# theislab/dca

Measured on NVIDIA H100. Metric: cells/sec (ZINB AE epoch, device-timed), higher is better.
Workload: dtype bf16-gemm/f32-acc/f32-loss

## Files before the change

### dca_b200/_lib.py

```python
from __future__ import annotations

import ctypes as C
import os

_HERE = os.path.dirname(os.path.abspath(__file__))
LIB_PATH = os.path.join(_HERE, "libdca_b200.so")

DCA_MAX_HIDDEN = 8
DCA_NAME_LEN = 48

ACTIVATION_IDS = {"relu": 0, "linear": 1, "elu": 2, "selu": 3, "tanh": 4, "sigmoid": 5, "hard_sigmoid": 6,
                  "softplus": 7, "softsign": 8, "exponential": 9, "LeakyReLU": 10, "PReLU": 11}
OPTIMIZERS = {"RMSprop": (0, 1e-3), "SGD": (1, 1e-2), "Adagrad": (2, 1e-2), "Adadelta": (3, 1.0), "Adam": (4, 1e-3),
              "Adamax": (5, 2e-3), "Nadam": (6, 2e-3)}
OPTIMIZERS.update({k.lower(): v for k, v in list(OPTIMIZERS.items())})
AE_TYPE_IDS = {"zinb-conddisp": 0, "zinb": 1, "nb-conddisp": 2, "nb": 3,
               "poisson": 4, "normal": 5, "nb-shared": 6, "zinb-shared": 7, "zinb-elempi": 8, "nb-fork": 9, "zinb-fork": 10}
F32, BF16 = 0, 1
GEMM_AUTO, GEMM_GENERIC, GEMM_TCGEN05 = 0, 1, 2
REGION_PARAMS, REGION_GRADS, REGION_RMS, REGION_BN_STATE, REGION_EPOCH_ACC = 0, 1, 2, 3, 4


class DcaError(RuntimeError):
    pass


class Config(C.Structure):
    _fields_ = [
        ("struct_bytes", C.c_int32), ("n_in", C.c_int32), ("n_out", C.c_int32),
        ("n_hidden", C.c_int32), ("hidden", C.c_int32 * DCA_MAX_HIDDEN),
        ("ae_type", C.c_int32), ("batchnorm", C.c_int32), ("max_batch", C.c_int32),
        ("x_dtype", C.c_int32), ("gemm_path", C.c_int32),
        ("ridge", C.c_float), ("l1", C.c_float), ("l2", C.c_float),
        ("l1_enc", C.c_float), ("l2_enc", C.c_float),
        ("bn_momentum", C.c_float), ("bn_eps", C.c_float),
        ("rms_rho", C.c_float), ("rms_eps", C.c_float),
        ("elempi_shared", C.c_int32), ("sync_bn", C.c_int32),
        ("activation", C.c_int32), ("input_dropout", C.c_float),
        ("hidden_dropout", C.c_float * DCA_MAX_HIDDEN), ("dropout_seed", C.c_uint64),
    ]


class TensorInfo(C.Structure):
    _fields_ = [("name", C.c_char * DCA_NAME_LEN), ("offset", C.c_int64),
                ("rows", C.c_int32), ("cols", C.c_int32)]


class PackedCountsDesc(C.Structure):
    _fields_ = [
        ("struct_bytes", C.c_int32), ("bits", C.c_int32), ("n_rows", C.c_int64), ("genes", C.c_int32),
        ("max_row_nibble_bytes", C.c_int32), ("packed", C.c_void_p), ("ovf_indptr", C.c_void_p),
        ("ovf_entries", C.c_void_p), ("nib_indptr", C.c_void_p), ("nibbles", C.c_void_p), ("n_counts", C.c_void_p),
    ]


_vp, _i32, _i64, _f, _sz = C.c_void_p, C.c_int32, C.c_int64, C.c_float, C.c_size_t
PROTOTYPES = {
    "dca_version": (C.c_int, []),
    "dca_last_error": (C.c_char_p, []),
    "dca_config_default": (None, [C.POINTER(Config)]),
    "dca_arena_bytes": (C.c_int, [C.POINTER(Config), C.POINTER(_sz)]),
    "dca_create": (C.c_int, [C.POINTER(Config), _vp, _sz, C.POINTER(_vp)]),
    "dca_destroy": (C.c_int, [_vp]),
    "dca_param_count": (C.c_int, [_vp, C.POINTER(_i64), C.POINTER(_i32)]),
    "dca_param_info": (C.c_int, [_vp, _i32, C.POINTER(TensorInfo)]),
    "dca_state_count": (C.c_int, [_vp, C.POINTER(_i64), C.POINTER(_i32)]),
    "dca_state_info": (C.c_int, [_vp, _i32, C.POINTER(TensorInfo)]),
    "dca_region": (C.c_int, [_vp, _i32, C.POINTER(_vp), C.POINTER(_i64)]),
    "dca_init_params": (C.c_int, [_vp, C.c_uint64, _vp]),
    "dca_params_changed": (C.c_int, [_vp, _vp]),
    "dca_train_step": (C.c_int, [_vp, _vp, _i64, _vp, _i64, _vp, _vp, _i32, _vp]),
    "dca_train_step_phase": (C.c_int, [_vp, _vp, _i64, _vp, _i64, _vp, _vp, _i32, _i32, _vp]),
    "dca_grad_buckets": (C.c_int, [_vp, C.POINTER(_i64)]),
    "dca_comm_unique_id": (C.c_int, [_vp]),
    "dca_comm_init": (C.c_int, [_vp, _vp, _i32, _i32]),
    "dca_comm_destroy": (C.c_int, [_vp]),
    "dca_allreduce": (C.c_int, [_vp, _vp]),
    "dca_train_step_dp": (C.c_int, [_vp, _vp, _i64, _vp, _i64, _vp, _vp, _i32, _vp]),
    "dca_set_optimizer": (C.c_int, [_vp, _i32, _vp]),
    "dca_reset_optimizer": (C.c_int, [_vp, _vp]),
    "dca_apply_update": (C.c_int, [_vp, _f, _f, _f, _vp]),
    "dca_eval_step": (C.c_int, [_vp, _vp, _i64, _vp, _i64, _vp, _vp, _i32, _vp]),
    "dca_predict": (C.c_int, [_vp, _vp, _i64, _vp, _vp, _i32, _vp, _vp, _vp, _i64, _vp, _vp]),
    "dca_read_loss": (C.c_int, [_vp, C.POINTER(_f), C.POINTER(_i32), _vp]),
    "dca_read_epoch_acc": (C.c_int, [_vp, C.POINTER(C.c_double * 4), _i32, _vp]),
    "dca_train_step_host": (C.c_int, [_vp, _vp, _vp, _vp, _i32, _f, _f, C.POINTER(_f), _vp]),
    "dca_set_input_transform": (C.c_int, [_vp, _vp, _vp, _i32, _i32, _vp]),
    "dca_set_loss_ring": (C.c_int, [_vp, _vp, _i32]),
    "dca_stream_begin": (C.c_int, [_vp, _vp, _i64, _vp, _i64, _i32, _vp]),
    "dca_stream_begin_packed": (C.c_int, [_vp, _vp, _i32, _i64, _vp, _vp, _vp, _i64, _i32, _vp]),
    "dca_stream_begin_sparse": (C.c_int, [_vp, _vp, _vp, _vp, _vp, _vp, _vp, _i64, _i32, _vp]),
    "dca_stream_step": (C.c_int, [_vp, _i64, _i64, _vp]),
    "dca_stream_end": (C.c_int, [_vp, _vp]),
    "dca_expand_packed_counts": (C.c_int, [_vp, _i32, _vp, _vp, _vp, _i32, _i32, _vp, _vp, _i32, _i32, _vp, _vp, _i32, _vp,
                                           _vp]),
    "dca_expand_sparse_counts": (C.c_int, [_vp, _vp, _vp, _i32, _vp, _vp, _vp, _i32, _i32, _vp, _vp, _i32, _i32, _vp, _vp,
                                           _i32, _vp, _vp]),
    "dca_zinb_loss_fwd_bwd": (C.c_int, [_vp, _i64, _vp, _vp, _vp, _vp, _vp, _i64, _i32, _i32, _i32, _f, _f,
                                        _vp, _vp, _vp, _i32, _vp, _vp, _vp, _sz, _vp]),
    "dca_zinb_loss_workspace_bytes": (C.c_int, [_i32, _i32, C.POINTER(_sz)]),
    "dca_zinb_loss_fwd": (C.c_int, [_vp, _i64, _vp, _vp, _vp, _vp, _vp, _i64, _i32, _i32, _i32, _f,
                                    _vp, _vp, _sz, _vp]),
    "dca_zinb_elem_host": (C.c_int, [_i32, _f, _f, _f, _f, _f, _f, C.POINTER(_f * 4)]),
    "dca_dropout_mask_host": (C.c_int, [C.c_uint64, C.c_uint64, _i32, _i64, _f, _vp]),
    "dca_activation_host": (C.c_int, [_i32, _f, _f, C.POINTER(_f * 2)]),
    "dca_dense_heads_fwd": (C.c_int, [_vp, _i64, _i32, _i32, _i32, _vp, _vp, _vp, _vp, _vp, _vp, _vp,
                                      _vp, _vp, _vp, _i64, _vp]),
    "dca_tc_heads_fwd": (C.c_int, [_vp, _i32, _vp, _vp, _i32, _i32, C.POINTER(_i32 * 3), _vp, _vp, _vp, _vp, _i64, _vp]),
    "dca_tc_heads_loss": (C.c_int, [_vp, _i32, _vp, _vp, _i32, _vp, _i64, _vp, _vp, _f, _f, _vp, _vp, _vp, _i64, _vp,
                                    _vp, _sz, _vp]),
    "dca_tc_gene_gemm": (C.c_int, [_i32, _vp, _vp, _vp, _i64, _i32, _i32, _i32, _vp, _vp, _vp, _vp, _vp, _vp, _i64, _i32,
                                   _vp, _vp, _vp, _vp]),
    "dca_tc_gene_gemm_sms": (C.c_int, [_i32, _vp, _vp, _vp, _i64, _i32, _i32, _i32, _vp, _vp, _vp, _vp, _vp, _vp, _i64,
                                       _i32, _vp, _vp, _vp, _vp, _i32]),
    "dca_tc_gene_gemm_rows": (C.c_int, [_i32, _vp, _vp, _vp, _i64, _vp, _i32, _i32, _i32, _vp, _vp, _vp, _vp, _vp, _vp,
                                        _i64, _i32, _vp, _vp, _vp, _vp, _i32]),
    "dca_tc_probe": (C.c_int, [_vp, _i32, _i32, _vp, _i32, _i32, _i32, _i32, _i32, _i32, _i32, _i32, _i32, _i32, _i32,
                               _vp, _vp]),
    "dca_profile_enable": (C.c_int, [_vp, _i32]),
    "dca_profile_read": (C.c_int, [_vp, C.POINTER(C.c_double * 6), C.POINTER(C.c_int64 * 6), _i32]),
    "dca_engine_info": (C.c_int, [_vp, C.POINTER(_i32 * 8)]),
    "dca_write_text_matrix": (C.c_int, [C.c_char_p, _vp, _i32, _i64, _i64, _i64, _vp, _vp, _i32, _i32]),
    "dca_read_text_counts": (C.c_int, [C.c_char_p, _i32, _i32, _i64, _i32, _vp, _vp, _i64, _vp, _vp, _i64, _vp]),
    "dca_count_escapes": (C.c_int, [_vp, _i32, _i64, _i64, _i64, _vp, _i32]),
    "dca_pack_counts": (C.c_int, [_vp, _i32, _i64, _i64, _i64, _i32, _vp, _vp, _vp, _i32]),
    "dca_sparse_counts": (C.c_int, [_vp, _i32, _i64, _i64, _i64, _vp, _vp, _i32]),
    "dca_pack_sparse": (C.c_int, [_vp, _i32, _i64, _i64, _i64, _vp, _vp, _vp, _vp, _vp, _i32]),
    "dca_preprocess_workspace_bytes": (C.c_int, [_i64, _i32, C.POINTER(_sz)]),
    "dca_counts_csr_to_dense": (C.c_int, [_vp, _vp, _vp, _i64, _i32, _vp, _i64, _vp]),
    "dca_count_totals": (C.c_int, [_vp, _i64, _i64, _i32, _vp, _vp, _vp, _vp, _sz, _vp]),
    "dca_gather_counts": (C.c_int, [_vp, _i64, _vp, _i64, _vp, _i32, _vp, _i64, _vp]),
    "dca_log_moments": (C.c_int, [_vp, _i64, _i64, _i32, _vp, C.c_double, _i32, _vp, _vp, _vp, _sz, _vp]),
    "dca_normalize_write": (C.c_int, [_vp, _i64, _i64, _i32, _vp, C.c_double, _i32, _vp, _vp, _vp, _i32, _i64, _vp]),
    "dca_stats_workspace_bytes": (C.c_int, [_i64, _i32, _i64, C.POINTER(_sz)]),
    "dca_stats_begin": (C.c_int, [_i64, _i32, _vp, _sz, _vp]),
    "dca_count_totals_rows": (C.c_int, [_vp, _i64, _i64, _i64, _i64, _i32, _vp, _vp, _sz, _vp]),
    "dca_count_totals_finish": (C.c_int, [_i64, _i32, _vp, _vp, _vp, _sz, _vp]),
    "dca_log_moments_rows": (C.c_int, [_i32, _vp, _i64, _i64, _i64, _i64, _i32, _vp, C.c_double, _i32, _vp, _vp, _sz,
                                       _vp]),
    "dca_log_moments_finish": (C.c_int, [_i32, _i64, _i32, _i32, _vp, _vp, _sz, _vp]),
    "dca_set_input_transform_exact": (C.c_int, [_vp, _vp, _vp, C.c_double, _i32, _vp]),
    "dca_stream_row_totals": (C.c_int, [_vp, _vp]),
    "dca_stream_predict": (C.c_int, [_vp, _i64, _i64, _vp, _vp, _vp, _i64, _vp, _vp]),
    "dca_stream_eval": (C.c_int, [_vp, _i64, _i64, _vp]),
    "dca_stream_capacity": (C.c_int, [_vp, C.POINTER(_i64), C.POINTER(_i64)]),
    "dca_expand_packed_counts_exact": (C.c_int, [_vp, _i32, _vp, _vp, _vp, _i32, _i32, C.c_double, _i32, _vp, _vp, _vp,
                                                 _vp, _i32, _vp, _vp]),
    "dca_expand_sparse_counts_exact": (C.c_int, [_vp, _vp, _vp, _i32, _vp, _vp, _vp, _i32, _i32, C.c_double, _i32, _vp,
                                                 _vp, _vp, _vp, _i32, _vp, _vp]),
    "dca_pack_count_rows": (C.c_int, [_vp, _i64, _i64, _i32, _vp, _i64, _vp]),
    "dca_pack_rows_device": (C.c_int, [_vp, _i64, _i64, _i64, C.POINTER(PackedCountsDesc), _vp]),
    "dca_expand_rows_exact": (C.c_int, [C.POINTER(PackedCountsDesc), _vp, _i32, C.c_double, _i32, _vp, _vp, _vp, _vp, _i32,
                                        _vp, _vp]),
    "dca_packed_train_step": (C.c_int, [_vp, C.POINTER(PackedCountsDesc), _vp, _i32, _vp]),
    "dca_packed_eval_step": (C.c_int, [_vp, C.POINTER(PackedCountsDesc), _vp, _i32, _vp]),
    "dca_packed_predict": (C.c_int, [_vp, C.POINTER(PackedCountsDesc), _vp, _i32, _vp, _vp, _vp, _i64, _vp, _vp]),
    "dca_launch_count": (C.c_int64, []),
    "dca_set_tunable": (C.c_int, [C.c_char_p, C.c_int64]),
}

_lib = None


def load():
    global _lib
    if _lib is not None:
        return _lib
    if not os.path.exists(LIB_PATH):
        raise ImportError(
            "dca_b200: %s not found. Build it with `python -c 'import __graft_entry__ as g; g.build()'` "
            "(or `make -C dca_b200/csrc`). There is no CPU fallback." % LIB_PATH)
    lib = C.CDLL(LIB_PATH)
    for name, (res, args) in PROTOTYPES.items():
        fn = getattr(lib, name)
        fn.restype = res
        fn.argtypes = args
    _lib = lib
    return lib


def check(status: int, what: str = ""):
    if status != 0:
        msg = load().dca_last_error().decode("utf-8", "replace")
        if status == -1:
            raise ValueError("%s: %s" % (what or "dca_b200", msg))
        raise DcaError("%s failed (status %d): %s" % (what or "dca_b200", status, msg))


def set_tunable(name: str, value: int):
    check(load().dca_set_tunable(name.encode(), int(value)), "dca_set_tunable")


def default_config() -> Config:
    cfg = Config()
    load().dca_config_default(C.byref(cfg))
    return cfg
```

### dca_b200/csrc/dca_internal.cuh

```cuda
#pragma once
#include <cuda_runtime.h>
#include <cuda_bf16.h>
#include <stdint.h>
#include <stddef.h>
#include <atomic>
#include "../../include/dca_b200.h"

namespace dca {

void set_error(const char* fmt, ...);
extern std::atomic<long long> g_launches;
inline void count_launch(int n = 1) { g_launches.fetch_add(n, std::memory_order_relaxed); }

#define DCA_CUDA_OK(expr)                                                              \
  do {                                                                                 \
    cudaError_t _e = (expr);                                                           \
    if (_e != cudaSuccess) {                                                           \
      ::dca::set_error("%s failed: %s (%s:%d)", #expr, cudaGetErrorString(_e), __FILE__, __LINE__); \
      return DCA_ERR_CUDA;                                                             \
    }                                                                                  \
  } while (0)

#define DCA_LAUNCH_CHECK()                                                             \
  do {                                                                                 \
    ::dca::count_launch();                                                             \
    cudaError_t _e = cudaGetLastError();                                               \
    if (_e != cudaSuccess) {                                                           \
      ::dca::set_error("kernel launch failed: %s (%s:%d)", cudaGetErrorString(_e), __FILE__, __LINE__); \
      return DCA_ERR_CUDA;                                                             \
    }                                                                                  \
  } while (0)

#define DCA_TRY(expr)                \
  do {                               \
    int _s = (expr);                 \
    if (_s != DCA_OK) return _s;     \
  } while (0)

static inline int cdiv(long long a, long long b) { return (int)((a + b - 1) / b); }

enum Epilogue : int {
  EPI_STORE = 0,
  EPI_ACCUM = 1,
  EPI_MEAN_ACT = 2,
  EPI_DISP_ACT = 3,
  EPI_SIGMOID = 4,
  EPI_LINEAR_SCALE = 5
};

struct GemmArgs {
  const void* A; int64_t lda; int a_bf16; int transA;
  const int32_t* a_rows;
  const float* B; int64_t ldb; int transB;
  float* C; int64_t ldc;
  int M, N, K;
  const float* bias;
  const float* row_scale;
  int epilogue;
  int splits;
};
int gemm_generic(const GemmArgs& g, cudaStream_t s);

int fill_rows_with_bias(float* C, int64_t ldc, int M, int N, const float* bias, cudaStream_t s);
int col_sums(const float* a, const float* b, int64_t ld, int M, int N, double* out_sum, double* out_prod,
             double* scratch, cudaStream_t s);
int col_sums_scratch_elems(int M, int N);
int bn_train_finalize(const double* sum, const double* sq, int M, int N, float eps, float momentum,
                      float* mean, float* inv_std, float* moving_mean, float* moving_var, cudaStream_t s);
int bn_relu_fwd(const float* a, int64_t ld, int M, int N, const float* mean, const float* inv_std,
                const float* beta, float* xhat, float* h, __nv_bfloat16* h_bf16, cudaStream_t s);
int bn_infer_prepare(const float* moving_mean, const float* moving_var, int N, float eps,
                     float* mean, float* inv_std, cudaStream_t s);
int bias_relu_fwd(const float* a, int64_t ld, int M, int N, float* h, __nv_bfloat16* h_bf16, cudaStream_t s);
int relu_bwd(float* dh, const float* h, int64_t ld, int M, int N, cudaStream_t s);
int bn_bwd_apply(float* g_inout, const float* xhat, int64_t ld, int M, int N, const float* inv_std,
                 const double* sum_g, const double* sum_gx, float* dbeta, cudaStream_t s, int stat_rows = 0);
int col_sum_to_float(const double* sum, int N, float* out, cudaStream_t s);
int theta_prepare(const float* theta_raw, int G, float* theta, float* chain, cudaStream_t s);
int theta_grad_finish(const float* dtheta, const float* chain, int G, float scale, float* grad_out, cudaStream_t s);
int add_reg_grad(const float* w, float* g, int64_t n, float l1, float l2, cudaStream_t s);
int reg_penalty(const float* w, int64_t n, float l1, float l2, double* acc, cudaStream_t s);
int rmsprop_update(float* params, const float* grads, float* rms, int64_t n, float lr, float clip,
                   float rho, float eps, float grad_scale, __nv_bfloat16* shadow, float* loss_out, cudaStream_t s);
struct OptScalars { int kind; float lr, clip, gs, c0, c1, c2, c3, c4; };
int optimizer_update(float* params, const float* grads, float* s1, float* s2, int64_t n, OptScalars o, __nv_bfloat16* shadow,
                     float* loss_out, cudaStream_t s);
int glorot_fill(float* w, int64_t n, int fan_in, int fan_out, uint64_t seed, uint64_t stream_id, cudaStream_t s);
int fill_value(float* p, int64_t n, float v, cudaStream_t s);
int cast_to_bf16(const float* in, __nv_bfloat16* out, int64_t n, cudaStream_t s);

__device__ __forceinline__ float pre_log_value(float y, double sf64, int flags) {
  float q = (flags & DCA_PRE_SIZE_FACTORS) ? (float)((double)y / sf64) : y;
  if ((flags & DCA_PRE_LOG1P) && q != 0.f) q = (float)log1p((double)q);
  return q;
}
struct ExactXform {
  const double* n_counts; double median; int flags;
  const double* mean; const double* std; const float* x_zero;
};
int exact_zero_inputs(const double* mean, const double* std, int n, float* x_zero, cudaStream_t s);
int expand_counts(const void* cnt, int bits, const float* sf_in, int M, int n, const float* mean, const float* inv_std, int use_sf,
                  int use_log1p, float* Yout, void* Xout, int x_bf16, float* sf_out, const int64_t* ovf_indptr,
                  const void* ovf_entries, cudaStream_t s, const ExactXform* ex = nullptr, const int32_t* rows = nullptr);
int expand_sparse(const void* bitmap, const int64_t* nib_indptr, const void* nibbles, const float* sf_in, int M, int n,
                  const float* mean, const float* inv_std, int use_sf, int use_log1p, float* Yout, void* Xout, int x_bf16,
                  float* sf_out, const int64_t* ovf_indptr, const void* ovf_entries, int max_row_nibble_bytes, cudaStream_t s,
                  const ExactXform* ex = nullptr, const int32_t* rows = nullptr);
int check_packed_counts(const char* who, const dca_packed_counts* p);
int gather_rows_bf16(const void* X, int x_bf16, int64_t ldx, const int32_t* rows, int M, int n, __nv_bfloat16* out,
                     cudaStream_t s);

namespace tc {
int heads_fwd_tc(const __nv_bfloat16* Hb, int B, const __nv_bfloat16* const W[3], const float* const bias[3], int G,
                 int n_heads, const int kind[3], const float* row_scale, float* const out[3], int64_t ld_out, int sm_count,
                 cudaStream_t s);
int gene_gemm_tc(int mode, const __nv_bfloat16* const Z[3], int64_t ldz, const int32_t* rows, int B, int G, int n_heads,
                 const __nv_bfloat16* H, const __nv_bfloat16* const W[3], float* out_b, float* const dW[3], int64_t dW_ld,
                 int dW_transposed, float* const db[3], void* ws, size_t ws_bytes, int sm_count, cudaStream_t s);
size_t gene_gemm_workspace_bytes(int B);
int flash_zinb_tc(const __nv_bfloat16* H3, int B, int G, const __nv_bfloat16* const W[3], const float* const bias[3],
                  const float* Y, int64_t ldy, const int32_t* rows, const float* sf, float ridge, float inv_n,
                  float* dH3, float* const dW[3], float* const db[3], void* ws, size_t ws_bytes, double* loss_sum,
                  const double* penalty, float* loss_slot, double* epoch_acc, int batch, const float* lf_dev, int sm_count,
                  cudaStream_t s);
}

struct LossArgs {
  const float* Y; int64_t ldy; const int32_t* rows; const float* sf;
  const float* m; const float* d; const float* pi; int64_t ld;
  int B, G; int ae_type; float ridge; float inv_n;
  void* dzm; void* dzd; void* dzp; int grad_bf16;
  float* dtheta;
  double* loss_sum;
  void* ws; size_t ws_bytes;
  int counter_ready = 0;
  float* fin_loss_slot = nullptr; double* fin_epoch_acc = nullptr; const double* fin_penalty = nullptr; int fin_batch = 0;
};
size_t loss_workspace_bytes(int B, int G);
extern int g_fused_heads_default;
const float* loss_log_fact_table();
int zinb_loss_fwd_bwd(const LossArgs& a, cudaStream_t s);
int zinb_loss_fwd(const LossArgs& a, cudaStream_t s);

struct HeadsLossArgs {
  const __nv_bfloat16* H3; int B, G;
  const __nv_bfloat16* W[3]; const float* bias[3];
  const float* Y; int64_t ldy; const int32_t* rows; const float* sf;
  float ridge, inv_n;
  __nv_bfloat16* dz[3]; int64_t ldz;
  double* loss_sum; void* ws; size_t ws_bytes;
  int counter_ready = 0;
  float* fin_loss_slot = nullptr; double* fin_epoch_acc = nullptr; const double* fin_penalty = nullptr; int fin_batch = 0;
};
int heads_loss_tc(const HeadsLossArgs& a, cudaStream_t s);

}
```

### dca_b200/csrc/dense_tc.cu

```cuda
#include <mutex>
#include "engine.h"
#include "tc_common.cuh"
#include "head_act.cuh"

namespace dca {
namespace tc {

typedef CUresult (*EncodeTiledFn)(CUtensorMap*, CUtensorMapDataType, cuuint32_t, void*, const cuuint64_t*,
                                  const cuuint64_t*, const cuuint32_t*, const cuuint32_t*, CUtensorMapInterleave,
                                  CUtensorMapSwizzle, CUtensorMapL2promotion, CUtensorMapFloatOOBfill);

static EncodeTiledFn encode_fn() {
  static EncodeTiledFn fn = nullptr;
  static std::once_flag once;
  std::call_once(once, [] {
    void* p = nullptr;
    cudaDriverEntryPointQueryResult q;
    if (cudaGetDriverEntryPoint("cuTensorMapEncodeTiled", &p, cudaEnableDefault, &q) == cudaSuccess &&
        q == cudaDriverEntryPointSuccess)
      fn = reinterpret_cast<EncodeTiledFn>(p);
  });
  return fn;
}

int make_tensor_map_2d(CUtensorMap* out, const void* base, int elem_bytes, int is_bf16, uint64_t rows, uint64_t cols,
                       uint64_t ld_elems, uint32_t box_rows, uint32_t box_cols, int swizzle) {
  EncodeTiledFn fn = encode_fn();
  if (!fn) { set_error("cuTensorMapEncodeTiled is not available from the driver"); return DCA_ERR_CUDA; }
  cuuint64_t dims[2] = {cols, rows};
  cuuint64_t strides[1] = {ld_elems * (uint64_t)elem_bytes};
  cuuint32_t box[2] = {box_cols, box_rows};
  cuuint32_t estr[2] = {1, 1};
  const CUtensorMapDataType dt = is_bf16 ? CU_TENSOR_MAP_DATA_TYPE_BFLOAT16 : CU_TENSOR_MAP_DATA_TYPE_FLOAT32;
  CUresult r = fn(out, dt, 2, const_cast<void*>(base), dims, strides, box, estr, CU_TENSOR_MAP_INTERLEAVE_NONE,
                  swizzle ? CU_TENSOR_MAP_SWIZZLE_128B : CU_TENSOR_MAP_SWIZZLE_NONE, CU_TENSOR_MAP_L2_PROMOTION_L2_256B,
                  CU_TENSOR_MAP_FLOAT_OOB_FILL_NONE);
  if (r != CUDA_SUCCESS) {
    set_error("cuTensorMapEncodeTiled failed (%d): rows=%llu cols=%llu ld=%llu box=%ux%u elem=%d", (int)r,
              (unsigned long long)rows, (unsigned long long)cols, (unsigned long long)ld_elems, box_rows, box_cols, elem_bytes);
    return DCA_ERR_CUDA;
  }
  return DCA_OK;
}

struct ProbeParams {
  int a_mn, b_mn, M, N, K;
  int a_boxes, a_box_bytes, a_box_c0, a_box_c1;
  int b_boxes, b_box_bytes, b_box_c0, b_box_c1;
  uint32_t a_lbo, a_sbo, a_kstep, a_kblock_steps, a_kblock_bytes, a_mn64_bytes;
  uint32_t b_lbo, b_sbo, b_kstep, b_kblock_steps, b_kblock_bytes, b_mn64_bytes;
};

template <int NC, int TA, int TB>
__device__ __forceinline__ void probe_mma(float (&acc)[NC / 2], uint64_t da, uint64_t db) {
  if constexpr (NC == 128) wgmma_m64n128k16<TA, TB>(acc, da, db, 1u);
  else wgmma_m64n64k16<TA, TB>(acc, da, db, 1u);
}

template <int NC>
__device__ __forceinline__ void probe_chunk(const ProbeParams& p, uint32_t sa, uint32_t sb, int m0, int n0, float* D) {
  float acc[NC / 2];
#pragma unroll
  for (int i = 0; i < NC / 2; ++i) acc[i] = 0.f;
  const uint32_t a0 = sa + (uint32_t)(m0 / 64) * p.a_mn64_bytes, b0 = sb + (uint32_t)(n0 / 64) * p.b_mn64_bytes;
  wgmma_fence();
  for (int j = 0; j < p.K / 16; ++j) {
    const uint32_t aoff = (j / p.a_kblock_steps) * p.a_kblock_bytes + (j % p.a_kblock_steps) * p.a_kstep;
    const uint32_t boff = (j / p.b_kblock_steps) * p.b_kblock_bytes + (j % p.b_kblock_steps) * p.b_kstep;
    const uint64_t da = make_smem_desc(a0 + aoff, p.a_lbo, p.a_sbo), db = make_smem_desc(b0 + boff, p.b_lbo, p.b_sbo);
    if (p.a_mn) { if (p.b_mn) probe_mma<NC, 1, 1>(acc, da, db); else probe_mma<NC, 1, 0>(acc, da, db); }
    else        { if (p.b_mn) probe_mma<NC, 0, 1>(acc, da, db); else probe_mma<NC, 0, 0>(acc, da, db); }
  }
  wgmma_commit();
  wgmma_wait<0>();
  acc_fence(acc);
  const int w = threadIdx.x >> 5, l = threadIdx.x & 31;
#pragma unroll
  for (int i = 0; i < NC / 2; ++i) {
    const int row = m0 + 16 * w + (l >> 2) + 8 * ((i >> 1) & 1), col = n0 + 8 * (i >> 2) + 2 * (l & 3) + (i & 1);
    D[(size_t)row * p.N + col] = acc[i];
  }
}

__global__ void __launch_bounds__(128, 1)
tc_probe_kernel(const __grid_constant__ CUtensorMap map_a, const __grid_constant__ CUtensorMap map_b,
                const ProbeParams p, float* __restrict__ D) {
  extern __shared__ __align__(1024) uint8_t smem_raw[];
  uint8_t* smem = smem_raw + ((1024u - (smem_u32(smem_raw) & 1023u)) & 1023u);
  __shared__ uint64_t bar_load;
  uint8_t* sa = smem;
  uint8_t* sb = smem + (size_t)p.a_boxes * p.a_box_bytes;
  if (threadIdx.x == 0) { mbar_init(&bar_load, 1); fence_barrier_init(); }
  __syncthreads();
  if (threadIdx.x == 0) {
    mbar_expect_tx(&bar_load, (uint32_t)(p.a_boxes * p.a_box_bytes + p.b_boxes * p.b_box_bytes));
    for (int i = 0; i < p.a_boxes; ++i) tma_load_2d(sa + (size_t)i * p.a_box_bytes, &map_a, i * p.a_box_c0, i * p.a_box_c1, &bar_load);
    for (int i = 0; i < p.b_boxes; ++i) tma_load_2d(sb + (size_t)i * p.b_box_bytes, &map_b, i * p.b_box_c0, i * p.b_box_c1, &bar_load);
  }
  mbar_wait(&bar_load, 0);
  for (int m0 = 0; m0 < p.M; m0 += 64)
    for (int n0 = 0; n0 < p.N;) {
      if (p.N - n0 >= 128) { probe_chunk<128>(p, smem_u32(sa), smem_u32(sb), m0, n0, D); n0 += 128; }
      else { probe_chunk<64>(p, smem_u32(sa), smem_u32(sb), m0, n0, D); n0 += 64; }
    }
}

namespace k2 {
constexpr int BM = 128, BN = 128, BK = 64;
constexpr int kThreads = 256;
constexpr uint32_t kABytes = BM * BK * 2, kBBytes = BN * BK * 2;
constexpr uint32_t kSmemBytes = kABytes + kBBytes + 1024;

struct Params {
  int B, G, n_heads;
  int kind[3];
  int m_tiles, n_tiles_per_head;
  const float* bias[3];
  const float* row_scale;
  float* out[3]; int64_t ld_out;
};

__global__ void __launch_bounds__(kThreads, 2)
heads_fwd_kernel(const __grid_constant__ CUtensorMap map_h, const __grid_constant__ CUtensorMap map_w0,
                 const __grid_constant__ CUtensorMap map_w1, const __grid_constant__ CUtensorMap map_w2, const Params p) {
  extern __shared__ __align__(1024) uint8_t smem_raw[];
  uint8_t* smem = smem_raw + ((1024u - (smem_u32(smem_raw) & 1023u)) & 1023u);
  __shared__ uint64_t full_bar;
  const int mt = blockIdx.x % p.m_tiles, r = blockIdx.x / p.m_tiles;
  const int nt = r % p.n_tiles_per_head, hs = r / p.n_tiles_per_head;
  if (threadIdx.x == 0) {
    mbar_init(&full_bar, 1);
    fence_barrier_init();
    const CUtensorMap* mw = hs == 0 ? &map_w0 : (hs == 1 ? &map_w1 : &map_w2);
    mbar_expect_tx(&full_bar, kABytes + kBBytes);
    tma_load_2d(smem, &map_h, 0, mt * BM, &full_bar);
    tma_load_2d(smem + kABytes, mw, nt * BN, 0, &full_bar);
    tma_load_2d(smem + kABytes + kBBytes / 2, mw, nt * BN + 64, 0, &full_bar);
  }
  __syncthreads();
  const int wg = threadIdx.x >> 7, w = (threadIdx.x >> 5) & 3, l = threadIdx.x & 31;
  const int col0 = nt * BN + 2 * (l & 3);
  const int row0 = mt * BM + wg * 64 + 16 * w + (l >> 2);
  const float* bias = p.bias[hs];
  const int kind = p.kind[hs];
  float2 bz[16];
#pragma unroll
  for (int c = 0; c < 16; ++c) bz[c] = (col0 + 8 * c < p.G) ? *reinterpret_cast<const float2*>(bias + col0 + 8 * c) : make_float2(0.f, 0.f);
  float rs[2] = {1.f, 1.f};
  if (kind == EPI_MEAN_ACT && p.row_scale) {
    if (row0 < p.B) rs[0] = p.row_scale[row0];
    if (row0 + 8 < p.B) rs[1] = p.row_scale[row0 + 8];
  }
  float acc[64];
#pragma unroll
  for (int i = 0; i < 64; ++i) acc[i] = 0.f;
  mbar_wait(&full_bar, 0);
  head_tile_mma(acc, smem_u32(smem) + wg * 64 * 128, smem_u32(smem) + kABytes);
  float* out = p.out[hs];
  auto emit = [&](auto act) {
#pragma unroll
    for (int h = 0; h < 2; ++h) {
      const int row = row0 + 8 * h;
      if (row >= p.B) continue;
      float* orow = out + (int64_t)row * p.ld_out;
#pragma unroll
      for (int c = 0; c < 16; ++c) {
        const int col = col0 + 8 * c;
        if (col < p.G)
          *reinterpret_cast<float2*>(orow + col) =
              make_float2(act(acc[4 * c + 2 * h], bz[c].x, rs[h]), act(acc[4 * c + 2 * h + 1], bz[c].y, rs[h]));
      }
    }
  };
  if (kind == EPI_MEAN_ACT) emit([](float a, float b, float s) { return head_out<EPI_MEAN_ACT>(a, b, s); });
  else if (kind == EPI_DISP_ACT) emit([](float a, float b, float s) { return head_out<EPI_DISP_ACT>(a, b, s); });
  else emit([](float a, float b, float s) { return head_out<EPI_SIGMOID>(a, b, s); });
}
}

int heads_fwd_tc(const __nv_bfloat16* Hb, int B, const __nv_bfloat16* const W[3], const float* const bias[3], int G,
                 int n_heads, const int kind[3], const float* row_scale, float* const out[3], int64_t ld_out, int sm_count,
                 cudaStream_t s) {
  using namespace k2;
  if (ld_out % 4 != 0 || G % 8 != 0) { set_error("heads_fwd_tc: G must be a multiple of 8 and ld_out of 4 (TMA strides)"); return DCA_ERR_BAD_ARG; }
  CUtensorMap mh, mw[3];
  DCA_TRY(make_tensor_map_2d(&mh, Hb, 2, 1, (uint64_t)B, 64, 64, BM, BK, 1));
  for (int i = 0; i < 3; ++i)
    DCA_TRY(make_tensor_map_2d(&mw[i], W[i < n_heads ? i : 0], 2, 1, 64, (uint64_t)G, (uint64_t)G, 64, 64, 1));
  Params p;
  p.B = B; p.G = G; p.n_heads = n_heads;
  for (int i = 0; i < 3; ++i) { const int k = i < n_heads ? i : 0; p.kind[i] = kind[i]; p.bias[i] = bias[k]; p.out[i] = out[k]; }
  p.m_tiles = cdiv(B, BM); p.n_tiles_per_head = cdiv(G, BN);
  p.row_scale = row_scale; p.ld_out = ld_out;
  (void)sm_count;
  static bool attr_set = false;
  if (!attr_set) {
    DCA_CUDA_OK(cudaFuncSetAttribute(heads_fwd_kernel, cudaFuncAttributeMaxDynamicSharedMemorySize, (int)kSmemBytes));
    attr_set = true;
  }
  const int grid = p.m_tiles * p.n_tiles_per_head * n_heads;
  heads_fwd_kernel<<<grid, kThreads, kSmemBytes, s>>>(mh, mw[0], mw[1], mw[2], p);
  DCA_LAUNCH_CHECK();
  return DCA_OK;
}

}

Engine::~Engine() {
  comm_destroy();
  for (auto e : prof.ev) cudaEventDestroy(e);
  for (auto& g : graphs) if (g.exec) cudaGraphExecDestroy(g.exec);
  if (hs.copy) cudaStreamDestroy(hs.copy);
  if (hs.expand) cudaStreamDestroy(hs.expand);
  for (int k = 0; k < 3; ++k) {
    if (hs.ready[k]) cudaEventDestroy(hs.ready[k]);
    if (hs.step_done[k]) cudaEventDestroy(hs.step_done[k]);
  }
  for (int k = 0; k < 2; ++k) {
    if (hs.h2d_done[k]) cudaEventDestroy(hs.h2d_done[k]);
    if (hs.cnt_free[k]) cudaEventDestroy(hs.cnt_free[k]);
  }
}

}

using namespace dca;

extern "C" int dca_tc_probe(const void* A, int32_t a_rows, int32_t a_cols, const void* Bm, int32_t b_rows, int32_t b_cols,
                            int32_t a_mn_major, int32_t b_mn_major, int32_t M, int32_t N, int32_t K,
                            int32_t a_lbo, int32_t a_sbo, int32_t b_lbo, int32_t b_sbo, float* D, void* stream) {
  using namespace tc;
  if (M != 128 || N % 64 != 0 || N < 64 || N > 256 || K % 64 != 0 || K <= 0 || K > 256) {
    set_error("dca_tc_probe: need M=128, N%%64==0 (64..256), K%%64==0 (<=256)"); return DCA_ERR_BAD_ARG;
  }
  ProbeParams p{};
  p.a_mn = a_mn_major; p.b_mn = b_mn_major; p.M = M; p.N = N; p.K = K;
  CUtensorMap ma, mb;
  auto setup = [&](int mn, int mn_extent, int rows, int cols, const void* base, CUtensorMap* map, int& boxes, int& box_bytes,
                   int& c0, int& c1, uint32_t& lbo, uint32_t& sbo, uint32_t& kstep, uint32_t& kb_steps, uint32_t& kb_bytes,
                   uint32_t& mn64_bytes, int lbo_o, int sbo_o) -> int {
    if (!mn) {
      if (rows != mn_extent || cols != K) { set_error("dca_tc_probe: K-major operand must be [MN x K]"); return DCA_ERR_BAD_ARG; }
      DCA_TRY(make_tensor_map_2d(map, base, 2, 1, rows, cols, cols, mn_extent, 64, 1));
      boxes = K / 64; box_bytes = mn_extent * 128; c0 = 64; c1 = 0;
      lbo = 0; sbo = 1024; kstep = 32; kb_steps = 4; kb_bytes = box_bytes; mn64_bytes = 64 * 128;
    } else {
      if (rows != K || cols != mn_extent || mn_extent % 64) { set_error("dca_tc_probe: MN-major operand must be [K x MN], MN%%64==0"); return DCA_ERR_BAD_ARG; }
      DCA_TRY(make_tensor_map_2d(map, base, 2, 1, rows, cols, cols, K, 64, 1));
      boxes = mn_extent / 64; box_bytes = K * 128; c0 = 64; c1 = 0;
      lbo = box_bytes; sbo = 1024; kstep = 2048; kb_steps = 1u << 30; kb_bytes = 0; mn64_bytes = box_bytes;
    }
    if (lbo_o >= 0) lbo = lbo_o;
    if (sbo_o >= 0) sbo = sbo_o;
    return DCA_OK;
  };
  DCA_TRY(setup(a_mn_major, M, a_rows, a_cols, A, &ma, p.a_boxes, p.a_box_bytes, p.a_box_c0, p.a_box_c1, p.a_lbo, p.a_sbo,
                p.a_kstep, p.a_kblock_steps, p.a_kblock_bytes, p.a_mn64_bytes, a_lbo, a_sbo));
  DCA_TRY(setup(b_mn_major, N, b_rows, b_cols, Bm, &mb, p.b_boxes, p.b_box_bytes, p.b_box_c0, p.b_box_c1, p.b_lbo, p.b_sbo,
                p.b_kstep, p.b_kblock_steps, p.b_kblock_bytes, p.b_mn64_bytes, b_lbo, b_sbo));
  const size_t smem = (size_t)p.a_boxes * p.a_box_bytes + (size_t)p.b_boxes * p.b_box_bytes + 1024;
  DCA_CUDA_OK(cudaFuncSetAttribute(tc_probe_kernel, cudaFuncAttributeMaxDynamicSharedMemorySize, (int)smem));
  tc_probe_kernel<<<1, 128, smem, (cudaStream_t)stream>>>(ma, mb, p, D);
  DCA_LAUNCH_CHECK();
  return DCA_OK;
}

extern "C" int dca_tc_heads_fwd(const void* Hb, int32_t batch, const void* Wk, const float* bias, int32_t genes,
                                int32_t n_heads, const int32_t kind[3], const float* row_scale, float* out0, float* out1,
                                float* out2, int64_t ld_out, void* stream) {
  if (!Hb || !Wk || !bias || batch <= 0 || genes <= 0 || n_heads < 1 || n_heads > 3 || !out0) {
    set_error("dca_tc_heads_fwd: bad argument"); return DCA_ERR_BAD_ARG;
  }
  int dev = 0, sms = 132;
  cudaGetDevice(&dev);
  cudaDeviceGetAttribute(&sms, cudaDevAttrMultiProcessorCount, dev);
  int k[3] = {kind[0], n_heads > 1 ? kind[1] : 0, n_heads > 2 ? kind[2] : 0};
  float* outs[3] = {out0, out1, out2};
  const __nv_bfloat16* W[3]; const float* b[3];
  for (int i = 0; i < 3; ++i) {
    const int j = i < n_heads ? i : 0;
    W[i] = (const __nv_bfloat16*)Wk + (size_t)j * 64 * genes; b[i] = bias + (size_t)j * genes;
  }
  return tc::heads_fwd_tc((const __nv_bfloat16*)Hb, batch, W, b, genes, n_heads, k, row_scale, outs, ld_out, sms,
                          (cudaStream_t)stream);
}
```

### dca_b200/csrc/engine.cu

```cuda
#include <cmath>
#include <cstdarg>
#include <cstdio>
#include <cstring>
#include <cstdlib>
#include <string>
#include <vector>
#include "dca_internal.cuh"
#include "engine.h"

namespace dca {

std::atomic<long long> g_launches{0};
static thread_local char g_err[512] = "";

void set_error(const char* fmt, ...) {
  va_list ap;
  va_start(ap, fmt);
  vsnprintf(g_err, sizeof(g_err), fmt, ap);
  va_end(ap);
}

namespace {

inline size_t align_up(size_t v, size_t a = 256) { return (v + a - 1) / a * a; }

__global__ void add_double_kernel(double* p, double v) { *p += v; }
__global__ void gather_sf_kernel(const float* __restrict__ sf, const int32_t* __restrict__ rows, int n,
                                 float* __restrict__ out) {
  const int i = blockIdx.x * blockDim.x + threadIdx.x;
  if (i < n) out[i] = sf ? sf[rows ? rows[i] : i] : 1.0f;
}
__global__ void copy_strided_kernel(const float* __restrict__ in, int64_t ldi, float* __restrict__ out, int64_t ldo,
                                    int M, int N) {
  const int64_t i = (int64_t)blockIdx.x * blockDim.x + threadIdx.x;
  if (i >= (int64_t)M * N) return;
  const int r = (int)(i / N), c = (int)(i % N);
  out[(int64_t)r * ldo + c] = in[(int64_t)r * ldi + c];
}

int validate(const dca_config* c) {
  if (!c) { set_error("config is NULL"); return DCA_ERR_BAD_ARG; }
  if (c->struct_bytes != (int32_t)sizeof(dca_config)) {
    set_error("dca_config.struct_bytes=%d does not match library (%zu): header/library mismatch", c->struct_bytes,
              sizeof(dca_config));
    return DCA_ERR_BAD_ARG;
  }
  if (c->n_in <= 0 || c->n_out <= 0) { set_error("n_in/n_out must be positive (got %d, %d)", c->n_in, c->n_out); return DCA_ERR_BAD_ARG; }
  if (c->n_hidden < 0 || c->n_hidden > DCA_MAX_HIDDEN) { set_error("n_hidden must be in [0,%d]", DCA_MAX_HIDDEN); return DCA_ERR_BAD_ARG; }
  for (int i = 0; i < c->n_hidden; ++i)
    if (c->hidden[i] <= 0) { set_error("hidden[%d] must be positive", i); return DCA_ERR_BAD_ARG; }
  if (c->ae_type < 0 || c->ae_type > DCA_AE_ZINB_FORK) { set_error("autoencoder type not supported (ae_type=%d)", c->ae_type); return DCA_ERR_UNSUPPORTED; }
  if (c->max_batch <= 0) { set_error("max_batch must be positive"); return DCA_ERR_BAD_ARG; }
  if (c->x_dtype != DCA_F32 && c->x_dtype != DCA_BF16) { set_error("x_dtype must be DCA_F32 or DCA_BF16"); return DCA_ERR_BAD_ARG; }
  if (c->gemm_path < 0 || c->gemm_path > 2) { set_error("unknown gemm_path %d", c->gemm_path); return DCA_ERR_BAD_ARG; }
  if (c->activation < DCA_ACT_RELU || c->activation > DCA_ACT_PRELU) { set_error("unknown activation %d", c->activation); return DCA_ERR_BAD_ARG; }
  if (c->activation == DCA_ACT_PRELU && c->ae_type >= DCA_AE_NB_FORK) {
    set_error("activation PReLU is not available for the fork types"); return DCA_ERR_UNSUPPORTED;
  }
  if (!(c->input_dropout >= 0.f && c->input_dropout < 1.f)) { set_error("input_dropout must be in [0, 1)"); return DCA_ERR_BAD_ARG; }
  for (int i = 0; i < c->n_hidden; ++i)
    if (!(c->hidden_dropout[i] >= 0.f && c->hidden_dropout[i] < 1.f)) { set_error("hidden_dropout[%d] must be in [0, 1)", i); return DCA_ERR_BAD_ARG; }
  return DCA_OK;
}

void add_tensor(std::vector<dca_tensor_info>& v, int64_t& off, const std::string& name, int rows, int cols) {
  dca_tensor_info t;
  memset(&t, 0, sizeof(t));
  snprintf(t.name, sizeof(t.name), "%s", name.c_str());
  t.offset = off; t.rows = rows; t.cols = cols;
  off += (int64_t)rows * cols;
  v.push_back(t);
}

std::string layer_name(int i, int n) {
  const int center = n / 2;
  if (i == center) return "center";
  if (i < center) return "enc" + std::to_string(i);
  return "dec" + std::to_string(i - center);
}

}

int Engine::plan(const dca_config& c) {
  cfg = c;
  L = c.n_hidden;
  has_pi = (c.ae_type == DCA_AE_ZINB_CONDDISP || c.ae_type == DCA_AE_ZINB);
  cond = (c.ae_type == DCA_AE_ZINB_CONDDISP || c.ae_type == DCA_AE_NB_CONDDISP);
  params.clear(); states.clear(); reg_items.clear();
  int64_t off = 0, soff = 0;
  x_kind = 0; n_branch = 0; trunk_L = L;
  if (c.ae_type >= DCA_AE_POISSON) {
    DCA_TRY(x_plan_params(c, off, soff));
  } else {
  int prev = c.n_in;
  maxh = 1;
  for (int i = 0; i < L; ++i) {
    const std::string nm = layer_name(i, L);
    const int h = c.hidden[i];
    lay[i].in = prev; lay[i].out = h;
    lay[i].W = off; add_tensor(params, off, nm + "/kernel", prev, h);
    lay[i].b = off; add_tensor(params, off, nm + "/bias", 1, h);
    if (c.batchnorm) {
      lay[i].beta = off; add_tensor(params, off, nm + "/bn_beta", 1, h);
      lay[i].mm = soff; add_tensor(states, soff, nm + "/bn_moving_mean", 1, h);
      lay[i].mv = soff; add_tensor(states, soff, nm + "/bn_moving_var", 1, h);
    }
    if (c.activation == DCA_ACT_PRELU) { lay[i].alpha = off; add_tensor(params, off, nm + "_act/alpha", 1, h); }
    lay[i].drop = c.hidden_dropout[i]; lay[i].id = i;
    prev = h;
    if (h > maxh) maxh = h;
  }
  K_head = prev;
  head_W[0] = off; add_tensor(params, off, "mean/kernel", prev, c.n_out);
  head_b[0] = off; add_tensor(params, off, "mean/bias", 1, c.n_out);
  head_W[1] = head_b[1] = head_W[2] = head_b[2] = theta_off = -1;
  if (cond) {
    head_W[1] = off; add_tensor(params, off, "dispersion/kernel", prev, c.n_out);
    head_b[1] = off; add_tensor(params, off, "dispersion/bias", 1, c.n_out);
  }
  if (has_pi) {
    head_W[2] = off; add_tensor(params, off, "pi/kernel", prev, c.n_out);
    head_b[2] = off; add_tensor(params, off, "pi/bias", 1, c.n_out);
  }
  if (!cond) { theta_off = off; add_tensor(params, off, "dispersion/theta", 1, c.n_out); }
  }
  P = off; S = soff;

  const int G = c.n_out;
  const size_t B = (size_t)c.max_batch;
  size_t o = 0;
  auto take = [&](size_t bytes) { size_t at = o; o = align_up(o + bytes); return at; };
  o_params = take(sizeof(float) * (size_t)P);
  o_grads = take(sizeof(float) * (size_t)(P + 2));
  o_rms = take(sizeof(float) * (size_t)P);
  o_opt2 = take(sizeof(float) * (size_t)P);
  o_state = take(sizeof(float) * (size_t)(S > 0 ? S : 1));
  o_acc = take(sizeof(double) * 8);
  for (int i = 0; i < L; ++i) {
    const size_t h = (size_t)c.hidden[i];
    lay[i].o_a = take(sizeof(float) * B * h);
    lay[i].o_xhat = take(sizeof(float) * B * h);
    lay[i].o_h = take(sizeof(float) * B * h);
    lay[i].o_mean = take(sizeof(float) * h);
    lay[i].o_inv = take(sizeof(float) * h);
  }
  for (int k = 0; k < 3; ++k) o_head[k] = take(sizeof(float) * B * (size_t)G);
  o_dh[0] = take(sizeof(float) * B * (size_t)maxh);
  o_dh[1] = take(sizeof(float) * B * (size_t)maxh);
  const size_t statw = (size_t)(maxh > G ? maxh : G);
  o_dsum = take(sizeof(double) * statw);
  o_dprod = take(sizeof(double) * statw);
  o_scratch = take(sizeof(double) * (size_t)col_sums_scratch_elems((int)B, (int)statw));
  o_theta = take(sizeof(float) * (size_t)G);
  o_chain = take(sizeof(float) * (size_t)G);
  o_dtheta = take(sizeof(float) * (size_t)G);
  o_sfb = take(sizeof(float) * B);
  loss_ws_bytes = loss_workspace_bytes((int)B, G);
  o_lossws = take(loss_ws_bytes);
  o_rowsbuf = take(sizeof(int32_t) * B);
  o_step = take(256);
  if (c.activation == DCA_ACT_PRELU) o_actscr = take(sizeof(float) * B * (size_t)maxh);
  if (c.input_dropout > 0.f) o_xdrop = take((c.x_dtype == DCA_BF16 ? sizeof(__nv_bfloat16) : sizeof(float)) * B * (size_t)c.n_in);
  mid_ok = !x_kind && plain_hidden() && mid_supported(c.hidden, L);
  o_bar = take(256);
  o_midpart = take(sizeof(double) * mid_partial_doubles());
  o_midgpart = take(sizeof(float) * mid_grad_partial_floats(L));
  n_slots = 0;
  slot_head[0] = 0; slot_kind[0] = EPI_MEAN_ACT; n_slots = 1;
  if (cond) { slot_head[n_slots] = 1; slot_kind[n_slots] = EPI_DISP_ACT; ++n_slots; }
  if (has_pi) { slot_head[n_slots] = 2; slot_kind[n_slots] = EPI_SIGMOID; ++n_slots; }
  const bool want_tc = c.gemm_path != DCA_GEMM_GENERIC && !x_kind;
  tc_heads = want_tc && L >= 1 && K_head == 64 && (G % 8 == 0);
  tc_enc = want_tc && L >= 1 && c.hidden[0] == 64 && (c.n_in % 8 == 0);
  if (tc_heads) for (int k = 0; k < 3; ++k) if (head_W[k] >= 0 && (head_W[k] % 8) != 0) tc_heads = false;
  {
    const char* ev = getenv("DCA_FUSED_HEADS");
    const bool want = ev ? atoi(ev) != 0 : g_fused_heads_default != 0;
    fused_heads = want && tc_heads && cond && has_pi && L >= 1 && (G % 8 == 0);
  }
  if (tc_enc && (lay[0].W % 8) != 0) tc_enc = false;
  if (tc_heads || tc_enc) o_pbf = take(2 * (size_t)P);
  if (tc_heads || tc_enc) { ggws_bytes = tc::gene_gemm_workspace_bytes((int)B); o_ggws = take(ggws_bytes); }
  if (tc_heads) {
    o_h3b = take(2 * B * 64);
    for (int k = 0; k < n_slots; ++k) o_dzb[k] = take(2 * B * (size_t)G);
  }
  if (tc_enc) {
    o_da1b = take(2 * B * 64);
    if (c.x_dtype != DCA_BF16) o_xb = take(2 * B * (size_t)c.n_in);
  }
  for (int k = 0; k < 2; ++k) { o_cnt[k] = take(sizeof(uint16_t) * B * (size_t)c.n_in); o_sfst[k] = take(sizeof(float) * B); }
  ovf_cap = (int64_t)(B * (size_t)c.n_in / 32); if (ovf_cap < 4096) ovf_cap = 4096;
  for (int k = 0; k < 2; ++k) { o_ovp[k] = take(sizeof(int64_t) * (B + 1)); o_ove[k] = take(8 * (size_t)ovf_cap); }
  nib_cap = (int64_t)(B * (size_t)c.n_in / 4) + 64;
  for (int k = 0; k < 2; ++k) { o_nibp[k] = take(sizeof(int64_t) * (B + 1)); o_nib[k] = take((size_t)nib_cap); }
  o_gmean = take(sizeof(float) * (size_t)c.n_in); o_ginv = take(sizeof(float) * (size_t)c.n_in);
  o_gmean64 = take(sizeof(double) * (size_t)c.n_in); o_gstd64 = take(sizeof(double) * (size_t)c.n_in);
  o_gx0 = take(sizeof(float) * (size_t)c.n_in);
  for (int k = 0; k < 2; ++k) o_ncst[k] = take(sizeof(double) * B);
  const size_t xb = (c.x_dtype == DCA_BF16) ? 2 : 4;
  for (int k = 0; k < kExpBufs; ++k) {
    o_sx[k] = take(xb * B * (size_t)c.n_in);
    o_sy[k] = take(sizeof(float) * B * (size_t)G);
    o_ssf[k] = take(sizeof(float) * B);
  }
  o_stage_x = o_sx[0]; o_stage_y = o_sy[0]; o_stage_sf = o_ssf[0];
  if (x_kind) x_plan_arena(B, take);
  arena_bytes = o;
  return DCA_OK;
}

void Engine::mark(int phase, cudaStream_t s) {
  if (!prof.on) return;
  if (prof.n == prof.ev.size()) {
    cudaEvent_t e;
    if (cudaEventCreate(&e) != cudaSuccess) return;
    prof.ev.push_back(e); prof.phase.push_back(-1);
  }
  prof.phase[prof.n] = phase;
  cudaEventRecord(prof.ev[prof.n], s);
  ++prof.n;
}

int Engine::prof_collect() {
  if (prof.n == 0) return DCA_OK;
  DCA_CUDA_OK(cudaEventSynchronize(prof.ev[prof.n - 1]));
  for (size_t i = 0; i + 1 < prof.n; ++i) {
    const int ph = prof.phase[i];
    if (ph < 0 || ph >= DCA_N_PHASES) continue;
    float ms = 0.f;
    if (cudaEventElapsedTime(&ms, prof.ev[i], prof.ev[i + 1]) == cudaSuccess) { prof.ms[ph] += ms; prof.cnt[ph] += 1; }
  }
  prof.n = 0;
  return DCA_OK;
}

void Engine::bind(void* base_) {
  base = reinterpret_cast<char*>(base_);
}

int Engine::gemm_auto(GemmArgs g, cudaStream_t s) {
  const long long tiles = (long long)cdiv(g.M, 64) * cdiv(g.N, 64), target = 2ll * sm_count;
  int splits = 1;
  if (g.epilogue == EPI_ACCUM && tiles < target && g.K >= 256) {
    splits = (int)((target + tiles - 1) / tiles);
    const int maxs = g.K / 128;
    if (splits > maxs) splits = maxs;
    if (splits < 1) splits = 1;
  }
  g.splits = splits;
  return gemm_generic(g, s);
}

int Engine::forward(const void* X, int64_t ldx, const int32_t* rows, int Bn, bool training, cudaStream_t s) {
  const void* hin = X; int64_t ldin = ldx; int in_bf16 = x_override_bf16 ? 1 : (cfg.x_dtype == DCA_BF16); const int32_t* gather = rows;
  cur_x = XOperand{};
  if (tc_enc && (reinterpret_cast<uintptr_t>(X) & 15) == 0) {
    if (in_bf16 && ldx % 8 == 0) cur_x = XOperand{reinterpret_cast<const __nv_bfloat16*>(X), ldx, rows};
    else if (!in_bf16 && ldx % 4 == 0) {
      DCA_TRY(gather_rows_bf16(X, in_bf16, ldx, rows, Bn, cfg.n_in, bf(o_xb), s));
      cur_x = XOperand{bf(o_xb), cfg.n_in, nullptr};
    }
  }
  const bool fused = use_mid(Bn);
  for (int i = 0; i < (fused ? 1 : L); ++i) {
    Layer& l = lay[i];
    float* a = f(l.o_a);
    DCA_TRY(fill_rows_with_bias(a, l.out, Bn, l.out, pp(l.b), s));
    if (i == 0 && cur_x.base) {
      const __nv_bfloat16* Z[3] = {cur_x.base, cur_x.base, cur_x.base};
      const __nv_bfloat16* W1[3] = {bf(o_pbf) + lay[0].W, bf(o_pbf) + lay[0].W, bf(o_pbf) + lay[0].W};
      DCA_TRY(tc::gene_gemm_tc(1, Z, cur_x.ld, cur_x.rows, Bn, cfg.n_in, 1, nullptr, W1, a, nullptr, 0, 0, nullptr, base + o_ggws, ggws_bytes, sm_count, s));
    } else {
    GemmArgs g{};
    g.A = hin; g.lda = ldin; g.a_bf16 = in_bf16; g.transA = 0; g.a_rows = gather;
    g.B = pp(l.W); g.ldb = l.out; g.transB = 0;
    g.C = a; g.ldc = l.out; g.M = Bn; g.N = l.out; g.K = l.in; g.epilogue = EPI_ACCUM;
    DCA_TRY(gemm_auto(g, s));
    }
    if (fused) break;
    if (cfg.batchnorm) {
      if (training) {
        DCA_TRY(col_sums(a, nullptr, l.out, Bn, l.out, d(o_dsum), d(o_dprod), d(o_scratch), s));
        DCA_TRY(bn_allreduce(d(o_dsum), d(o_dprod), l.out, s));
        DCA_TRY(bn_train_finalize(d(o_dsum), d(o_dprod), bn_rows(Bn), l.out, cfg.bn_eps, cfg.bn_momentum, f(l.o_mean),
                                  f(l.o_inv), st(l.mm), st(l.mv), s));
      } else {
        DCA_TRY(bn_infer_prepare(st(l.mm), st(l.mv), l.out, cfg.bn_eps, f(l.o_mean), f(l.o_inv), s));
      }
    }
    DCA_TRY(act_fwd(l, Bn, training, (tc_heads && i == L - 1) ? bf(o_h3b) : nullptr, s));
    hin = f(l.o_h); ldin = l.out; in_bf16 = 0; gather = nullptr;
  }
  if (fused) {
    mid::Params mp;
    mid_params(mp, Bn, training);
    DCA_TRY(mid_forward(mp, s));
    hin = f(lay[L - 1].o_h); ldin = lay[L - 1].out; in_bf16 = 0; gather = nullptr;
  }
  head_in = hin; head_ld = ldin; head_bf16 = in_bf16; head_rows = gather;
  return DCA_OK;
}

int Engine::x_gather_sf(const float* sf, const int32_t* rows, int Bn, cudaStream_t s) {
  gather_sf_kernel<<<cdiv(Bn, 256), 256, 0, s>>>(sf, rows, Bn, f(o_sfb));
  DCA_LAUNCH_CHECK();
  return DCA_OK;
}

void Engine::mid_params(mid::Params& p, int Bn, bool training) {
  memset(&p, 0, sizeof(p));
  p.L = L; p.B = Bn; p.training = training ? 1 : 0; p.batchnorm = cfg.batchnorm; p.center = L / 2;
  for (int i = 0; i < L; ++i) {
    Layer& l = lay[i];
    p.w[i] = l.out; p.W[i] = pp(l.W); p.b[i] = pp(l.b);
    p.beta[i] = cfg.batchnorm ? pp(l.beta) : nullptr;
    p.mm[i] = cfg.batchnorm ? st(l.mm) : nullptr; p.mv[i] = cfg.batchnorm ? st(l.mv) : nullptr;
    p.mean[i] = f(l.o_mean); p.inv[i] = f(l.o_inv); p.xhat[i] = f(l.o_xhat); p.h[i] = f(l.o_h);
    p.gW[i] = gp(l.W); p.gb[i] = gp(l.b); p.gbeta[i] = cfg.batchnorm ? gp(l.beta) : nullptr;
  }
  p.a0 = f(lay[0].o_a); p.a_center = f(lay[L / 2].o_a);
  p.h_last_bf16 = tc_heads ? bf(o_h3b) : nullptr;
  p.partial = d(o_midpart); p.gpart = f(o_midgpart); p.bar = reinterpret_cast<unsigned*>(base + o_bar);
  p.eps = cfg.bn_eps; p.momentum = cfg.bn_momentum;
}

int Engine::heads_forward(int Bn, float* m_out, float* d_out, float* p_out, int64_t ld_out, const float* row_scale,
                          cudaStream_t s) {
  const int G = cfg.n_out;
  if (tc_heads && (ld_out % 4 == 0)) {
    float* outs_by_head[3] = {m_out, d_out, p_out};
    bool all = true;
    for (int k = 0; k < n_slots; ++k) all = all && outs_by_head[slot_head[k]] && ((reinterpret_cast<uintptr_t>(outs_by_head[slot_head[k]]) & 15) == 0);
    if (all) {
      float* outs[3] = {nullptr, nullptr, nullptr};
      for (int k = 0; k < n_slots; ++k) outs[k] = outs_by_head[slot_head[k]];
      for (int k = n_slots; k < 3; ++k) outs[k] = outs[0];
      const __nv_bfloat16* Wk[3]; const float* bk[3];
      for (int k = 0; k < 3; ++k) { const int kk = k < n_slots ? k : 0; Wk[k] = bf(o_pbf) + head_W[slot_head[kk]]; bk[k] = pp(head_b[slot_head[kk]]); }
      return tc::heads_fwd_tc(bf(o_h3b), Bn, Wk, bk, G, n_slots, slot_kind, row_scale, outs, ld_out, sm_count, s);
    }
  }
  struct H { int k; float* out; int epi; const float* rs; } hs[3] = {
      {0, m_out, EPI_MEAN_ACT, row_scale}, {1, d_out, EPI_DISP_ACT, nullptr}, {2, p_out, EPI_SIGMOID, nullptr}};
  for (auto& h : hs) {
    if (head_W[h.k] < 0 || !h.out) continue;
    GemmArgs g{};
    g.A = head_in; g.lda = head_ld; g.a_bf16 = head_bf16; g.transA = 0; g.a_rows = head_rows;
    g.B = pp(head_W[h.k]); g.ldb = G; g.transB = 0;
    g.C = h.out; g.ldc = ld_out; g.M = Bn; g.N = G; g.K = K_head;
    g.bias = pp(head_b[h.k]); g.row_scale = h.rs; g.epilogue = h.epi; g.splits = 1;
    DCA_TRY(gemm_generic(g, s));
  }
  return DCA_OK;
}

int Engine::penalty(cudaStream_t s, bool& any) {
  any = false;
  auto coeff = [&](int i, float& l1, float& l2) {
    const int center = L / 2;
    const bool enc = (i >= 0 && i <= center);
    l1 = (enc && cfg.l1_enc != 0.f) ? cfg.l1_enc : cfg.l1;
    l2 = (enc && cfg.l2_enc != 0.f) ? cfg.l2_enc : cfg.l2;
  };
  for (int i = 0; i < L; ++i) {
    float l1, l2; coeff(i, l1, l2);
    if (l1 != 0.f || l2 != 0.f) any = true;
  }
  if (cfg.l1 != 0.f || cfg.l2 != 0.f) any = true;
  if (!any) return DCA_OK;
  DCA_CUDA_OK(cudaMemsetAsync(d(o_acc) + 5, 0, sizeof(double), s));
  for (int i = 0; i < L; ++i) {
    float l1, l2; coeff(i, l1, l2);
    if (l1 == 0.f && l2 == 0.f) continue;
    const int64_t n = (int64_t)lay[i].in * lay[i].out;
    DCA_TRY(reg_penalty(pp(lay[i].W), n, l1, l2, d(o_acc) + 5, s));
    DCA_TRY(add_reg_grad(pp(lay[i].W), gp(lay[i].W), n, l1, l2, s));
  }
  if (cfg.l1 != 0.f || cfg.l2 != 0.f) {
    for (int k = 0; k < 3; ++k) {
      if (head_W[k] < 0) continue;
      const int64_t n = (int64_t)K_head * cfg.n_out;
      DCA_TRY(reg_penalty(pp(head_W[k]), n, cfg.l1, cfg.l2, d(o_acc) + 5, s));
      DCA_TRY(add_reg_grad(pp(head_W[k]), gp(head_W[k]), n, cfg.l1, cfg.l2, s));
    }
  }
  return DCA_OK;
}

int Engine::train_step(const void* X, int64_t ldx, const float* Y, int64_t ldy, const float* sf, const int32_t* rows,
                       int Bn, cudaStream_t s, int phase) {
  if (phase < 0 || phase > 3) { set_error("dca_train_step: phase must be 0, 1, 2 or 3"); return DCA_ERR_BAD_ARG; }
  if (!X || !Y) { set_error("dca_train_step: X and Y must not be NULL"); return DCA_ERR_BAD_ARG; }
  if (Bn <= 0 || Bn > cfg.max_batch) { set_error("dca_train_step: batch %d outside (0, max_batch=%d]", Bn, cfg.max_batch); return DCA_ERR_BAD_ARG; }
  if (!graphs_enabled || prof.on || s == nullptr || s == cudaStreamLegacy || s == cudaStreamPerThread)
    return phase == 3 ? train_step_dp_body(X, ldx, Y, ldy, sf, rows, Bn, s) : train_step_body(X, ldx, Y, ldy, sf, rows, Bn, s, phase);
  StepGraph* g = nullptr;
  for (auto& c : graphs)
    if (c.X == X && c.ldx == ldx && c.Y == Y && c.ldy == ldy && c.sf == sf && c.Bn == Bn && c.has_rows == (rows != nullptr) && c.phase == phase) { g = &c; break; }
  if (!g) {
    if (graphs.size() >= 16) { for (auto& c : graphs) if (c.exec) cudaGraphExecDestroy(c.exec); graphs.clear(); }
    graphs.push_back(StepGraph{X, ldx, Y, ldy, sf, Bn, rows != nullptr, phase, nullptr, 0, 0});
    g = &graphs.back();
  }
  int32_t* rbuf = reinterpret_cast<int32_t*>(base + o_rowsbuf);
  if (!g->exec && g->seen >= 1 && g->seen < 1000) {
    const long long l0 = g_launches.load();
    if (cudaStreamBeginCapture(s, cudaStreamCaptureModeThreadLocal) == cudaSuccess) {
      const int st = phase == 3 ? train_step_dp_body(X, ldx, Y, ldy, sf, rows ? rbuf : nullptr, Bn, s)
                                : train_step_body(X, ldx, Y, ldy, sf, rows ? rbuf : nullptr, Bn, s, phase);
      cudaGraph_t graph = nullptr;
      const cudaError_t ce = cudaStreamEndCapture(s, &graph);
      if (st == DCA_OK && ce == cudaSuccess && graph && cudaGraphInstantiate(&g->exec, graph, 0) == cudaSuccess) {
        g->launches = g_launches.load() - l0;
        g_launches.store(l0);
      } else {
        if (getenv("DCA_GRAPH_DEBUG"))
          fprintf(stderr, "[dca_b200] graph capture failed: body status %d (%s), end-capture %s\n", st, g_err,
                  cudaGetErrorString(ce));
        g->exec = nullptr; g->seen = 1000;
        (void)cudaGetLastError();
      }
      if (graph) cudaGraphDestroy(graph);
    } else {
      if (getenv("DCA_GRAPH_DEBUG")) fprintf(stderr, "[dca_b200] cudaStreamBeginCapture failed: %s\n", cudaGetErrorString(cudaGetLastError()));
      (void)cudaGetLastError(); g->seen = 1000;
    }
  }
  if (g->exec) {
    if (rows && phase != 2) DCA_CUDA_OK(cudaMemcpyAsync(rbuf, rows, sizeof(int32_t) * (size_t)Bn, cudaMemcpyDeviceToDevice, s));
    DCA_CUDA_OK(cudaGraphLaunch(g->exec, s));
    count_launch((int)g->launches);
    return DCA_OK;
  }
  if (g->seen < 1000) ++g->seen;
  return phase == 3 ? train_step_dp_body(X, ldx, Y, ldy, sf, rows, Bn, s) : train_step_body(X, ldx, Y, ldy, sf, rows, Bn, s, phase);
}

int Engine::train_step_body(const void* X, int64_t ldx, const float* Y, int64_t ldy, const float* sf, const int32_t* rows,
                            int Bn, cudaStream_t s, int phase) {
  if (x_kind) return phase == 2 ? DCA_OK : x_train_step_body(X, ldx, Y, ldy, sf, rows, Bn, s);
  const int G = cfg.n_out;
  float* dh = f(o_dh[0]); float* dh2 = f(o_dh[1]);
  const int32_t* xrows = rows;
  if (cfg.input_dropout > 0.f) {
    if (phase != 2) {
      DCA_TRY(bump_step(s));
      DCA_TRY(drop_input(X, x_override_bf16 ? 1 : (cfg.x_dtype == DCA_BF16), ldx, rows, Bn, s));
    }
    X = base + o_xdrop; ldx = cfg.n_in; xrows = nullptr;
  } else if (phase != 2 && !plain_hidden()) DCA_TRY(bump_step(s));
  if (phase != 2) {
  DCA_CUDA_OK(cudaMemsetAsync(gp(0), 0, sizeof(float) * (size_t)(P + 2), s));
  bool any_pen = false;
  mark(0, s);
  DCA_TRY(penalty(s, any_pen));
  DCA_TRY(forward(X, ldx, xrows, Bn, true, s));
  mark(1, s);
  float* Mb = f(o_head[0]); float* Db = f(o_head[1]); float* Pb = f(o_head[2]);
  const float inv_n = 1.0f / ((float)Bn * (float)G);
  const bool fuse = fused_heads && (ldy % 4 == 0) && ((reinterpret_cast<uintptr_t>(Y) & 15) == 0);
  if (fuse) {
    mark(2, s);
    DCA_CUDA_OK(cudaMemsetAsync(dh, 0, sizeof(float) * (size_t)Bn * K_head, s));
    const float* lf_dev = loss_log_fact_table();
    if (!lf_dev) return DCA_ERR_CUDA;
    const __nv_bfloat16* Wk[3]; const float* bk[3]; float* dWp[3]; float* dbp[3];
    for (int k = 0; k < 3; ++k) { Wk[k] = bf(o_pbf) + head_W[k]; bk[k] = pp(head_b[k]); dWp[k] = gp(head_W[k]); dbp[k] = gp(head_b[k]); }
    DCA_TRY(tc::flash_zinb_tc(bf(o_h3b), Bn, G, Wk, bk, Y, ldy, rows, sf, cfg.ridge, inv_n, dh, dWp, dbp, base + o_lossws,
                              loss_ws_bytes, d(o_acc) + 4, any_pen ? d(o_acc) + 5 : nullptr, gp(P), d(o_acc), Bn, lf_dev,
                              sm_count, s));
  } else {
  const bool heads_loss = tc_heads && cond && has_pi && (ldy % 4 == 0) && ((reinterpret_cast<uintptr_t>(Y) & 15) == 0);
  if (!heads_loss) DCA_TRY(heads_forward(Bn, Mb, cond ? Db : nullptr, has_pi ? Pb : nullptr, G, nullptr, s));
  if (!cond) DCA_TRY(theta_prepare(pp(theta_off), G, f(o_theta), f(o_chain), s));
  mark(2, s);

  if (heads_loss) {
    HeadsLossArgs ha{};
    ha.H3 = bf(o_h3b); ha.B = Bn; ha.G = G;
    for (int k = 0; k < 3; ++k) { ha.W[k] = bf(o_pbf) + head_W[slot_head[k]]; ha.bias[k] = pp(head_b[slot_head[k]]); ha.dz[k] = bf(o_dzb[k]); }
    ha.Y = Y; ha.ldy = ldy; ha.rows = rows; ha.sf = sf; ha.ridge = cfg.ridge; ha.inv_n = inv_n; ha.ldz = G;
    ha.loss_sum = d(o_acc) + 4; ha.ws = base + o_lossws; ha.ws_bytes = loss_ws_bytes;
    ha.counter_ready = 1;
    ha.fin_loss_slot = gp(P); ha.fin_epoch_acc = d(o_acc); ha.fin_penalty = any_pen ? d(o_acc) + 5 : nullptr; ha.fin_batch = Bn;
    DCA_TRY(heads_loss_tc(ha, s));
  } else {
  LossArgs la{};
  la.Y = Y; la.ldy = ldy; la.rows = rows; la.sf = sf;
  la.m = Mb; la.d = cond ? Db : f(o_theta); la.pi = has_pi ? Pb : nullptr; la.ld = G;
  la.B = Bn; la.G = G; la.ae_type = cfg.ae_type; la.ridge = cfg.ridge; la.inv_n = inv_n;
  la.dzm = Mb; la.dzd = cond ? Db : nullptr; la.dzp = has_pi ? Pb : nullptr; la.grad_bf16 = 0;
  if (tc_heads) {
    void* slot_buf[3] = {nullptr, nullptr, nullptr};
    for (int k = 0; k < n_slots; ++k) slot_buf[slot_head[k]] = bf(o_dzb[k]);
    la.dzm = slot_buf[0]; la.dzd = cond ? slot_buf[1] : nullptr; la.dzp = has_pi ? slot_buf[2] : nullptr; la.grad_bf16 = 1;
  }
  la.dtheta = cond ? nullptr : f(o_dtheta);
  la.loss_sum = d(o_acc) + 4; la.ws = base + o_lossws; la.ws_bytes = loss_ws_bytes;
  la.counter_ready = 1;
  la.fin_loss_slot = gp(P); la.fin_epoch_acc = d(o_acc); la.fin_penalty = any_pen ? d(o_acc) + 5 : nullptr; la.fin_batch = Bn;
  DCA_TRY(zinb_loss_fwd_bwd(la, s));
  if (!cond) {
    DCA_TRY(theta_grad_finish(f(o_dtheta), f(o_chain), G, inv_n, gp(theta_off), s));
  }
  }

  mark(3, s);
  if (L > 0) DCA_CUDA_OK(cudaMemsetAsync(dh, 0, sizeof(float) * (size_t)Bn * K_head, s));
  float* dz[3] = {Mb, cond ? Db : nullptr, has_pi ? Pb : nullptr};
  if (tc_heads) {
    const __nv_bfloat16* Z[3]; const __nv_bfloat16* Wk[3]; float* dWp[3]; float* dbp[3];
    for (int k = 0; k < 3; ++k) {
      const int kk = k < n_slots ? k : 0;
      Z[k] = bf(o_dzb[kk]); Wk[k] = bf(o_pbf) + head_W[slot_head[kk]];
      dWp[k] = gp(head_W[slot_head[kk]]); dbp[k] = gp(head_b[slot_head[kk]]);
    }
    if (dp_split_heads && comm && n_slots > 1) {
      for (int k = 0; k < n_slots; ++k) {
        const __nv_bfloat16* Z1[3] = {Z[k], Z[k], Z[k]}; const __nv_bfloat16* W1[3] = {Wk[k], Wk[k], Wk[k]};
        float* dW1[3] = {dWp[k], dWp[k], dWp[k]}; float* db1[3] = {dbp[k], dbp[k], dbp[k]};
        DCA_TRY(tc::gene_gemm_tc(3, Z1, G, nullptr, Bn, G, 1, bf(o_h3b), W1, dh, dW1, G, 1, db1, base + o_ggws, ggws_bytes, sm_count, s));
        const int h = slot_head[k];
        DCA_CUDA_OK(cudaEventRecord(ev_fork, s));
        DCA_CUDA_OK(cudaStreamWaitEvent(comm_stream, ev_fork, 0));
        DCA_TRY(allreduce_range(head_W[h], head_b[h] + G, comm_stream));
      }
    } else
    DCA_TRY(tc::gene_gemm_tc(3, Z, G, nullptr, Bn, G, n_slots, bf(o_h3b), Wk, dh, dWp, G, 1, dbp, base + o_ggws, ggws_bytes, sm_count, s));
  } else
  for (int k = 0; k < 3; ++k) {
    if (head_W[k] < 0 || !dz[k]) continue;
    GemmArgs g{};
    g.A = head_in; g.lda = head_ld; g.a_bf16 = head_bf16; g.transA = 1; g.a_rows = head_rows;
    g.B = dz[k]; g.ldb = G; g.transB = 0;
    g.C = gp(head_W[k]); g.ldc = G; g.M = K_head; g.N = G; g.K = Bn; g.epilogue = EPI_ACCUM;
    DCA_TRY(gemm_auto(g, s));
    DCA_TRY(col_sums(dz[k], nullptr, G, Bn, G, d(o_dsum), nullptr, d(o_scratch), s));
    DCA_TRY(col_sum_to_float(d(o_dsum), G, gp(head_b[k]), s));
    if (L > 0) {
      GemmArgs b{};
      b.A = dz[k]; b.lda = G; b.a_bf16 = 0; b.transA = 0; b.a_rows = nullptr;
      b.B = pp(head_W[k]); b.ldb = G; b.transB = 1;
      b.C = dh; b.ldc = K_head; b.M = Bn; b.N = K_head; b.K = G; b.epilogue = EPI_ACCUM;
      DCA_TRY(gemm_auto(b, s));
    }
  }
  }
  }
  if (phase == 1) { mark(-1, s); return DCA_OK; }
  mark(4, s);
  if (L > 0 && use_mid(Bn)) {
    mid::Params mp;
    mid_params(mp, Bn, true);
    mp.dh_last = dh; mp.da0 = dh2; mp.da0_bf16 = cur_x.base ? bf(o_da1b) : nullptr;
    mp.max_ctas = dp_reserve_sms ? (sm_count - dp_reserve_sms) : 0;
    DCA_TRY(mid_backward(mp, s));
    Layer& l = lay[0];
    if (cur_x.base) {
      const __nv_bfloat16* Z[3] = {cur_x.base, cur_x.base, cur_x.base};
      float* dWp[3] = {gp(l.W), gp(l.W), gp(l.W)};
      DCA_TRY(tc::gene_gemm_tc(2, Z, cur_x.ld, cur_x.rows, Bn, cfg.n_in, 1, bf(o_da1b), nullptr, nullptr, dWp, l.out, 0, nullptr, nullptr, 0, sm_count - dp_reserve_sms, s));
    } else {
      GemmArgs g{};
      g.A = X; g.lda = ldx; g.a_bf16 = x_override_bf16 ? 1 : (cfg.x_dtype == DCA_BF16); g.transA = 1; g.a_rows = xrows;
      g.B = dh2; g.ldb = l.out; g.transB = 0;
      g.C = gp(l.W); g.ldc = l.out; g.M = l.in; g.N = l.out; g.K = Bn; g.epilogue = EPI_ACCUM;
      DCA_TRY(gemm_auto(g, s));
    }
  } else
  for (int i = L - 1; i >= 0; --i) {
    Layer& l = lay[i];
    DCA_TRY(act_bwd(l, dh, Bn, s));
    if (cfg.batchnorm) {
      DCA_TRY(col_sums(dh, f(l.o_xhat), l.out, Bn, l.out, d(o_dsum), d(o_dprod), d(o_scratch), s));
      if (bn_synced()) {
        DCA_TRY(col_sum_to_float(d(o_dsum), l.out, gp(l.beta), s));
        DCA_TRY(bn_allreduce(d(o_dsum), d(o_dprod), l.out, s));
        DCA_TRY(bn_bwd_apply(dh, f(l.o_xhat), l.out, Bn, l.out, f(l.o_inv), d(o_dsum), d(o_dprod), nullptr, s, bn_rows(Bn)));
      } else
      DCA_TRY(bn_bwd_apply(dh, f(l.o_xhat), l.out, Bn, l.out, f(l.o_inv), d(o_dsum), d(o_dprod), gp(l.beta), s));
    }
    if (i == 0 && cur_x.base) {
      DCA_TRY(cast_to_bf16(dh, bf(o_da1b), (int64_t)Bn * l.out, s));
      const __nv_bfloat16* Z[3] = {cur_x.base, cur_x.base, cur_x.base};
      float* dWp[3] = {gp(l.W), gp(l.W), gp(l.W)};
      DCA_TRY(tc::gene_gemm_tc(2, Z, cur_x.ld, cur_x.rows, Bn, cfg.n_in, 1, bf(o_da1b), nullptr, nullptr, dWp, l.out, 0, nullptr, nullptr, 0, sm_count, s));
      DCA_TRY(col_sums(dh, nullptr, l.out, Bn, l.out, d(o_dsum), nullptr, d(o_scratch), s));
      DCA_TRY(col_sum_to_float(d(o_dsum), l.out, gp(l.b), s));
      continue;
    }
    const void* ain = (i == 0) ? X : (const void*)f(lay[i - 1].o_h);
    GemmArgs g{};
    g.A = ain; g.lda = (i == 0) ? ldx : lay[i - 1].out; g.a_bf16 = (i == 0) ? (x_override_bf16 ? 1 : (cfg.x_dtype == DCA_BF16)) : 0;
    g.transA = 1; g.a_rows = (i == 0) ? xrows : nullptr;
    g.B = dh; g.ldb = l.out; g.transB = 0;
    g.C = gp(l.W); g.ldc = l.out; g.M = l.in; g.N = l.out; g.K = Bn; g.epilogue = EPI_ACCUM;
    DCA_TRY(gemm_auto(g, s));
    DCA_TRY(col_sums(dh, nullptr, l.out, Bn, l.out, d(o_dsum), nullptr, d(o_scratch), s));
    DCA_TRY(col_sum_to_float(d(o_dsum), l.out, gp(l.b), s));
    if (i > 0) {
      GemmArgs b{};
      b.A = dh; b.lda = l.out; b.transA = 0;
      b.B = pp(l.W); b.ldb = l.out; b.transB = 1;
      b.C = dh2; b.ldc = l.in; b.M = Bn; b.N = l.in; b.K = l.out; b.epilogue = EPI_STORE; b.splits = 1;
      DCA_TRY(gemm_generic(b, s));
      float* t = dh; dh = dh2; dh2 = t;
    }
  }
  mark(-1, s);
  return DCA_OK;
}

int Engine::apply_update(float lr, float clip, float grad_scale, cudaStream_t s) {
  mark(5, s);
  float* ring_slot = loss_ring ? loss_ring + (ring_pos++ % ring_n) : nullptr;
  if (opt_kind != DCA_OPT_RMSPROP) {
    OptScalars o{}; o.kind = opt_kind; o.lr = lr; o.clip = clip; o.gs = grad_scale;
    const double t = (double)(++opt_iter), b1 = 0.9, b2 = 0.999;
    if (opt_kind == DCA_OPT_ADAM) o.c0 = (float)((double)lr * sqrt(1.0 - pow(b2, t)) / (1.0 - pow(b1, t)));
    else if (opt_kind == DCA_OPT_ADAMAX) o.c0 = (float)((double)lr / (1.0 - pow(b1, t)));
    else if (opt_kind == DCA_OPT_NADAM) {
      const double sd = 0.004;
      const double mu_t = b1 * (1.0 - 0.5 * pow(0.96, t * sd)), mu_t1 = b1 * (1.0 - 0.5 * pow(0.96, (t + 1.0) * sd));
      const double sched_new = nadam_sched * mu_t, sched_next = sched_new * mu_t1;
      nadam_sched = sched_new;
      o.c0 = (float)(1.0 / (1.0 - sched_new)); o.c1 = (float)(1.0 / (1.0 - sched_next)); o.c2 = (float)(1.0 / (1.0 - pow(b2, t)));
      o.c3 = (float)mu_t; o.c4 = (float)mu_t1;
    }
    DCA_TRY(optimizer_update(pp(0), gp(0), f(o_rms), f(o_opt2), P, o, (tc_heads || tc_enc) ? bf(o_pbf) : nullptr, ring_slot, s));
    mark(-1, s);
    return DCA_OK;
  }
  DCA_TRY(rmsprop_update(pp(0), gp(0), f(o_rms), P, lr, clip, cfg.rms_rho, cfg.rms_eps, grad_scale,
                         (tc_heads || tc_enc) ? bf(o_pbf) : nullptr, ring_slot, s));
  mark(-1, s);
  return DCA_OK;
}

int Engine::reset_optimizer(cudaStream_t s) {
  DCA_CUDA_OK(cudaMemsetAsync(f(o_rms), 0, sizeof(float) * (size_t)P, s));
  DCA_CUDA_OK(cudaMemsetAsync(f(o_opt2), 0, sizeof(float) * (size_t)P, s));
  opt_iter = 0; nadam_sched = 1.0;
  return DCA_OK;
}

int Engine::eval_step(const void* X, int64_t ldx, const float* Y, int64_t ldy, const float* sf, const int32_t* rows,
                      int Bn, cudaStream_t s) {
  if (!X || !Y) { set_error("dca_eval_step: X and Y must not be NULL"); return DCA_ERR_BAD_ARG; }
  if (Bn <= 0 || Bn > cfg.max_batch) { set_error("dca_eval_step: batch %d outside (0, max_batch=%d]", Bn, cfg.max_batch); return DCA_ERR_BAD_ARG; }
  if (x_kind) return x_eval_step(X, ldx, Y, ldy, sf, rows, Bn, s);
  const int G = cfg.n_out;
  DCA_TRY(forward(X, ldx, rows, Bn, false, s));
  float* Mb = f(o_head[0]); float* Db = f(o_head[1]); float* Pb = f(o_head[2]);
  DCA_TRY(heads_forward(Bn, Mb, cond ? Db : nullptr, has_pi ? Pb : nullptr, G, nullptr, s));
  if (!cond) DCA_TRY(theta_prepare(pp(theta_off), G, f(o_theta), f(o_chain), s));
  LossArgs la{};
  la.Y = Y; la.ldy = ldy; la.rows = rows; la.sf = sf;
  la.m = Mb; la.d = cond ? Db : f(o_theta); la.pi = has_pi ? Pb : nullptr; la.ld = G;
  la.B = Bn; la.G = G; la.ae_type = cfg.ae_type; la.ridge = cfg.ridge; la.inv_n = 1.f;
  la.loss_sum = d(o_acc) + 2; la.ws = base + o_lossws; la.ws_bytes = loss_ws_bytes;
  DCA_TRY(zinb_loss_fwd(la, s));
  add_double_kernel<<<1, 1, 0, s>>>(d(o_acc) + 3, (double)Bn * (double)G);
  DCA_LAUNCH_CHECK();
  return DCA_OK;
}

int Engine::predict(const void* X, int64_t ldx, const float* sf, const int32_t* rows, int Bn, float* mean_out,
                    float* disp_out, float* pi_out, int64_t ld_out, float* latent_out, cudaStream_t s) {
  if (!X) { set_error("dca_predict: X must not be NULL"); return DCA_ERR_BAD_ARG; }
  if (Bn <= 0 || Bn > cfg.max_batch) { set_error("dca_predict: batch %d outside (0, max_batch=%d]", Bn, cfg.max_batch); return DCA_ERR_BAD_ARG; }
  if (x_kind) return x_predict(X, ldx, sf, rows, Bn, mean_out, disp_out, pi_out, ld_out, latent_out, s);
  const int G = cfg.n_out;
  DCA_TRY(forward(X, ldx, rows, Bn, false, s));
  if (latent_out) {
    if (L == 0) { set_error("dca_predict: no hidden layer -> no latent output"); return DCA_ERR_BAD_ARG; }
    const int c = L / 2;
    copy_strided_kernel<<<cdiv((int64_t)Bn * lay[c].out, 256), 256, 0, s>>>(f(lay[c].o_a), lay[c].out, latent_out,
                                                                            lay[c].out, Bn, lay[c].out);
    DCA_LAUNCH_CHECK();
  }
  const bool want_heads = mean_out || (cond && disp_out) || (has_pi && pi_out);
  if (want_heads) {
    gather_sf_kernel<<<cdiv(Bn, 256), 256, 0, s>>>(sf, rows, Bn, f(o_sfb));
    DCA_LAUNCH_CHECK();
    DCA_TRY(heads_forward(Bn, mean_out, cond ? disp_out : nullptr, has_pi ? pi_out : nullptr, ld_out, f(o_sfb), s));
  }
  if (!cond && disp_out) {
    DCA_TRY(theta_prepare(pp(theta_off), G, disp_out, f(o_chain), s));
  }
  return DCA_OK;
}

bool Engine::tc_supported() const { return tc_heads && tc_enc; }
const char* Engine::tc_reason() const {
  return "tensor-core path needs hidden_size[0] == hidden_size[-1] == 64, n_in % 8 == 0 and n_out % 8 == 0";
}
int Engine::setup_tc() {
  if (const char* e = getenv("DCA_GRAPH")) graphs_enabled = !(e[0] == '0');
  int dev = 0;
  DCA_CUDA_OK(cudaGetDevice(&dev));
  DCA_CUDA_OK(cudaDeviceGetAttribute(&sm_count, cudaDevAttrMultiProcessorCount, dev));
  if (mid_ok && !mid_device_ok()) mid_ok = false;
  if (tc_heads || tc_enc) {
    int major = 0;
    DCA_CUDA_OK(cudaDeviceGetAttribute(&major, cudaDevAttrComputeCapabilityMajor, dev));
    if (major != 9) { set_error("libdca_b200 is built for sm_90a only (device compute capability %d.x)", major); return DCA_ERR_UNSUPPORTED; }
  }
  return DCA_OK;
}
int Engine::refresh_shadows(cudaStream_t s) {
  if (!tc_heads && !tc_enc) return DCA_OK;
  return cast_to_bf16(pp(0), bf(o_pbf), P, s);
}

int Engine::init_params(uint64_t seed, cudaStream_t s) {
  DCA_CUDA_OK(cudaMemsetAsync(pp(0), 0, sizeof(float) * (size_t)P, s));
  DCA_TRY(reset_optimizer(s));
  DCA_CUDA_OK(cudaMemsetAsync(gp(0), 0, sizeof(float) * (size_t)(P + 2), s));
  DCA_CUDA_OK(cudaMemsetAsync(d(o_acc), 0, sizeof(double) * 8, s));
  uint64_t sid = 0;
  if (x_kind) {
    for (auto& t : params) {
      const std::string nm(t.name);
      if (nm.size() < 7 || nm.compare(nm.size() - 7, 7, "/kernel") != 0) continue;
      const int fi = t.rows == 1 ? t.cols : t.rows, fo = t.cols;
      DCA_TRY(glorot_fill(pp(t.offset), (int64_t)t.rows * t.cols, fi, fo, seed, sid++, s));
    }
    if (cfg.batchnorm)
      for (auto& t : states) {
        const std::string nm(t.name);
        DCA_TRY(fill_value(st(t.offset), t.cols, nm.find("moving_var") != std::string::npos ? 1.f : 0.f, s));
      }
    return DCA_OK;
  }
  for (int i = 0; i < L; ++i)
    DCA_TRY(glorot_fill(pp(lay[i].W), (int64_t)lay[i].in * lay[i].out, lay[i].in, lay[i].out, seed, sid++, s));
  for (int k = 0; k < 3; ++k)
    if (head_W[k] >= 0) DCA_TRY(glorot_fill(pp(head_W[k]), (int64_t)K_head * cfg.n_out, K_head, cfg.n_out, seed, 100 + k, s));
  if (cfg.batchnorm)
    for (int i = 0; i < L; ++i) {
      DCA_TRY(fill_value(st(lay[i].mm), lay[i].out, 0.f, s));
      DCA_TRY(fill_value(st(lay[i].mv), lay[i].out, 1.f, s));
    }
  return DCA_OK;
}

}

using namespace dca;


extern "C" int dca_version(void) { return DCA_B200_VERSION; }
extern "C" const char* dca_last_error(void) { return g_err; }
extern "C" int64_t dca_launch_count(void) { return (int64_t)g_launches.load(); }

extern "C" void dca_config_default(dca_config* c) {
  if (!c) return;
  memset(c, 0, sizeof(*c));
  c->struct_bytes = (int32_t)sizeof(dca_config);
  c->n_hidden = 3; c->hidden[0] = 64; c->hidden[1] = 32; c->hidden[2] = 64;
  c->ae_type = DCA_AE_ZINB_CONDDISP;
  c->batchnorm = 1; c->max_batch = 32; c->x_dtype = DCA_F32; c->gemm_path = DCA_GEMM_AUTO;
  c->bn_momentum = 0.99f; c->bn_eps = 1e-3f; c->rms_rho = 0.9f; c->rms_eps = 1e-7f;
}

extern "C" int dca_arena_bytes(const dca_config* cfg, size_t* bytes) {
  DCA_TRY(validate(cfg));
  if (!bytes) { set_error("dca_arena_bytes: bytes is NULL"); return DCA_ERR_BAD_ARG; }
  Engine e;
  DCA_TRY(e.plan(*cfg));
  *bytes = e.arena_bytes;
  return DCA_OK;
}

extern "C" int dca_create(const dca_config* cfg, void* arena, size_t arena_bytes, dca_handle** out) {
  if (!out) { set_error("dca_create: out is NULL"); return DCA_ERR_BAD_ARG; }
  *out = nullptr;
  DCA_TRY(validate(cfg));
  int ndev = 0;
  if (cudaGetDeviceCount(&ndev) != cudaSuccess || ndev == 0) {
    (void)cudaGetLastError();
    set_error("dca_create: no CUDA device available (this library has no CPU fallback)");
    return DCA_ERR_NO_DEVICE;
  }
  dca_handle* h = new dca_handle();
  int st = h->e.plan(*cfg);
  if (st != DCA_OK) { delete h; return st; }
  if (cfg->gemm_path == DCA_GEMM_TCGEN05 && !h->e.tc_supported()) {
    set_error("dca_create: gemm_path=TCGEN05 requested but the layer shapes do not qualify (%s)", h->e.tc_reason());
    delete h; return DCA_ERR_UNSUPPORTED;
  }
  cudaGetDevice(&h->device);
  if (arena) {
    if (arena_bytes < h->e.arena_bytes) {
      set_error("dca_create: arena too small (%zu < %zu)", arena_bytes, h->e.arena_bytes);
      delete h; return DCA_ERR_BAD_ARG;
    }
    if (reinterpret_cast<uintptr_t>(arena) & 255) { set_error("dca_create: arena must be 256-byte aligned"); delete h; return DCA_ERR_BAD_ARG; }
    h->e.bind(arena);
  } else {
    void* p = nullptr;
    cudaError_t ce = cudaMalloc(&p, h->e.arena_bytes);
    if (ce != cudaSuccess) { set_error("dca_create: cudaMalloc(%zu) failed: %s", h->e.arena_bytes, cudaGetErrorString(ce)); delete h; return DCA_ERR_CUDA; }
    h->owned = p;
    h->e.bind(p);
  }
  cudaError_t ce = cudaMemset(h->e.base, 0, h->e.arena_bytes);
  if (ce != cudaSuccess) { set_error("dca_create: cudaMemset failed: %s", cudaGetErrorString(ce)); if (h->owned) cudaFree(h->owned); delete h; return DCA_ERR_CUDA; }
  st = h->e.setup_tc();
  if (st != DCA_OK) { if (h->owned) cudaFree(h->owned); delete h; return st; }
  *out = h;
  return DCA_OK;
}

extern "C" int dca_destroy(dca_handle* h) {
  if (!h) return DCA_OK;
  if (h->owned) cudaFree(h->owned);
  delete h;
  return DCA_OK;
}

#define DCA_NEED_HANDLE(h) \
  if (!(h)) { set_error("%s: handle is NULL", __func__); return DCA_ERR_BAD_ARG; }

extern "C" int dca_param_count(const dca_handle* h, int64_t* n, int32_t* nt) {
  DCA_NEED_HANDLE(h);
  if (n) *n = h->e.P;
  if (nt) *nt = (int32_t)h->e.params.size();
  return DCA_OK;
}
extern "C" int dca_param_info(const dca_handle* h, int32_t i, dca_tensor_info* info) {
// ... 611 lines not shown
```

### dca_b200/csrc/gene_gemm_tc.cu

```cuda
#include "engine.h"
#include "tc_common.cuh"

namespace dca {
namespace tc {
int g_gg_profile = 0;
namespace gg {

constexpr int kThreads = 256;
constexpr uint32_t kZBytes = 128 * 128 * 2;
constexpr uint32_t kWBytes = 64 * 128 * 2;
constexpr uint32_t kHBytes = 128 * 64 * 2;
constexpr uint32_t kOutBytes = 128 * 64 * 4;
constexpr uint32_t kOnesBytes = 16 * 128;
constexpr int kMaxGb = 4;
constexpr int kMaxSlots = 16;

template <bool DO_A, bool DO_B>
constexpr int stages() { return DO_A && DO_B ? 2 : 3; }
template <bool DO_A, bool DO_B>
constexpr uint32_t stage_bytes() { return kZBytes + (DO_B ? kWBytes : 0) + (DO_A ? kHBytes : 0); }
template <bool DO_A, bool DO_B, bool COLSUM>
constexpr uint32_t smem_bytes() {
  return stages<DO_A, DO_B>() * stage_bytes<DO_A, DO_B>() + (DO_A ? kOutBytes : 0) + (COLSUM ? kOnesBytes : 0) + 1024;
}

struct Params {
  int B, G, n_heads;
  int n_cb, n_gb;
  int gb_per_item, cb_per_item;
  int gene_ranges, cell_splits;
  int total_items;
  float* db[3];
  float* part; int64_t part_stride;
  const int32_t* rows; const __nv_bfloat16* zsrc; int64_t ldz;
};

__device__ __forceinline__ void cp_async_16(uint32_t smem_dst, const void* src, uint32_t src_bytes) {
  asm volatile("cp.async.cg.shared.global [%0], [%1], 16, %2;" ::"r"(smem_dst), "l"(src), "r"(src_bytes) : "memory");
}
__device__ __forceinline__ void cp_async_commit() { asm volatile("cp.async.commit_group;" ::: "memory"); }
template <int N>
__device__ __forceinline__ void cp_async_wait() { asm volatile("cp.async.wait_group %0;" ::"n"(N) : "memory"); }

template <bool DO_A, bool DO_B, bool COLSUM, bool WK, int MAXG>
__global__ void __launch_bounds__(kThreads, 1)
gene_gemm_kernel(const __grid_constant__ CUtensorMap map_z0, const __grid_constant__ CUtensorMap map_z1,
                 const __grid_constant__ CUtensorMap map_z2, const __grid_constant__ CUtensorMap map_h,
                 const __grid_constant__ CUtensorMap map_w0, const __grid_constant__ CUtensorMap map_w1,
                 const __grid_constant__ CUtensorMap map_w2, const __grid_constant__ CUtensorMap map_dw0, const __grid_constant__ CUtensorMap map_dw1,
                 const __grid_constant__ CUtensorMap map_dw2, const int dw_transposed, const Params p) {
  constexpr int kStages = stages<DO_A, DO_B>();
  constexpr uint32_t kStage = stage_bytes<DO_A, DO_B>();
  extern __shared__ __align__(1024) uint8_t smem_raw[];
  uint8_t* smem = smem_raw + ((1024u - (smem_u32(smem_raw) & 1023u)) & 1023u);
  uint8_t* s_st = smem;
  float* s_o = reinterpret_cast<float*>(s_st + kStages * kStage);
  uint8_t* s_ones = reinterpret_cast<uint8_t*>(s_o) + (DO_A ? kOutBytes : 0);
  __shared__ uint64_t full[kStages];

  if (threadIdx.x == 0) {
    for (int i = 0; i < kStages; ++i) mbar_init(&full[i], 1);
    fence_barrier_init();
  }
  if (COLSUM) {
    for (int i = threadIdx.x; i < (int)kOnesBytes / 4; i += kThreads) reinterpret_cast<uint32_t*>(s_ones)[i] = 0x3F803F80u;
    fence_proxy_async_smem();
  }
  __syncthreads();

  const int wg = threadIdx.x >> 7, w = (threadIdx.x >> 5) & 3, l = threadIdx.x & 31;
  const int frow = 16 * w + (l >> 2), fcol = 2 * (l & 3);

  auto stage_begin = [&]() {
    if (threadIdx.x == 0) bulk_wait_read<0>();
    __syncthreads();
  };
  auto stage_end = [&](const CUtensorMap* m, int c0, int c1) {
    fence_proxy_async_smem();
    __syncthreads();
    if (threadIdx.x == 0) { tma_reduce_add_2d(m, c0, c1, s_o); bulk_commit(); }
  };

  uint32_t T0 = 0;
  const bool gather = p.rows != nullptr;
  const int g_rh = threadIdx.x >> 3, g_c = threadIdx.x & 7, g_h = g_rh & 1, g_r0 = g_rh >> 1;
  const uint32_t g_dst = g_h * (kZBytes / 2) + g_r0 * 128 + ((g_c ^ (g_r0 & 7)) << 4);
  int src_row[8];
  for (int item = blockIdx.x; item < p.total_items; item += gridDim.x) {
    const int cs = item % p.cell_splits, r = item / p.cell_splits;
    const int gr = r % p.gene_ranges, head = r / p.gene_ranges;
    const int gb0 = gr * p.gb_per_item, ng = min(p.n_gb, gb0 + p.gb_per_item) - gb0;
    const int cb0 = cs * p.cb_per_item, ncb = min(p.n_cb, cb0 + p.cb_per_item) - cb0;
    const int n_tiles = ng * ncb;
    const CUtensorMap* mz = head == 0 ? &map_z0 : (head == 1 ? &map_z1 : &map_z2);
    const CUtensorMap* mw = head == 0 ? &map_w0 : (head == 1 ? &map_w1 : &map_w2);
    const CUtensorMap* mdw = head == 0 ? &map_dw0 : (head == 1 ? &map_dw1 : &map_dw2);

    auto issue = [&](int t) {
      const int st = (T0 + t) % kStages;
      const int cb = cb0 + t / ng, gb = gb0 + t % ng;
      uint8_t* dst = s_st + st * kStage;
      mbar_expect_tx(&full[st], gather ? kStage - kZBytes : kStage);
      if (!gather) {
        tma_load_2d(dst, mz, gb * 128, cb * 128, &full[st]);
        tma_load_2d(dst + kZBytes / 2, mz, gb * 128 + 64, cb * 128, &full[st]);
      }
      if (DO_B) {
        if (WK) {
          tma_load_2d(dst + kZBytes, mw, gb * 128, 0, &full[st]);
          tma_load_2d(dst + kZBytes + kWBytes / 2, mw, gb * 128 + 64, 0, &full[st]);
        } else {
          tma_load_2d(dst + kZBytes, mw, 0, gb * 128, &full[st]);
        }
      }
      if (DO_A) tma_load_2d(dst + kZBytes + (DO_B ? kWBytes : 0), &map_h, 0, cb * 128, &full[st]);
    };
    auto load_rows = [&](int t) {
      const int cb = cb0 + t / ng;
#pragma unroll
      for (int i = 0; i < 8; ++i) {
        const int r = cb * 128 + g_r0 + 16 * i;
        src_row[i] = r < p.B ? __ldg(p.rows + r) : -1;
      }
    };
    auto copy_rows = [&](int t) {
      const int st = (T0 + t) % kStages, g0 = (gb0 + t % ng) * 128 + g_h * 64 + g_c * 8;
      const uint32_t gbytes = g0 < p.G ? (uint32_t)min(16, 2 * (p.G - g0)) : 0u;
      const uint32_t dst = smem_u32(s_st + st * kStage) + g_dst;
#pragma unroll
      for (int i = 0; i < 8; ++i) {
        const bool ok = src_row[i] >= 0 && gbytes != 0;
        cp_async_16(dst + i * 2048, ok ? p.zsrc + (int64_t)src_row[i] * p.ldz + g0 : p.zsrc, ok ? gbytes : 0u);
      }
      if (t + 1 < n_tiles) load_rows(t + 1);
    };
    if (gather) load_rows(0);
    for (int t = 0; t < kStages - 1; ++t) {
      if (t < n_tiles) {
        if (threadIdx.x == 0) issue(t);
        if (gather) copy_rows(t);
      }
      if (gather) cp_async_commit();
    }

    float acc_b[DO_B ? 32 : 1];
    float acc_a[DO_A ? MAXG : 1][32];
    float acc_c[COLSUM ? MAXG : 1][8];
#pragma unroll
    for (int j = 0; j < (DO_A ? MAXG : 1); ++j)
#pragma unroll
      for (int i = 0; i < 32; ++i) acc_a[j][i] = 0.f;
#pragma unroll
    for (int j = 0; j < (COLSUM ? MAXG : 1); ++j)
#pragma unroll
      for (int i = 0; i < 8; ++i) acc_c[j][i] = 0.f;

    int t = 0;
    for (int cbi = 0; cbi < ncb; ++cbi) {
      const int cb = cb0 + cbi;
#pragma unroll
      for (int i = 0; i < (DO_B ? 32 : 1); ++i) acc_b[i] = 0.f;
#pragma unroll
      for (int jj = 0; jj < (DO_A ? MAXG : 1); ++jj)
      for (int j = jj; j < (DO_A ? min(jj + 1, ng) : ng); ++j) {
        if (t + kStages - 1 < n_tiles) {
          if (threadIdx.x == 0) issue(t + kStages - 1);
          if (gather) copy_rows(t + kStages - 1);
        }
        if (gather) {
          cp_async_commit();
          cp_async_wait<kStages - 1>();
          fence_proxy_async_smem();
          __syncthreads();
        }
        const int st = (T0 + t) % kStages;
        mbar_wait(&full[st], ((T0 + t) / kStages) & 1);
        const uint32_t zb = smem_u32(s_st + st * kStage), wb = zb + kZBytes, hb = wb + (DO_B ? kWBytes : 0);
        wgmma_fence();
        if constexpr (DO_B) {
#pragma unroll
          for (int h = 0; h < 2; ++h)
#pragma unroll
            for (int k = 0; k < 4; ++k) {
              const uint64_t da = make_smem_desc(zb + h * (kZBytes / 2) + wg * 64 * 128 + k * 32, 0, 1024);
              if (WK) wgmma_m64n64k16<0, 0>(acc_b, da, make_smem_desc(wb + h * (kWBytes / 2) + k * 32, 0, 1024), 1u);
              else wgmma_m64n64k16<0, 1>(acc_b, da, make_smem_desc(wb + (h * 4 + k) * 2048, 0, 1024), 1u);
            }
        }
        if constexpr (DO_A) {
#pragma unroll
          for (int k = 0; k < 8; ++k) {
            const uint64_t da = make_smem_desc(zb + wg * (kZBytes / 2) + k * 2048, 0, 1024);
            wgmma_m64n64k16<1, 1>(acc_a[jj], da, make_smem_desc(hb + k * 2048, 0, 1024), 1u);
            if constexpr (COLSUM) wgmma_m64n16k16<1, 0>(acc_c[jj], da, make_smem_desc(smem_u32(s_ones) + (k & 3) * 32, 0, 1024), 1u);
          }
        }
        wgmma_commit();
        wgmma_wait<0>();
        if constexpr (DO_B) acc_fence(acc_b);
        if constexpr (DO_A) {
#pragma unroll
          for (int jj2 = 0; jj2 < MAXG; ++jj2) acc_fence(acc_a[jj2]);
        }
        if constexpr (COLSUM) {
#pragma unroll
          for (int jj2 = 0; jj2 < MAXG; ++jj2) acc_fence(acc_c[jj2]);
        }
        __syncthreads();
        ++t;
      }
      if constexpr (DO_B) {
        float* dst = p.part + (int64_t)(head * p.gene_ranges + gr) * p.part_stride + (int64_t)cb * 128 * 64;
#pragma unroll
        for (int i = 0; i < 32; i += 2) {
          const int row = wg * 64 + frow + 8 * ((i >> 1) & 1), col = 8 * (i >> 2) + fcol;
          *reinterpret_cast<float2*>(dst + row * 64 + col) = make_float2(acc_b[i], acc_b[i + 1]);
        }
      }
    }
    T0 += n_tiles;
    if constexpr (DO_A) {
#pragma unroll
      for (int j = 0; j < MAXG; ++j) {
        if (j >= ng) break;
        const int gb = gb0 + j;
        stage_begin();
        if (dw_transposed) {
#pragma unroll
          for (int i = 0; i < 32; ++i) {
            const int g = wg * 64 + frow + 8 * ((i >> 1) & 1), f = 8 * (i >> 2) + fcol + (i & 1);
            s_o[f * 128 + g] = acc_a[j][i];
          }
          stage_end(mdw, gb * 128, 0);
        } else {
#pragma unroll
          for (int i = 0; i < 32; i += 2) {
            const int g = wg * 64 + frow + 8 * ((i >> 1) & 1), f = 8 * (i >> 2) + fcol;
            *reinterpret_cast<float2*>(s_o + g * 64 + f) = make_float2(acc_a[j][i], acc_a[j][i + 1]);
          }
          stage_end(mdw, 0, gb * 128);
        }
        if constexpr (COLSUM) {
          float* dbh = head == 0 ? p.db[0] : (head == 1 ? p.db[1] : p.db[2]);
          if ((l & 3) == 0 && dbh) {
            const int g = gb * 128 + wg * 64 + frow;
            if (g < p.G) atomicAdd(dbh + g, acc_c[j][0]);
            if (g + 8 < p.G) atomicAdd(dbh + g + 8, acc_c[j][2]);
          }
        }
      }
    }
  }
  if (threadIdx.x == 0) bulk_wait<0>();
}

__global__ void gene_gemm_reduce_kernel(const float* __restrict__ part, int slots, int64_t stride, float* __restrict__ out,
                                        int64_t n) {
  const int64_t i = ((int64_t)blockIdx.x * blockDim.x + threadIdx.x) * 4;
  if (i >= n) return;
  float4 acc = *reinterpret_cast<const float4*>(out + i);
  for (int sl = 0; sl < slots; ++sl) {
    const float4 v = __ldcs(reinterpret_cast<const float4*>(part + sl * stride + i));
    acc.x += v.x; acc.y += v.y; acc.z += v.z; acc.w += v.w;
  }
  *reinterpret_cast<float4*>(out + i) = acc;
}

}

size_t gene_gemm_workspace_bytes(int B) { return sizeof(float) * (size_t)gg::kMaxSlots * cdiv(B, 128) * 128 * 64; }

int gene_gemm_tc(int mode, const __nv_bfloat16* const Z[3], int64_t ldz, const int32_t* rows, int B, int G, int n_heads,
                 const __nv_bfloat16* H, const __nv_bfloat16* const W[3], float* out_b, float* const dW[3], int64_t dW_ld,
                 int dW_transposed, float* const db[3], void* ws, size_t ws_bytes, int sm_count, cudaStream_t s) {
  using namespace gg;
  if (ldz % 8 != 0) { set_error("gene_gemm_tc: ldz must be a multiple of 8 (16-byte TMA stride)"); return DCA_ERR_BAD_ARG; }
  if (mode < 1 || mode > 3) { set_error("gene_gemm_tc: bad mode %d", mode); return DCA_ERR_BAD_ARG; }
  if (rows && (mode == 3 || n_heads != 1)) { set_error("gene_gemm_tc: row indices are for modes 1 and 2 (one Z)"); return DCA_ERR_BAD_ARG; }
  const bool do_a = mode & 2, do_b = mode & 1;
  if (do_b && (!ws || ws_bytes < gene_gemm_workspace_bytes(B))) { set_error("gene_gemm_tc: workspace too small"); return DCA_ERR_BAD_ARG; }
  CUtensorMap mz[3], mh, mw[3], mdw[3];
  for (int i = 0; i < 3; ++i) DCA_TRY(make_tensor_map_2d(&mz[i], Z[i < n_heads ? i : 0], 2, 1, (uint64_t)B, (uint64_t)G, (uint64_t)ldz, 128, 64, 1));
  mh = mz[0];
  for (int i = 0; i < 3; ++i) mw[i] = mdw[i] = mz[0];
  if (do_a) {
    DCA_TRY(make_tensor_map_2d(&mh, H, 2, 1, (uint64_t)B, 64, 64, 128, 64, 1));
    for (int i = 0; i < 3; ++i) {
      float* d = dW[i < n_heads ? i : 0];
      if (dW_transposed) DCA_TRY(make_tensor_map_2d(&mdw[i], d, 4, 0, 64, (uint64_t)G, (uint64_t)dW_ld, 64, 128, 0));
      else {
        if (dW_ld != 64) { set_error("gene_gemm_tc: non-transposed dW needs ld == 64"); return DCA_ERR_BAD_ARG; }
        DCA_TRY(make_tensor_map_2d(&mdw[i], d, 4, 0, (uint64_t)G, 64, 64, 128, 64, 0));
      }
    }
  }
  if (do_b) {
    for (int i = 0; i < 3; ++i) {
      const __nv_bfloat16* w = W[i < n_heads ? i : 0];
      if (mode == 3) DCA_TRY(make_tensor_map_2d(&mw[i], w, 2, 1, 64, (uint64_t)G, (uint64_t)G, 64, 64, 1));
      else DCA_TRY(make_tensor_map_2d(&mw[i], w, 2, 1, (uint64_t)G, 64, 64, 128, 64, 1));
    }
  }
  Params base{};
  base.B = B; base.G = G; base.n_heads = n_heads;
  base.n_cb = cdiv(B, 128); base.n_gb = cdiv(G, 128);
  for (int i = 0; i < 3; ++i) base.db[i] = db ? db[i] : nullptr;
  base.part = reinterpret_cast<float*>(ws); base.part_stride = (int64_t)base.n_cb * 128 * 64;
  base.rows = rows; base.zsrc = Z[0]; base.ldz = ldz;

#define DCA_GG_LAUNCH(P, A, Bb, Cc, WKk, MG)                                                                           \
  do {                                                                                                                 \
    static bool attr = false;                                                                                          \
    constexpr uint32_t sm = smem_bytes<A, Bb, Cc>();                                                                       \
    if (!attr) { DCA_CUDA_OK(cudaFuncSetAttribute(gene_gemm_kernel<A, Bb, Cc, WKk, MG>, cudaFuncAttributeMaxDynamicSharedMemorySize, (int)sm)); attr = true; } \
    gene_gemm_kernel<A, Bb, Cc, WKk, MG><<<min(P.total_items, sm_count), kThreads, sm, s>>>(mz[0], mz[1], mz[2], mh, mw[0], mw[1], mw[2],      \
                                                                          mdw[0], mdw[1], mdw[2], dW_transposed, P);  \
    DCA_LAUNCH_CHECK();                                                                                                \
  } while (0)

  if (do_a) {
    Params p = base;
    int best_gpi = 1; long long best_cost = -1;
    for (int gpi = 1; gpi <= kMaxGb; ++gpi) {
      const long long items = (long long)cdiv(p.n_gb, gpi) * n_heads, rounds = (items + sm_count - 1) / sm_count;
      const long long cost = rounds * ((long long)gpi * p.n_cb + 2ll * gpi);
      if (best_cost < 0 || cost < best_cost) { best_cost = cost; best_gpi = gpi; }
    }
    p.gb_per_item = best_gpi; p.gene_ranges = cdiv(p.n_gb, best_gpi);
    p.cb_per_item = p.n_cb; p.cell_splits = 1;
    p.total_items = p.gene_ranges * n_heads;
    if (mode == 3) DCA_GG_LAUNCH(p, true, false, true, false, kMaxGb);
    else DCA_GG_LAUNCH(p, true, false, false, false, kMaxGb);
  }
  if (do_b) {
    Params p = base;
    p.cb_per_item = 1; p.cell_splits = p.n_cb;
    int gsplits = cdiv(4 * sm_count, p.n_cb * n_heads); if (gsplits < 1) gsplits = 1;
    if (gsplits > kMaxSlots / n_heads) gsplits = kMaxSlots / n_heads;
    if (gsplits > p.n_gb) gsplits = p.n_gb;
    while (gsplits > 1 && cdiv(p.n_gb, gsplits) < 4) --gsplits;
    p.gb_per_item = cdiv(p.n_gb, gsplits); p.gene_ranges = cdiv(p.n_gb, p.gb_per_item);
    p.total_items = p.gene_ranges * p.cell_splits * n_heads;
    if (mode == 3) DCA_GG_LAUNCH(p, false, true, false, true, 1);
    else DCA_GG_LAUNCH(p, false, true, false, false, 1);
    const int64_t n = (int64_t)B * 64;
    gene_gemm_reduce_kernel<<<(unsigned)cdiv(n / 4, 256), 256, 0, s>>>(p.part, p.gene_ranges * n_heads, p.part_stride, out_b, n);
    DCA_LAUNCH_CHECK();
  }
#undef DCA_GG_LAUNCH
  return DCA_OK;
}

}
}

using namespace dca;
extern "C" int dca_tc_gene_gemm_rows(int32_t mode, const void* Z0, const void* Z1, const void* Z2, int64_t ldz,
                                     const int32_t* rows, int32_t batch, int32_t genes, int32_t n_heads, const void* H,
                                     const void* W, float* out_b, float* dW0, float* dW1, float* dW2, int64_t dW_ld,
                                     int32_t dW_transposed, float* db0, float* db1, float* db2, void* stream, int32_t sm_count) {
  if (!Z0 || batch <= 0 || genes <= 0 || n_heads < 1 || n_heads > 3) { set_error("dca_tc_gene_gemm: bad argument"); return DCA_ERR_BAD_ARG; }
  int dev = 0, sms = 132;
  cudaGetDevice(&dev);
  cudaDeviceGetAttribute(&sms, cudaDevAttrMultiProcessorCount, dev);
  if (sm_count > 0 && sm_count < sms) sms = sm_count;
  const __nv_bfloat16* Z[3] = {(const __nv_bfloat16*)Z0, (const __nv_bfloat16*)Z1, (const __nv_bfloat16*)Z2};
  float* dW[3] = {dW0, dW1, dW2};
  float* db[3] = {db0, db1, db2};
  const __nv_bfloat16* Wp[3];
  for (int i = 0; i < 3; ++i) Wp[i] = (const __nv_bfloat16*)W + (mode == 3 ? (size_t)(i < n_heads ? i : 0) * 64 * genes : 0);
  cudaStream_t st = (cudaStream_t)stream;
  const size_t ws_bytes = tc::gene_gemm_workspace_bytes(batch);
  void* ws = nullptr;
  DCA_CUDA_OK(cudaMallocAsync(&ws, ws_bytes, st));
  const int rc = tc::gene_gemm_tc(mode, Z, ldz, rows, batch, genes, n_heads, (const __nv_bfloat16*)H, Wp, out_b, dW,
                                  dW_ld, dW_transposed, db, ws, ws_bytes, sms, st);
  DCA_CUDA_OK(cudaFreeAsync(ws, st));
  return rc;
}
extern "C" int dca_tc_gene_gemm_sms(int32_t mode, const void* Z0, const void* Z1, const void* Z2, int64_t ldz,
                                    int32_t batch, int32_t genes, int32_t n_heads, const void* H, const void* W, float* out_b,
                                    float* dW0, float* dW1, float* dW2, int64_t dW_ld, int32_t dW_transposed, float* db0,
                                    float* db1, float* db2, void* stream, int32_t sm_count) {
  return dca_tc_gene_gemm_rows(mode, Z0, Z1, Z2, ldz, nullptr, batch, genes, n_heads, H, W, out_b, dW0, dW1, dW2, dW_ld,
                               dW_transposed, db0, db1, db2, stream, sm_count);
}
extern "C" int dca_tc_gene_gemm(int32_t mode, const void* Z0, const void* Z1, const void* Z2, int64_t ldz, int32_t batch,
                                int32_t genes, int32_t n_heads, const void* H, const void* W, float* out_b, float* dW0,
                                float* dW1, float* dW2, int64_t dW_ld, int32_t dW_transposed, float* db0, float* db1,
                                float* db2, void* stream) {
  return dca_tc_gene_gemm_sms(mode, Z0, Z1, Z2, ldz, batch, genes, n_heads, H, W, out_b, dW0, dW1, dW2, dW_ld,
                              dW_transposed, db0, db1, db2, stream, 0);
}
```

### dca_b200/csrc/tc_common.cuh

```cuda
#pragma once
#include <cuda.h>
#include <cuda_runtime.h>
#include <cuda_bf16.h>
#include <stdint.h>

namespace dca {
namespace tc {

__device__ __forceinline__ uint32_t smem_u32(const void* p) { return (uint32_t)__cvta_generic_to_shared(p); }

__device__ __forceinline__ void mbar_init(uint64_t* bar, uint32_t count) {
  asm volatile("mbarrier.init.shared::cta.b64 [%0], %1;" ::"r"(smem_u32(bar)), "r"(count));
}
__device__ __forceinline__ void fence_barrier_init() { asm volatile("fence.mbarrier_init.release.cluster;" ::: "memory"); }
__device__ __forceinline__ void mbar_expect_tx(uint64_t* bar, uint32_t bytes) {
  asm volatile("mbarrier.arrive.expect_tx.shared::cta.b64 _, [%0], %1;" ::"r"(smem_u32(bar)), "r"(bytes) : "memory");
}
__device__ __forceinline__ bool mbar_try_wait(uint64_t* bar, uint32_t parity) {
  uint32_t ok;
  asm volatile(
      "{\n\t.reg .pred p;\n\t"
      "mbarrier.try_wait.parity.shared::cta.b64 p, [%1], %2;\n\t"
      "selp.u32 %0, 1, 0, p;\n\t}"
      : "=r"(ok) : "r"(smem_u32(bar)), "r"(parity) : "memory");
  return ok != 0;
}
__device__ __forceinline__ void mbar_wait(uint64_t* bar, uint32_t parity) {
  uint32_t polls = 0;
  long long t0 = 0;
  while (!mbar_try_wait(bar, parity)) {
    if ((++polls & 0x3FFF) == 0) {
      const long long now = clock64();
      if (t0 == 0) t0 = now;
      else if (now - t0 > 4000000000ll) __trap();
    }
  }
}
__device__ __forceinline__ void mbar_arrive(uint64_t* bar) {
  asm volatile("mbarrier.arrive.shared::cta.b64 _, [%0];" ::"r"(smem_u32(bar)) : "memory");
}

__device__ __forceinline__ void mbar_wait_backoff(uint64_t* bar, uint32_t parity, uint32_t sleep_ns) {
  if (mbar_try_wait(bar, parity)) return;
  uint32_t polls = 0;
  long long t0 = 0;
  do {
    if (sleep_ns) __nanosleep(sleep_ns);
    if ((++polls & 0x3FFF) == 0) {
      const long long now = clock64();
      if (t0 == 0) t0 = now;
      else if (now - t0 > 4000000000ll) __trap();
    }
  } while (!mbar_try_wait(bar, parity));
}

__device__ __forceinline__ void fence_proxy_async_smem() { asm volatile("fence.proxy.async.shared::cta;" ::: "memory"); }
__device__ __forceinline__ void named_barrier_sync(uint32_t id, uint32_t nthreads) {
  asm volatile("bar.sync %0, %1;" ::"r"(id), "r"(nthreads) : "memory");
}

__device__ __forceinline__ void tma_prefetch_desc(const CUtensorMap* m) {
  asm volatile("prefetch.tensormap [%0];" ::"l"(reinterpret_cast<uint64_t>(m)) : "memory");
}
__device__ __forceinline__ void tma_load_2d(void* smem_dst, const CUtensorMap* m, int32_t c0, int32_t c1, uint64_t* bar) {
  asm volatile(
      "cp.async.bulk.tensor.2d.shared::cluster.global.mbarrier::complete_tx::bytes [%0], [%1, {%2, %3}], [%4];"
      ::"r"(smem_u32(smem_dst)), "l"(reinterpret_cast<uint64_t>(m)), "r"(c0), "r"(c1), "r"(smem_u32(bar)) : "memory");
}
__device__ __forceinline__ void tma_reduce_add_2d(const CUtensorMap* m, int32_t c0, int32_t c1, const void* smem_src) {
  asm volatile("cp.reduce.async.bulk.tensor.2d.global.shared::cta.add.tile.bulk_group [%0, {%1, %2}], [%3];"
               ::"l"(reinterpret_cast<uint64_t>(m)), "r"(c0), "r"(c1), "r"(smem_u32(smem_src)) : "memory");
}
__device__ __forceinline__ void bulk_commit() { asm volatile("cp.async.bulk.commit_group;" ::: "memory"); }
template <int N>
__device__ __forceinline__ void bulk_wait_read() { asm volatile("cp.async.bulk.wait_group.read %0;" ::"n"(N) : "memory"); }
template <int N>
__device__ __forceinline__ void bulk_wait() { asm volatile("cp.async.bulk.wait_group %0;" ::"n"(N) : "memory"); }

__device__ __forceinline__ uint64_t make_smem_desc(uint32_t smem_addr, uint32_t lbo_bytes, uint32_t sbo_bytes) {
  uint64_t d = 0;
  d |= (uint64_t)((smem_addr & 0x3FFFF) >> 4);
  d |= (uint64_t)((lbo_bytes >> 4) & 0x3FFF) << 16;
  d |= (uint64_t)((sbo_bytes >> 4) & 0x3FFF) << 32;
  d |= (uint64_t)1 << 62;
  return d;
}

__device__ __forceinline__ void wgmma_fence() { asm volatile("wgmma.fence.sync.aligned;" ::: "memory"); }
__device__ __forceinline__ void wgmma_commit() { asm volatile("wgmma.commit_group.sync.aligned;" ::: "memory"); }
template <int N>
__device__ __forceinline__ void wgmma_wait() { asm volatile("wgmma.wait_group.sync.aligned %0;" ::"n"(N) : "memory"); }

template <int TA, int TB>
__device__ __forceinline__ void wgmma_m64n16k16(float (&d)[8], uint64_t da, uint64_t db, uint32_t acc) {
  asm volatile(
      "{\n\t.reg .pred p;\n\tsetp.ne.b32 p, %10, 0;\n\t"
      "wgmma.mma_async.sync.aligned.m64n16k16.f32.bf16.bf16 {%0, %1, %2, %3, %4, %5, %6, %7},"
      " %8, %9, p, 1, 1, %11, %12;\n\t}"
      : "+f"(d[0]), "+f"(d[1]), "+f"(d[2]), "+f"(d[3]), "+f"(d[4]), "+f"(d[5]), "+f"(d[6]), "+f"(d[7])
      : "l"(da), "l"(db), "r"(acc), "n"(TA), "n"(TB));
}
template <int TA, int TB>
__device__ __forceinline__ void wgmma_m64n64k16(float (&d)[32], uint64_t da, uint64_t db, uint32_t acc) {
  asm volatile(
      "{\n\t.reg .pred p;\n\tsetp.ne.b32 p, %34, 0;\n\t"
      "wgmma.mma_async.sync.aligned.m64n64k16.f32.bf16.bf16 {"
      "%0, %1, %2, %3, %4, %5, %6, %7, %8, %9, %10, %11, %12, %13, %14, %15, "
      "%16, %17, %18, %19, %20, %21, %22, %23, %24, %25, %26, %27, %28, %29, %30, %31},"
      " %32, %33, p, 1, 1, %35, %36;\n\t}"
      : "+f"(d[0]), "+f"(d[1]), "+f"(d[2]), "+f"(d[3]), "+f"(d[4]), "+f"(d[5]), "+f"(d[6]), "+f"(d[7]), "+f"(d[8]), "+f"(d[9]), "+f"(d[10]), "+f"(d[11]), "+f"(d[12]), "+f"(d[13]), "+f"(d[14]), "+f"(d[15]), "+f"(d[16]), "+f"(d[17]), "+f"(d[18]), "+f"(d[19]), "+f"(d[20]), "+f"(d[21]), "+f"(d[22]), "+f"(d[23]), "+f"(d[24]), "+f"(d[25]), "+f"(d[26]), "+f"(d[27]), "+f"(d[28]), "+f"(d[29]), "+f"(d[30]), "+f"(d[31])
      : "l"(da), "l"(db), "r"(acc), "n"(TA), "n"(TB));
}
template <int TA, int TB>
__device__ __forceinline__ void wgmma_m64n128k16(float (&d)[64], uint64_t da, uint64_t db, uint32_t acc) {
  asm volatile(
      "{\n\t.reg .pred p;\n\tsetp.ne.b32 p, %66, 0;\n\t"
      "wgmma.mma_async.sync.aligned.m64n128k16.f32.bf16.bf16 {"
      "%0, %1, %2, %3, %4, %5, %6, %7, %8, %9, %10, %11, %12, %13, %14, %15, "
      "%16, %17, %18, %19, %20, %21, %22, %23, %24, %25, %26, %27, %28, %29, %30, %31, "
      "%32, %33, %34, %35, %36, %37, %38, %39, %40, %41, %42, %43, %44, %45, %46, %47, "
      "%48, %49, %50, %51, %52, %53, %54, %55, %56, %57, %58, %59, %60, %61, %62, %63},"
      " %64, %65, p, 1, 1, %67, %68;\n\t}"
      : "+f"(d[0]), "+f"(d[1]), "+f"(d[2]), "+f"(d[3]), "+f"(d[4]), "+f"(d[5]), "+f"(d[6]), "+f"(d[7]), "+f"(d[8]), "+f"(d[9]), "+f"(d[10]), "+f"(d[11]), "+f"(d[12]), "+f"(d[13]), "+f"(d[14]), "+f"(d[15]), "+f"(d[16]), "+f"(d[17]), "+f"(d[18]), "+f"(d[19]), "+f"(d[20]), "+f"(d[21]), "+f"(d[22]), "+f"(d[23]), "+f"(d[24]), "+f"(d[25]), "+f"(d[26]), "+f"(d[27]), "+f"(d[28]), "+f"(d[29]), "+f"(d[30]), "+f"(d[31]), "+f"(d[32]), "+f"(d[33]), "+f"(d[34]), "+f"(d[35]), "+f"(d[36]), "+f"(d[37]), "+f"(d[38]), "+f"(d[39]), "+f"(d[40]), "+f"(d[41]), "+f"(d[42]), "+f"(d[43]), "+f"(d[44]), "+f"(d[45]), "+f"(d[46]), "+f"(d[47]), "+f"(d[48]), "+f"(d[49]), "+f"(d[50]), "+f"(d[51]), "+f"(d[52]), "+f"(d[53]), "+f"(d[54]), "+f"(d[55]), "+f"(d[56]), "+f"(d[57]), "+f"(d[58]), "+f"(d[59]), "+f"(d[60]), "+f"(d[61]), "+f"(d[62]), "+f"(d[63])
      : "l"(da), "l"(db), "r"(acc), "n"(TA), "n"(TB));
}

template <int R>
__device__ __forceinline__ void acc_fence(float (&d)[R]) {
#pragma unroll
  for (int i = 0; i < R; ++i) asm volatile("" : "+f"(d[i])::"memory");
}

__device__ __forceinline__ bool elect_one() {
  uint32_t pred = 0;
  asm volatile("{\n\t.reg .pred px;\n\telect.sync _|px, 0xFFFFFFFF;\n\tselp.u32 %0, 1, 0, px;\n\t}" : "=r"(pred));
  return pred != 0;
}

__device__ __forceinline__ float ex2f(float x) { float y; asm("ex2.approx.ftz.f32 %0, %1;" : "=f"(y) : "f"(x)); return y; }
__device__ __forceinline__ float lg2f(float x) { float y; asm("lg2.approx.ftz.f32 %0, %1;" : "=f"(y) : "f"(x)); return y; }
__device__ __forceinline__ float rcpf(float x) { float y; asm("rcp.approx.ftz.f32 %0, %1;" : "=f"(y) : "f"(x)); return y; }

int make_tensor_map_2d(CUtensorMap* out, const void* base, int elem_bytes, int is_bf16, uint64_t rows, uint64_t cols,
                       uint64_t ld_elems, uint32_t box_rows, uint32_t box_cols, int swizzle);

}
}
```

### dca_b200/csrc/zinb_loss.cu

```cuda
#include "dca_internal.cuh"
#include <string>
#include "zinb_math.cuh"
#include "tc_common.cuh"
#include "head_act.cuh"
#include <cstdlib>

namespace dca {
namespace tc { extern int g_gg_profile; }

namespace {

constexpr int kThreads = 256;
constexpr int kVec = 4;
constexpr int kColsPerBlock = kThreads * kVec;
constexpr int kMaxBlocks = 65536;

struct LossTune { int target_blocks; unsigned producer_sleep_ns, consumer_sleep_ns; int branch_free; int ring; };
LossTune g_tune = {0 , 0u, 0u, 1 ,
                   1 };

int sm_count_cached() {
  static int n = 0;
  if (!n) { int dev = 0; if (cudaGetDevice(&dev) != cudaSuccess || cudaDeviceGetAttribute(&n, cudaDevAttrMultiProcessorCount, dev) != cudaSuccess || n <= 0) n = 132; }
  return n;
// ... 464 lines not shown
    isnz[j] = active && !(y[j] < 1e-8f);
    const unsigned bal = __ballot_sync(kFull, isnz[j]);
    pos[j] = base + __popc(bal & lt); base += __popc(bal);
  }
  const int total = base;
#pragma unroll
  for (int j = 0; j < kVec; ++j)
    if (isnz[j]) q[pos[j]] = make_float4(y[j], mu[j], dd[j], pp[j]);
  __syncwarp();
  refill();
  const float m_lo = fminf(fminf(vm.x, vm.y), fminf(vm.z, vm.w)), m_hi = fmaxf(fmaxf(vm.x, vm.y), fmaxf(vm.z, vm.w));
  const float d_lo = fminf(fminf(dd[0], dd[1]), fminf(dd[2], dd[3])), d_hi = fmaxf(fmaxf(dd[0], dd[1]), fmaxf(dd[2], dd[3]));
  const bool plain = (m_lo > 1e-5f) && (m_hi < 1e6f) &&
                     (COND_DISP ? (d_lo > 0.03125f) && (d_hi < 1e4f) : (d_hi <= 1e6f));
  Raw2 zA, zB; Fin2 fA, fB;
  if (__all_sync(kFull, plain)) {
    zA = zinb_zero_pair<Ops, true>(muA, dA, pA); zB = zinb_zero_pair<Ops, true>(muB, dB, pB);
    fA = finish_factors_pair_plain<Ops, COND_DISP>(dA, pA, inv_n); fB = finish_factors_pair_plain<Ops, COND_DISP>(dB, pB, inv_n);
  } else {
    zA = zinb_zero_pair<Ops>(muA, dA, pA); zB = zinb_zero_pair<Ops>(muB, dB, pB);
    fA = finish_factors_pair<Ops, COND_DISP>(mA, dA, pA, inv_n); fB = finish_factors_pair<Ops, COND_DISP>(mB, dB, pB, inv_n);
  }
  lsum_lg += ((active && !isnz[0]) ? zA.lgD.x : 0.f) + ((active && !isnz[1]) ? zA.lgD.y : 0.f)
           + ((active && !isnz[2]) ? zB.lgD.x : 0.f) + ((active && !isnz[3]) ? zB.lgD.y : 0.f);
  for (int k = lane; k < total; k += 32) {
    const float4 it = q[k];
    const Raw1 e = zinb_nb_raw<Ops>(it.x, it.y, it.z, it.w, lf);
    lsum_nb += e.loss;
    q[k] = make_float4(e.gmu, e.dth, e.dpi, 0.f);
  }
  __syncwarp();
  if (isnz[0]) { const float4 e = q[pos[0]]; zA.gmu.x = e.x; zA.dth.x = e.y; zA.dpi.x = e.z; }
  if (isnz[1]) { const float4 e = q[pos[1]]; zA.gmu.y = e.x; zA.dth.y = e.y; zA.dpi.y = e.z; }
  if (isnz[2]) { const float4 e = q[pos[2]]; zB.gmu.x = e.x; zB.dth.x = e.y; zB.dpi.x = e.z; }
  if (isnz[3]) { const float4 e = q[pos[3]]; zB.gmu.y = e.x; zB.dth.y = e.y; zB.dpi.y = e.z; }
  __syncwarp();
  if (ridge != 0.f) {
    if (active) lsum_r += ridge * (pA.x * pA.x + pA.y * pA.y + pB.x * pB.x + pB.y * pB.y);
    zA.dpi = fma2(splat(2.0f * ridge), pA, zA.dpi); zB.dpi = fma2(splat(2.0f * ridge), pB, zB.dpi);
  }
  if (!COND_DISP && active) { tacc[0] += zA.dth.x; tacc[1] += zA.dth.y; tacc[2] += zB.dth.x; tacc[3] += zB.dth.y; }
  RowGrads g;
  g.gmA = mul2(zA.gmu, fA.fm); g.gmB = mul2(zB.gmu, fB.fm);
  g.gdA = mul2(zA.dth, fA.fd); g.gdB = mul2(zB.dth, fB.fd);
  g.gpA = mul2(zA.dpi, fA.fp); g.gpB = mul2(zB.dpi, fB.fp);
  return g;
}

template <int NT>
__device__ __forceinline__ void block_loss_fold(double dsum, double* red, int* s_last, double* __restrict__ loss_partial,
                                                const FoldArgs& fa, float inv_n) {
  constexpr unsigned kFull = 0xffffffffu;
  constexpr int kWarps = NT / 32;
  const int warp = threadIdx.x >> 5, lane = threadIdx.x & 31;
#pragma unroll
  for (int o = 16; o > 0; o >>= 1) dsum += __shfl_xor_sync(kFull, dsum, o);
  if (lane == 0) red[warp] = dsum;
  __syncthreads();
  if (threadIdx.x == 0) {
    double t = 0.0;
#pragma unroll
    for (int w = 0; w < kWarps; ++w) t += red[w];
    loss_partial[blockIdx.y * gridDim.x + blockIdx.x] = t;
    __threadfence();
    const unsigned nblk = gridDim.x * gridDim.y;
    const unsigned done = atomicAdd(fa.counter, 1u);
    *s_last = (done == nblk - 1);
    if (*s_last) *fa.counter = 0;
  }
  __syncthreads();
  if (!*s_last) return;
  __threadfence();
  const int n = gridDim.x * gridDim.y;
  double a = 0.0;
  for (int i = threadIdx.x; i < n; i += NT) a += __ldcg(loss_partial + i);
#pragma unroll
  for (int o = 16; o > 0; o >>= 1) a += __shfl_xor_sync(kFull, a, o);
  __syncthreads();
  if (lane == 0) red[warp] = a;
  __syncthreads();
  if (threadIdx.x == 0) {
    double t = 0.0;
#pragma unroll
    for (int w = 0; w < kWarps; ++w) t += red[w];
    *fa.loss_sum = t;
    if (fa.loss_slot) {
      double l = t * (double)inv_n;
      if (l != l) l = INFINITY;
      if (fa.penalty) l += *fa.penalty;
      const float lf32 = (float)l;
      fa.loss_slot[0] = lf32;
      fa.loss_slot[1] = (isfinite(lf32)) ? 0.f : 1.f;
      if (fa.epoch_acc) { fa.epoch_acc[0] += l * (double)fa.batch; fa.epoch_acc[1] += (double)fa.batch; }
    }
  }
}

template <bool COND_DISP, typename GT, bool IDXQ>
__global__ void __launch_bounds__(kThreads, 3)
zinb_loss_bwd_ring_kernel(const float* __restrict__ Y, int64_t ldy, const int32_t* __restrict__ rows,
                          const float* __restrict__ sf, const float* m, const float* d, const float* pi,
                          int64_t ld, int B, int G, float ridge, float inv_n, int rows_per_block,
                          GT* dzm, GT* dzd, GT* dzp, float* __restrict__ dth_acc,
                          double* __restrict__ loss_partial, const float* __restrict__ lf_global, const FoldArgs fa) {
  extern __shared__ __align__(128) unsigned char smem_ring[];
  constexpr int kWarps = kThreads / 32;
  constexpr int kArrays = COND_DISP ? 4 : 3;
  constexpr uint32_t kSegBytes = kThreads * 16;
  constexpr uint32_t kSlotBytes = kArrays * kSegBytes;
  constexpr int RING = IDXQ ? kRing + 1 : kRing;
  float4* items = reinterpret_cast<float4*>(smem_ring + RING * kSlotBytes);
  __shared__ double red[kWarps];
  __shared__ float lf[zmath::kLogFactN];
  __shared__ float s_sf[kMaxRowsPerBlock];
  __shared__ int s_row[kMaxRowsPerBlock];
  __shared__ int s_last;

  using Ops = zmath::FastOps;
  using namespace zmath;
  constexpr unsigned kFull = 0xffffffffu;
  const int warp = threadIdx.x >> 5, lane = threadIdx.x & 31;
  const int c0 = blockIdx.x * kColsPerBlock;
  const bool active = c0 + (int)threadIdx.x * kVec < G;
  const int col = active ? (int)threadIdx.x * kVec : (G - c0 - kVec);
  const int r0 = blockIdx.y * rows_per_block;
  const int nrows = min(rows_per_block, B - r0);
  if (threadIdx.x < kLogFactN) lf[threadIdx.x] = lf_global[threadIdx.x];
  for (int t = threadIdx.x; t < nrows; t += kThreads) {
    const int yr = rows ? rows[r0 + t] : (r0 + t);
    s_row[t] = yr;
    s_sf[t] = sf ? sf[yr] : 1.0f;
  }
  __syncthreads();

  const uint32_t my = tc::smem_u32(smem_ring) + threadIdx.x * 16;
  const uint32_t ring_end = my + RING * kSlotBytes;
  const float* ysrc = Y + c0 + col;
  const float* msrc = m + (int64_t)r0 * ld + c0 + col;
  const float* dsrc = COND_DISP ? d + (int64_t)r0 * ld + c0 + col : nullptr;
  const float* psrc = pi + (int64_t)r0 * ld + c0 + col;
  const uint32_t ldy32 = (uint32_t)ldy;
  int nxt = 0;
  uint32_t wslot = my;
  auto cp16 = [](uint32_t dst, const void* src) {
    asm volatile("cp.async.cg.shared.global [%0], [%1], 16;" ::"r"(dst), "l"(src) : "memory");
  };
  auto issue_next = [&]() {
    cp16(wslot, ysrc + (uint64_t)((uint32_t)s_row[nxt]) * ldy32);
    cp16(wslot + kSegBytes, msrc);
    if (COND_DISP) cp16(wslot + 2 * kSegBytes, dsrc);
    cp16(wslot + (kArrays - 1) * kSegBytes, psrc);
    msrc += ld; psrc += ld;
    if (COND_DISP) dsrc += ld;
    ++nxt; wslot += kSlotBytes;
    if (wslot == ring_end) wslot = my;
  };

  float lsum_lg = 0.f, lsum_nb = 0.f, lsum_r = 0.f;
  float tacc[kVec] = {0.f, 0.f, 0.f, 0.f};
  {
#pragma unroll
    for (int i = 0; i < RING; ++i) {
      if (i < nrows) issue_next();
      cp_async_commit();
    }
    float4* q = items + warp * (32 * kVec);
    unsigned char* qb = reinterpret_cast<unsigned char*>(items) + warp * (32 * kVec);
    auto lds32 = [](uint32_t addr) { float v; asm volatile("ld.shared.f32 %0, [%1];" : "=f"(v) : "r"(addr) : "memory"); return v; };
    auto sts32 = [](uint32_t addr, float v) { asm volatile("st.shared.f32 [%0], %1;" ::"r"(addr), "f"(v) : "memory"); };
    float thg[kVec] = {1.f, 1.f, 1.f, 1.f};
    if (!COND_DISP) {
#pragma unroll
      for (int j = 0; j < kVec; ++j) thg[j] = d[c0 + col + j];
    }
    const unsigned lt = (1u << lane) - 1u;
    GT* om = dzm + (int64_t)r0 * ld + c0 + col;
    GT* od = COND_DISP ? dzd + (int64_t)r0 * ld + c0 + col : nullptr;
    GT* op = dzp + (int64_t)r0 * ld + c0 + col;
    uint32_t rslot = my;
    auto lds128 = [](uint32_t addr) {
      float4 v;
      asm volatile("ld.shared.v4.f32 {%0,%1,%2,%3}, [%4];" : "=f"(v.x), "=f"(v.y), "=f"(v.z), "=f"(v.w) : "r"(addr) : "memory");
      return v;
    };
    for (int i = 0; i < nrows; ++i) {
      cp_async_wait<RING - 1>();
      const uint32_t cslot = rslot, wstrip = rslot - (uint32_t)lane * 16u;
      const float4 vy = lds128(rslot), vm = lds128(rslot + kSegBytes);
      const float4 vd = COND_DISP ? lds128(rslot + 2 * kSegBytes) : make_float4(thg[0], thg[1], thg[2], thg[3]);
      const float4 vp = lds128(rslot + (kArrays - 1) * kSegBytes);
      rslot += kSlotBytes;
      if (rslot == ring_end) rslot = my;
      const float row_sf = s_sf[i];
      if constexpr (!IDXQ) {
        const RowGrads g = zinb_row_ring<COND_DISP>(vy, vm, vd, vp, row_sf, active, ridge, inv_n, q, lf, lsum_lg, lsum_nb,
                                                    lsum_r, tacc, [&] { if (nxt < nrows) issue_next(); cp_async_commit(); });
        if (active) {
          st4(om, g.gmA.x, g.gmA.y, g.gmB.x, g.gmB.y);
          if (COND_DISP) st4(od, g.gdA.x, g.gdA.y, g.gdB.x, g.gdB.y);
          st4(op, g.gpA.x, g.gpA.y, g.gpB.x, g.gpB.y);
        }
      } else {
      const float y[kVec] = {vy.x, vy.y, vy.z, vy.w};
      const float2 mA = make_float2(vm.x, vm.y), mB = make_float2(vm.z, vm.w);
      const float2 dA = make_float2(vd.x, vd.y), dB = make_float2(vd.z, vd.w);
      const float2 pA = make_float2(vp.x, vp.y), pB = make_float2(vp.z, vp.w);
      const float2 muA = mul2(mA, splat(row_sf)), muB = mul2(mB, splat(row_sf));
      const float dd[kVec] = {dA.x, dA.y, dB.x, dB.y};
      bool isnz[kVec];
      int pos[kVec], base = 0;
#pragma unroll
      for (int j = 0; j < kVec; ++j) {
        isnz[j] = active && !(y[j] < 1e-8f);
        const unsigned bal = __ballot_sync(kFull, isnz[j]);
        pos[j] = base + __popc(bal & lt); base += __popc(bal);
      }
      const int total = base;
#pragma unroll
      for (int j = 0; j < kVec; ++j)
        if (isnz[j]) qb[pos[j]] = (unsigned char)(lane * kVec + j);
      __syncwarp();
      const float m_lo = fminf(fminf(vm.x, vm.y), fminf(vm.z, vm.w)), m_hi = fmaxf(fmaxf(vm.x, vm.y), fmaxf(vm.z, vm.w));
      const float d_lo = fminf(fminf(dd[0], dd[1]), fminf(dd[2], dd[3])), d_hi = fmaxf(fmaxf(dd[0], dd[1]), fmaxf(dd[2], dd[3]));
      const bool plain = (m_lo > 1e-5f) && (m_hi < 1e6f) &&
                         (COND_DISP ? (d_lo > 0.03125f) && (d_hi < 1e4f) : (d_hi <= 1e6f));
      Raw2 zA, zB; Fin2 fA, fB;
      if (__all_sync(kFull, plain)) {
        zA = zinb_zero_pair<Ops, true>(muA, dA, pA); zB = zinb_zero_pair<Ops, true>(muB, dB, pB);
        fA = finish_factors_pair_plain<Ops, COND_DISP>(dA, pA, inv_n); fB = finish_factors_pair_plain<Ops, COND_DISP>(dB, pB, inv_n);
      } else {
        zA = zinb_zero_pair<Ops>(muA, dA, pA); zB = zinb_zero_pair<Ops>(muB, dB, pB);
        fA = finish_factors_pair<Ops, COND_DISP>(mA, dA, pA, inv_n); fB = finish_factors_pair<Ops, COND_DISP>(mB, dB, pB, inv_n);
      }
      lsum_lg += ((active && !isnz[0]) ? zA.lgD.x : 0.f) + ((active && !isnz[1]) ? zA.lgD.y : 0.f)
               + ((active && !isnz[2]) ? zB.lgD.x : 0.f) + ((active && !isnz[3]) ? zB.lgD.y : 0.f);
      for (int k = lane; k < total; k += 32) {
        const int idx = qb[k];
        const uint32_t e4 = wstrip + (uint32_t)idx * 4u;
        const float th = COND_DISP ? lds32(e4 + 2 * kSegBytes) : __ldg(d + c0 + warp * (32 * kVec) + idx);
        const Raw1 e = zinb_nb_raw<Ops>(lds32(e4), lds32(e4 + kSegBytes) * row_sf, th, lds32(e4 + (kArrays - 1) * kSegBytes), lf);
        lsum_nb += e.loss;
        sts32(e4, e.gmu); sts32(e4 + kSegBytes, e.dth); sts32(e4 + (kArrays - 1) * kSegBytes, e.dpi);
      }
      __syncwarp();
      const float4 r0v = lds128(cslot), r1v = lds128(cslot + kSegBytes), r2v = lds128(cslot + (kArrays - 1) * kSegBytes);
      zA.gmu.x = isnz[0] ? r0v.x : zA.gmu.x; zA.dth.x = isnz[0] ? r1v.x : zA.dth.x; zA.dpi.x = isnz[0] ? r2v.x : zA.dpi.x;
      zA.gmu.y = isnz[1] ? r0v.y : zA.gmu.y; zA.dth.y = isnz[1] ? r1v.y : zA.dth.y; zA.dpi.y = isnz[1] ? r2v.y : zA.dpi.y;
      zB.gmu.x = isnz[2] ? r0v.z : zB.gmu.x; zB.dth.x = isnz[2] ? r1v.z : zB.dth.x; zB.dpi.x = isnz[2] ? r2v.z : zB.dpi.x;
      zB.gmu.y = isnz[3] ? r0v.w : zB.gmu.y; zB.dth.y = isnz[3] ? r1v.w : zB.dth.y; zB.dpi.y = isnz[3] ? r2v.w : zB.dpi.y;
      __syncwarp();
      if (nxt < nrows) issue_next();
      cp_async_commit();
      if (ridge != 0.f) {
        if (active) lsum_r += ridge * (pA.x * pA.x + pA.y * pA.y + pB.x * pB.x + pB.y * pB.y);
        zA.dpi = fma2(splat(2.0f * ridge), pA, zA.dpi); zB.dpi = fma2(splat(2.0f * ridge), pB, zB.dpi);
      }
      if (active) {
        if (!COND_DISP) { tacc[0] += zA.dth.x; tacc[1] += zA.dth.y; tacc[2] += zB.dth.x; tacc[3] += zB.dth.y; }
        const float2 gmA = mul2(zA.gmu, fA.fm), gmB = mul2(zB.gmu, fB.fm);
        const float2 gpA = mul2(zA.dpi, fA.fp), gpB = mul2(zB.dpi, fB.fp);
        st4(om, gmA.x, gmA.y, gmB.x, gmB.y);
        if (COND_DISP) {
          const float2 gdA = mul2(zA.dth, fA.fd), gdB = mul2(zB.dth, fB.fd);
          st4(od, gdA.x, gdA.y, gdB.x, gdB.y);
        }
        st4(op, gpA.x, gpA.y, gpB.x, gpB.y);
      }
      }
      om += ld; op += ld;
      if (COND_DISP) od += ld;
    }
    if (!COND_DISP && active) {
#pragma unroll
      for (int j = 0; j < kVec; ++j) atomicAdd(dth_acc + c0 + col + j, tacc[j]);
    }
  }
  block_loss_fold<kThreads>((double)lsum_nb + (double)lsum_r - (double)kLn2 * (double)lsum_lg,
                            red, &s_last, loss_partial, fa, inv_n);
}

namespace hl {
constexpr int kWG = 4;
constexpr int kCtaThreads = 128 * kWG;
constexpr int kRows = 4;
constexpr int kPieces = 16 / kRows;
constexpr uint32_t kWHeadBytes = 64 * 128 * 2;
constexpr uint32_t kHBytes = 64 * 64 * 2;
constexpr uint32_t kRowBytes = 3 * 128 * 4;
constexpr uint32_t kQPad = 512;
constexpr uint32_t kOffY = kQPad + kRows * kRowBytes;
constexpr uint32_t kWarpBytes = kOffY + kRows * 128 * 4;
constexpr uint32_t kOffH = 3 * kWHeadBytes;
constexpr uint32_t kOffStage = kOffH + kWG * kHBytes;
constexpr uint32_t kOffBias = kOffStage + kWG * 4 * kWarpBytes;
constexpr uint32_t kSmemBytes = kOffBias + 3 * 128 * 4 + 1024;
static_assert(kSmemBytes + 1024 <= 227 * 1024, "heads_loss_kernel: dynamic + 1 KB static shared memory over the sm_90 limit");

struct Params {
  const float* bias[3];
  const float* Y; int64_t ldy; const int32_t* rows; const float* sf;
  int B, G, nblk, units;
  float ridge, inv_n;
  __nv_bfloat16* dz[3]; int64_t ldz;
  double* loss_partial; const float* lf;
};

__device__ __forceinline__ uint32_t slot16(int i, int k) { return (uint32_t)((i ^ ((2 * k) & 6)) * 16); }

__device__ __forceinline__ void stage_acc(const float (&acc)[64], int piece, uint8_t* head_base) {
  const int lane = threadIdx.x & 31, k = (lane >> 2) & 3;
  if ((lane >> 4) != (piece & 1)) return;
  const bool hi = piece >= 2;
  uint8_t* dst = head_base + k * kRowBytes + (lane & 1) * 8;
#pragma unroll
  for (int c = 0; c < 16; ++c) {
    const int g = 8 * c + 2 * (lane & 3);
    *reinterpret_cast<float2*>(dst + slot16(g >> 2, k)) =
        make_float2(hi ? acc[4 * c + 2] : acc[4 * c], hi ? acc[4 * c + 3] : acc[4 * c + 1]);
  }
}

template <int KIND>
__device__ __forceinline__ float4 head_out4(const float4 a, const float4 b) {
  return make_float4(tc::head_out<KIND>(a.x, b.x, 1.0f), tc::head_out<KIND>(a.y, b.y, 1.0f),
                     tc::head_out<KIND>(a.z, b.z, 1.0f), tc::head_out<KIND>(a.w, b.w, 1.0f));
}
}

__global__ void __launch_bounds__(hl::kCtaThreads, 1)
heads_loss_kernel(const __grid_constant__ CUtensorMap map_h, const __grid_constant__ CUtensorMap map_w0,
                  const __grid_constant__ CUtensorMap map_w1, const __grid_constant__ CUtensorMap map_w2, const hl::Params p,
                  const FoldArgs fa) {
  using namespace hl;
  using namespace tc;
  extern __shared__ __align__(1024) uint8_t smem_hl_raw[];
  uint8_t* smem = smem_hl_raw + ((1024u - (smem_u32(smem_hl_raw) & 1023u)) & 1023u);
  __shared__ uint64_t w_bar, h_bar[kWG];
  __shared__ float lf[zmath::kLogFactN];
  __shared__ double red[kCtaThreads / 32];
  __shared__ int s_last;
  const int tid = threadIdx.x, wg = tid >> 7, warp = (tid >> 5) & 3, lane = tid & 31;
  float* s_bias = reinterpret_cast<float*>(smem + kOffBias);
  uint8_t* h_buf = smem + kOffH + wg * kHBytes;
  uint8_t* wbase = smem + kOffStage + (wg * 4 + warp) * kWarpBytes;
  uint8_t* rows_base = wbase + kQPad;
  const uint32_t my_y = smem_u32(wbase + kOffY) + lane * 16;
  if (tid < zmath::kLogFactN) lf[tid] = p.lf[tid];
  if (tid == 0) {
    mbar_init(&w_bar, 1);
    for (int g = 0; g < kWG; ++g) mbar_init(&h_bar[g], 1);
    fence_barrier_init();
  }
  __syncthreads();
  const CUtensorMap* mw[3] = {&map_w0, &map_w1, &map_w2};
  auto load_h = [&](int blk) {
    if ((tid & 127) == 0) { mbar_expect_tx(&h_bar[wg], kHBytes); tma_load_2d(h_buf, &map_h, 0, blk * 64, &h_bar[wg]); }
  };
  const int u0 = (int)((long long)blockIdx.x * p.units / gridDim.x), u1 = (int)((long long)(blockIdx.x + 1) * p.units / gridDim.x);
  uint32_t w_phase = 0, h_phase = 0;
  float lsum_lg = 0.f, lsum_nb = 0.f, lsum_r = 0.f;
  float tacc[kVec] = {0.f, 0.f, 0.f, 0.f};
  for (int u = u0; u < u1;) {
    const int t = u / p.nblk;
    const int seg_end = min(u1, (t + 1) * p.nblk);
    const int b_end = seg_end - t * p.nblk;
    int blk = u - t * p.nblk + wg;
    __syncthreads();
    if (tid == 0) {
      mbar_expect_tx(&w_bar, 3 * kWHeadBytes);
      for (int h = 0; h < 3; ++h) {
        tma_load_2d(smem + h * kWHeadBytes, mw[h], t * 128, 0, &w_bar);
        tma_load_2d(smem + h * kWHeadBytes + kWHeadBytes / 2, mw[h], t * 128 + 64, 0, &w_bar);
      }
    }
    if (tid < 3 * 128) {
      const int gcol = t * 128 + (tid & 127);
      const float* bias = wg == 0 ? p.bias[0] : (wg == 1 ? p.bias[1] : p.bias[2]);
      s_bias[tid] = gcol < p.G ? bias[gcol] : 0.f;
    }
    if (blk < b_end) load_h(blk);
    __syncthreads();
    mbar_wait(&w_bar, w_phase); w_phase ^= 1;
    const int gvalid = min(128, p.G - t * 128);
    const bool active = 4 * lane < gvalid;
    const int col = active ? 4 * lane : gvalid - kVec;
    const int64_t gcol0 = (int64_t)t * 128 + col;
    for (; blk < b_end; blk += kWG) {
      mbar_wait(&h_bar[wg], h_phase); h_phase ^= 1;
      for (int piece = 0; piece < kPieces; ++piece) {
        const int r0 = blk * 64 + warp * 16 + piece * kRows;
        int my_yr = 0; float my_sf = 1.f;
        if (lane < kRows && r0 + lane < p.B) {
          my_yr = p.rows ? p.rows[r0 + lane] : r0 + lane;
          my_sf = p.sf ? p.sf[my_yr] : 1.0f;
        }
        float acc[64];
        head_tile_mma(acc, smem_u32(h_buf), smem_u32(smem));
        stage_acc(acc, piece, rows_base);
#pragma unroll
        for (int k = 0; k < kRows; ++k) {
          const int yr = __shfl_sync(0xffffffffu, my_yr, k);
          if (r0 + k < p.B)
            asm volatile("cp.async.cg.shared.global [%0], [%1], 16;" ::"r"(my_y + k * 512), "l"(p.Y + (int64_t)yr * p.ldy + gcol0)
                         : "memory");
        }
        cp_async_commit();
        head_tile_mma(acc, smem_u32(h_buf), smem_u32(smem) + kWHeadBytes);
        stage_acc(acc, piece, rows_base + 512);
        head_tile_mma(acc, smem_u32(h_buf), smem_u32(smem) + 2 * kWHeadBytes);
        if (piece == kPieces - 1) {
          named_barrier_sync(1 + wg, 128);
          if (blk + kWG < b_end) load_h(blk + kWG);
        }
        stage_acc(acc, piece, rows_base + 1024);
        cp_async_wait<0>();
        __syncwarp();
        for (int k = 0; k < kRows; ++k) {
          const int r = r0 + k;
          if (r >= p.B) break;
          float4 vy;
          asm volatile("ld.shared.v4.f32 {%0,%1,%2,%3}, [%4];" : "=f"(vy.x), "=f"(vy.y), "=f"(vy.z), "=f"(vy.w) : "r"(my_y + k * 512)
                       : "memory");
          const float row_sf = __shfl_sync(0xffffffffu, my_sf, k);
          const uint8_t* src = rows_base + k * kRowBytes + slot16(col >> 2, k);
          const float4 am = *reinterpret_cast<const float4*>(src);
          const float4 ad = *reinterpret_cast<const float4*>(src + 512);
          const float4 ap = *reinterpret_cast<const float4*>(src + 1024);
          __syncwarp();
          const float4 vm = head_out4<EPI_MEAN_ACT>(am, *reinterpret_cast<const float4*>(s_bias + col));
          const float4 vd = head_out4<EPI_DISP_ACT>(ad, *reinterpret_cast<const float4*>(s_bias + 128 + col));
          const float4 vp = head_out4<EPI_SIGMOID>(ap, *reinterpret_cast<const float4*>(s_bias + 256 + col));
          float4* q = reinterpret_cast<float4*>(wbase + k * kRowBytes);
          const RowGrads g = zinb_row_ring<true>(vy, vm, vd, vp, row_sf, active, p.ridge, p.inv_n, q, lf, lsum_lg, lsum_nb,
                                                 lsum_r, tacc, [] {});
          if (active) {
            const int64_t off = (int64_t)r * p.ldz + gcol0;
            st4(p.dz[0] + off, g.gmA.x, g.gmA.y, g.gmB.x, g.gmB.y);
            st4(p.dz[1] + off, g.gdA.x, g.gdA.y, g.gdB.x, g.gdB.y);
            st4(p.dz[2] + off, g.gpA.x, g.gpA.y, g.gpB.x, g.gpB.y);
          }
        }
      }
    }
    u = seg_end;
  }
  block_loss_fold<kCtaThreads>((double)lsum_nb + (double)lsum_r - (double)zmath::kLn2 * (double)lsum_lg, red, &s_last,
                            p.loss_partial, fa, p.inv_n);
}

__global__ void fold_partials_kernel(const double* __restrict__ part, int n, double* out, int accumulate,
                                     const double* penalty, float inv_n, int batch, float* loss_slot, double* epoch_acc) {
  __shared__ double sm[32];
  double a = 0.0;
  for (int i = threadIdx.x; i < n; i += blockDim.x) a += part[i];
#pragma unroll
  for (int o = 16; o > 0; o >>= 1) a += __shfl_xor_sync(0xffffffffu, a, o);
  if ((threadIdx.x & 31) == 0) sm[threadIdx.x >> 5] = a;
  __syncthreads();
  if (threadIdx.x < 32) {
    a = (threadIdx.x < (blockDim.x >> 5)) ? sm[threadIdx.x] : 0.0;
#pragma unroll
    for (int o = 16; o > 0; o >>= 1) a += __shfl_xor_sync(0xffffffffu, a, o);
    if (threadIdx.x == 0) {
      *out = accumulate ? (*out + a) : a;
      if (loss_slot) {
        double l = a * (double)inv_n;
        if (l != l) l = INFINITY;
        if (penalty) l += *penalty;
        const float lf = (float)l;
        loss_slot[0] = lf;
        loss_slot[1] = (isfinite(lf)) ? 0.f : 1.f;
        if (epoch_acc) { epoch_acc[0] += l * (double)batch; epoch_acc[1] += (double)batch; }
      }
    }
  }
}

__device__ float g_log_fact[zmath::kLogFactN];

const float* log_fact_table_device() {
  static thread_local int ready_dev = -1;
  static thread_local float* cached = nullptr;
  int dev = 0;
  if (cudaGetDevice(&dev) != cudaSuccess) { set_error("cudaGetDevice failed"); return nullptr; }
  if (ready_dev == dev && cached) return cached;
  float* p = nullptr;
  if (cudaGetSymbolAddress((void**)&p, g_log_fact) != cudaSuccess) { set_error("cudaGetSymbolAddress failed"); return nullptr; }
  cached = p;
  if (ready_dev != dev) {
    float t[zmath::kLogFactN];
    zmath::fill_log_fact(t);
    if (cudaMemcpy(p, t, sizeof(t), cudaMemcpyHostToDevice) != cudaSuccess) { set_error("log-factorial table upload failed"); return nullptr; }
    ready_dev = dev;
  }
  return p;
}

template <bool BWD>
int launch(const LossArgs& a, cudaStream_t s) {
  if (a.B <= 0 || a.G <= 0) { set_error("zinb_loss: empty batch (B=%d, G=%d)", a.B, a.G); return DCA_ERR_BAD_ARG; }
  const bool has_pi = (a.ae_type == DCA_AE_ZINB_CONDDISP || a.ae_type == DCA_AE_ZINB);
  const bool cond = (a.ae_type == DCA_AE_ZINB_CONDDISP || a.ae_type == DCA_AE_NB_CONDDISP);
  if (!a.Y || !a.m || !a.d || (has_pi && !a.pi) || !a.loss_sum) { set_error("zinb_loss: null input"); return DCA_ERR_BAD_ARG; }
  if (BWD && (!a.dzm || (cond && !a.dzd) || (has_pi && !a.dzp) || (!cond && !a.dtheta))) {
    set_error("zinb_loss: null gradient output"); return DCA_ERR_BAD_ARG;
  }
  const float* lf_dev = log_fact_table_device();
  if (!lf_dev) return DCA_ERR_CUDA;
  const size_t need = loss_workspace_bytes(a.B, a.G);
  if (!a.ws || a.ws_bytes < need) { set_error("zinb_loss: workspace too small (%zu < %zu)", a.ws_bytes, need); return DCA_ERR_BAD_ARG; }
  double* lpart = reinterpret_cast<double*>(a.ws);
  auto al16 = [](const void* q) { return (reinterpret_cast<uintptr_t>(q) & 15) == 0; };
  bool vec = (a.G % 4 == 0) && (a.ld % 4 == 0) && (a.ldy % 4 == 0) && al16(a.Y) && al16(a.m) && (!cond || al16(a.d)) &&
             (!has_pi || al16(a.pi));
  if (BWD) vec = vec && al16(a.dzm) && (!cond || al16(a.dzd)) && (!has_pi || al16(a.dzp));
  const Plan p = make_plan(a.B, a.G, vec ? kColsPerBlock : kThreads);
  dim3 grid(p.col_blocks, p.row_chunks), block(kThreads);
  float* tpart = a.dtheta;
  if (BWD && !cond) DCA_CUDA_OK(cudaMemsetAsync(a.dtheta, 0, sizeof(float) * (size_t)a.G, s));

  static const bool use_compact = [] { const char* e = getenv("DCA_LOSS_KERNEL"); return e && e[0] == 'c'; }();
  const Plan ps = make_plan(a.B, a.G, kColsPerBlock, kMaxRowsPerBlock);
  const bool staged_ok = BWD && vec && has_pi && !use_compact && (long long)ps.row_chunks * ps.col_blocks <= kMaxBlocks &&
                         ps.row_chunks <= 65535;
  if (staged_ok) {
    grid = dim3(ps.col_blocks, ps.row_chunks);
    FoldArgs fa{reinterpret_cast<unsigned*>(reinterpret_cast<char*>(a.ws) + sizeof(double) * (size_t)kMaxBlocks), a.loss_sum,
                a.fin_penalty, a.fin_loss_slot, a.fin_epoch_acc, a.fin_batch};
    if (!a.counter_ready) DCA_CUDA_OK(cudaMemsetAsync(fa.counter, 0, sizeof(unsigned), s));
#define DCA_RING2(CD, GT, IQ)                                                                                     \
  do {                                                                                                             \
    constexpr size_t sm = IQ ? (size_t)(kRing + 1) * (CD ? 4 : 3) * kColsPerBlock * 4 + (size_t)(kThreads / 32) * 32 * kVec     \
                             : (size_t)kRing * (CD ? 4 : 3) * kColsPerBlock * 4 + (size_t)(kThreads / 32) * 32 * kVec * 16; \
    static bool attr = false;                                                                                      \
    if (!attr) { DCA_CUDA_OK(cudaFuncSetAttribute(zinb_loss_bwd_ring_kernel<CD, GT, IQ>, cudaFuncAttributeMaxDynamicSharedMemorySize, (int)sm)); attr = true; } \
    zinb_loss_bwd_ring_kernel<CD, GT, IQ><<<grid, kThreads, sm, s>>>(a.Y, a.ldy, a.rows, a.sf, a.m, a.d, a.pi, a.ld, a.B, a.G, a.ridge, \
        a.inv_n, ps.rows_per_block, (GT*)a.dzm, (GT*)a.dzd, (GT*)a.dzp, tpart, lpart, lf_dev, fa);                  \
  } while (0)
#define DCA_RING(CD, GT) do { if (g_tune.ring == 2) DCA_RING2(CD, GT, true); else DCA_RING2(CD, GT, false); } while (0)
    if (g_tune.ring) {
      if (a.grad_bf16) { if (cond) DCA_RING(true, __nv_bfloat16); else DCA_RING(false, __nv_bfloat16); }
      else             { if (cond) DCA_RING(true, float); else DCA_RING(false, float); }
      DCA_LAUNCH_CHECK();
      return DCA_OK;
    }
#undef DCA_RING
#undef DCA_RING2
#define DCA_STAGED2(CD, GT, BFV)                                                                                   \
  do {                                                                                                             \
    constexpr size_t sm = (size_t)kStageRows * (CD ? 4 : 3) * kColsPerBlock * 4 + (size_t)(kThreads / 32) * 32 * kVec * 16; \
    static bool attr = false;                                                                                      \
    if (!attr) { DCA_CUDA_OK(cudaFuncSetAttribute(zinb_loss_bwd_staged_kernel<CD, GT, BFV>, cudaFuncAttributeMaxDynamicSharedMemorySize, (int)sm)); attr = true; } \
    zinb_loss_bwd_staged_kernel<CD, GT, BFV><<<grid, kStagedThreads, sm, s>>>(a.Y, a.ldy, a.rows, a.sf, a.m, a.d, a.pi, a.ld, a.B, \
        a.G, a.ridge, a.inv_n, ps.rows_per_block, (GT*)a.dzm, (GT*)a.dzd, (GT*)a.dzp, tpart, lpart, lf_dev, fa,     \
        g_tune.producer_sleep_ns, g_tune.consumer_sleep_ns);                                                       \
  } while (0)
#define DCA_STAGED(CD, GT) do { if (g_tune.branch_free) DCA_STAGED2(CD, GT, true); else DCA_STAGED2(CD, GT, false); } while (0)
    if (a.grad_bf16) { if (cond) DCA_STAGED(true, __nv_bfloat16); else DCA_STAGED(false, __nv_bfloat16); }
    else             { if (cond) DCA_STAGED(true, float); else DCA_STAGED(false, float); }
#undef DCA_STAGED2
#undef DCA_STAGED
    DCA_LAUNCH_CHECK();
    return DCA_OK;
  } else if (BWD && vec && has_pi) {
#define DCA_COMPACT(CD, GT)                                                                                   \
  zinb_loss_bwd_compact_kernel<CD, GT><<<grid, block, 0, s>>>(a.Y, a.ldy, a.rows, a.sf, a.m, a.d, a.pi, a.ld, a.B, a.G, \
                                                              a.ridge, a.inv_n, p.rows_per_block, (GT*)a.dzm,  \
                                                              (GT*)a.dzd, (GT*)a.dzp, tpart, lpart, lf_dev)
    if (a.grad_bf16) { if (cond) DCA_COMPACT(true, __nv_bfloat16); else DCA_COMPACT(false, __nv_bfloat16); }
    else             { if (cond) DCA_COMPACT(true, float); else DCA_COMPACT(false, float); }
#undef DCA_COMPACT
  } else {
#define DCA_LOSS_LAUNCH(HP, CD, GT, V)                                                                 \
  zinb_loss_kernel<HP, CD, GT, V, BWD><<<grid, block, 0, s>>>(                                          \
      a.Y, a.ldy, a.rows, a.sf, a.m, a.d, a.pi, a.ld, a.B, a.G, a.ridge, a.inv_n, p.rows_per_block,      \
      (GT*)a.dzm, (GT*)a.dzd, (GT*)a.dzp, tpart, lpart, lf_dev)
#define DCA_LOSS_DISPATCH(GT, V)                                   \
  do {                                                             \
    if (has_pi && cond) DCA_LOSS_LAUNCH(true, true, GT, V);        \
    else if (has_pi && !cond) DCA_LOSS_LAUNCH(true, false, GT, V); \
    else if (!has_pi && cond) DCA_LOSS_LAUNCH(false, true, GT, V); \
    else DCA_LOSS_LAUNCH(false, false, GT, V);                     \
  } while (0)
    if (BWD && a.grad_bf16) {
      if (vec) DCA_LOSS_DISPATCH(__nv_bfloat16, 4); else DCA_LOSS_DISPATCH(__nv_bfloat16, 1);
    } else {
      if (vec) DCA_LOSS_DISPATCH(float, 4); else DCA_LOSS_DISPATCH(float, 1);
    }
#undef DCA_LOSS_DISPATCH
#undef DCA_LOSS_LAUNCH
  }
  DCA_LAUNCH_CHECK();
  fold_partials_kernel<<<1, 256, 0, s>>>(lpart, (int)(grid.x * grid.y), a.loss_sum, BWD ? 0 : 1, a.fin_penalty, a.inv_n,
                                         a.fin_batch, BWD ? a.fin_loss_slot : nullptr, a.fin_epoch_acc);
  DCA_LAUNCH_CHECK();
  return DCA_OK;
}

}

const float* loss_log_fact_table() { return log_fact_table_device(); }
int g_fused_heads_default = 0;

size_t loss_workspace_bytes(int B, int G) {
  (void)B; (void)G;
  return sizeof(double) * (size_t)kMaxBlocks + 256;
}

int zinb_loss_fwd_bwd(const LossArgs& a, cudaStream_t s) { return launch<true>(a, s); }
int zinb_loss_fwd(const LossArgs& a, cudaStream_t s) { return launch<false>(a, s); }

int heads_loss_tc(const HeadsLossArgs& a, cudaStream_t s) {
  using namespace hl;
  const int B = a.B, G = a.G;
  auto al = [](const void* q, uintptr_t n) { return (reinterpret_cast<uintptr_t>(q) & (n - 1)) == 0; };
  if (B <= 0 || G <= 0 || G % 8 != 0 || a.ldy % 4 != 0 || !al(a.Y, 16) || a.ldz % 4 != 0 || a.ldz < G ||
      !al(a.dz[0], 8) || !al(a.dz[1], 8) || !al(a.dz[2], 8)) {
    set_error("heads_loss_tc: need G %% 8 == 0, a 16-byte aligned Y with ldy %% 4 == 0 and 8-byte aligned dZ with ldz %% 4 == 0 (>= G)");
    return DCA_ERR_BAD_ARG;
  }
  const float* lf_dev = log_fact_table_device();
  if (!lf_dev) return DCA_ERR_CUDA;
  if (!a.ws || a.ws_bytes < loss_workspace_bytes(B, G)) { set_error("heads_loss_tc: workspace too small"); return DCA_ERR_BAD_ARG; }
  CUtensorMap mh, mw[3];
  DCA_TRY(tc::make_tensor_map_2d(&mh, a.H3, 2, 1, (uint64_t)B, 64, 64, 64, 64, 1));
  for (int i = 0; i < 3; ++i) DCA_TRY(tc::make_tensor_map_2d(&mw[i], a.W[i], 2, 1, 64, (uint64_t)G, (uint64_t)G, 64, 64, 1));
  Params p;
  for (int i = 0; i < 3; ++i) { p.bias[i] = a.bias[i]; p.dz[i] = a.dz[i]; }
  p.Y = a.Y; p.ldy = a.ldy; p.rows = a.rows; p.sf = a.sf; p.B = B; p.G = G; p.ldz = a.ldz;
  p.nblk = cdiv(B, 64);
  const long long units = (long long)cdiv(G, 128) * p.nblk;
  if (units > INT_MAX) { set_error("heads_loss_tc: %lld (gene tile, cell block) units, over 2^31 - 1", units); return DCA_ERR_BAD_ARG; }
  p.units = (int)units;
  p.ridge = a.ridge; p.inv_n = a.inv_n;
  p.loss_partial = reinterpret_cast<double*>(a.ws); p.lf = lf_dev;
  FoldArgs fa{reinterpret_cast<unsigned*>(reinterpret_cast<char*>(a.ws) + sizeof(double) * (size_t)kMaxBlocks), a.loss_sum,
              a.fin_penalty, a.fin_loss_slot, a.fin_epoch_acc, a.fin_batch};
  if (!a.counter_ready) DCA_CUDA_OK(cudaMemsetAsync(fa.counter, 0, sizeof(unsigned), s));
  static bool attr = false;
  if (!attr) { DCA_CUDA_OK(cudaFuncSetAttribute(heads_loss_kernel, cudaFuncAttributeMaxDynamicSharedMemorySize, (int)kSmemBytes)); attr = true; }
  const int grid = (int)std::min<long long>(p.units, sm_count_cached());
  heads_loss_kernel<<<grid, kCtaThreads, kSmemBytes, s>>>(mh, mw[0], mw[1], mw[2], p, fa);
  DCA_LAUNCH_CHECK();
  return DCA_OK;
}

}

using namespace dca;

extern "C" int dca_set_tunable(const char* name, int64_t value) {
  if (!name) { set_error("dca_set_tunable: null name"); return DCA_ERR_BAD_ARG; }
  const std::string n(name);
  if (n == "loss_target_blocks" && value >= 0 && value <= kMaxBlocks) g_tune.target_blocks = (int)value;
  else if (n == "loss_producer_sleep_ns" && value >= 0 && value <= 100000) g_tune.producer_sleep_ns = (unsigned)value;
  else if (n == "loss_consumer_sleep_ns" && value >= 0 && value <= 100000) g_tune.consumer_sleep_ns = (unsigned)value;
  else if (n == "fused_heads" && (value == 0 || value == 1)) g_fused_heads_default = (int)value;
  else if (n == "loss_branch_free" && (value == 0 || value == 1)) g_tune.branch_free = (int)value;
  else if (n == "loss_ring" && value >= 0 && value <= 2) g_tune.ring = (int)value;
  else if (n == "gg_profile" && (value == 0 || value == 1)) tc::g_gg_profile = (int)value;
  else { set_error("dca_set_tunable: unknown name or value out of range (%s = %lld)", name, (long long)value); return DCA_ERR_BAD_ARG; }
  return DCA_OK;
}

extern "C" int dca_zinb_loss_workspace_bytes(int32_t batch, int32_t genes, size_t* bytes) {
  if (!bytes || batch <= 0 || genes <= 0) { set_error("dca_zinb_loss_workspace_bytes: bad argument"); return DCA_ERR_BAD_ARG; }
  *bytes = loss_workspace_bytes(batch, genes);
  return DCA_OK;
}

extern "C" int dca_zinb_loss_fwd_bwd(const float* Y, int64_t ldy, const int32_t* rows, const float* sf,
                                     const float* m, const float* d, const float* pi, int64_t ld,
                                     int32_t batch, int32_t genes, int32_t ae_type, float ridge, float inv_n,
                                     void* dzm, void* dzd, void* dzp, int32_t grad_dtype, float* dtheta,
                                     double* loss_sum, void* workspace, size_t workspace_bytes, void* stream) {
  if (ae_type < 0 || ae_type > 3) { set_error("dca_zinb_loss_fwd_bwd: unknown ae_type %d", ae_type); return DCA_ERR_BAD_ARG; }
  LossArgs a{Y, ldy, rows, sf, m, d, pi, ld, batch, genes, ae_type, ridge, inv_n, dzm, dzd, dzp,
             grad_dtype == DCA_BF16 ? 1 : 0, dtheta, loss_sum, workspace, workspace_bytes};
  return zinb_loss_fwd_bwd(a, (cudaStream_t)stream);
}

extern "C" int dca_tc_heads_loss(const void* Hb, int32_t batch, const void* Wk, const float* bias, int32_t genes,
                                 const float* Y, int64_t ldy, const int32_t* rows, const float* sf, float ridge, float inv_n,
                                 void* dzm, void* dzd, void* dzp, int64_t ldz, double* loss_sum, void* workspace,
                                 size_t workspace_bytes, void* stream) {
  if (!Hb || !Wk || !bias || !Y || !dzm || !dzd || !dzp || !loss_sum || batch <= 0 || genes <= 0) {
    set_error("dca_tc_heads_loss: bad argument"); return DCA_ERR_BAD_ARG;
  }
  HeadsLossArgs a{};
  a.H3 = (const __nv_bfloat16*)Hb; a.B = batch; a.G = genes;
  for (int i = 0; i < 3; ++i) { a.W[i] = (const __nv_bfloat16*)Wk + (size_t)i * 64 * genes; a.bias[i] = bias + (size_t)i * genes; }
  a.Y = Y; a.ldy = ldy; a.rows = rows; a.sf = sf; a.ridge = ridge; a.inv_n = inv_n;
  a.dz[0] = (__nv_bfloat16*)dzm; a.dz[1] = (__nv_bfloat16*)dzd; a.dz[2] = (__nv_bfloat16*)dzp; a.ldz = ldz;
  a.loss_sum = loss_sum; a.ws = workspace; a.ws_bytes = workspace_bytes;
  return heads_loss_tc(a, (cudaStream_t)stream);
}

extern "C" int dca_zinb_loss_fwd(const float* Y, int64_t ldy, const int32_t* rows, const float* sf,
                                 const float* m, const float* d, const float* pi, int64_t ld, int32_t batch,
                                 int32_t genes, int32_t ae_type, float ridge, double* loss_sum, void* workspace,
                                 size_t workspace_bytes, void* stream) {
  if (ae_type < 0 || ae_type > 3) { set_error("dca_zinb_loss_fwd: unknown ae_type %d", ae_type); return DCA_ERR_BAD_ARG; }
  LossArgs a{Y, ldy, rows, sf, m, d, pi, ld, batch, genes, ae_type, ridge, 1.0f, nullptr, nullptr, nullptr,
             0, nullptr, loss_sum, workspace, workspace_bytes};
  return zinb_loss_fwd(a, (cudaStream_t)stream);
}

extern "C" int dca_zinb_elem_host(int32_t ae_type, float y, float m, float sf, float d, float pi, float ridge,
                                  float out[4]) {
  zmath::Elem e;
  static float lf[zmath::kLogFactN];
  static bool lf_ready = false;
  if (!lf_ready) { zmath::fill_log_fact(lf); lf_ready = true; }
  using P = zmath::PreciseOps;
  if (ae_type & 0x200) {
    const int base = ae_type & 0xff;
    if (base != DCA_AE_ZINB_CONDDISP && base != DCA_AE_ZINB) { set_error("dca_zinb_elem_host: kernel variant needs a ZINB type"); return DCA_ERR_BAD_ARG; }
    const bool cd = base == DCA_AE_ZINB_CONDDISP;
    const float2 m2 = zmath::splat(m), d2 = zmath::splat(d), p2 = zmath::splat(pi), mu2 = zmath::mul2(m2, zmath::splat(sf));
    const zmath::Fin2 f = cd ? zmath::finish_factors_pair<P, true>(m2, d2, p2, 1.0f) : zmath::finish_factors_pair<P, false>(m2, d2, p2, 1.0f);
    float loss, gmu, dth, dpi;
    if (y < 1e-8f) {
      const zmath::Raw2 z = zmath::zinb_zero_pair<P>(mu2, d2, p2);
      loss = -zmath::kLn2 * z.lgD.y; gmu = z.gmu.y; dth = z.dth.y; dpi = z.dpi.y;
    } else {
      const zmath::Raw1 r = zmath::zinb_nb_raw<P>(y, mu2.x, d, pi, lf);
      loss = r.loss; gmu = r.gmu; dth = r.dth; dpi = r.dpi;
    }
    if (ridge != 0.f) { loss += ridge * pi * pi; dpi = fmaf(2.0f * ridge, pi, dpi); }
    out[0] = loss; out[1] = gmu * f.fm.y; out[2] = dth * f.fd.y; out[3] = dpi * f.fp.y;
    return DCA_OK;
  }
  if (ae_type & 0x100) {
    const int base = ae_type & 0xff;
    if (base != DCA_AE_ZINB_CONDDISP && base != DCA_AE_ZINB) { set_error("dca_zinb_elem_host: kernel variant needs a ZINB type"); return DCA_ERR_BAD_ARG; }
    if (y < 1e-8f) {
      e = base == DCA_AE_ZINB_CONDDISP ? zmath::zinb_elem_zero_bf<P, true>(m, sf, d, pi, ridge)
                                       : zmath::zinb_elem_zero_bf<P, false>(m, sf, d, pi, ridge);
    } else if (base == DCA_AE_ZINB_CONDDISP) {
      e = zmath::zinb_elem_nb_mu<P>(y, m * sf, d, pi, ridge, lf);
      if (!(m > 1e-5f && m < 1e6f)) e.gm = 0.f;
    } else {
      e = zmath::zinb_elem<P, true, false>(y, m, sf, d, pi, ridge, lf);
    }
    out[0] = e.loss; out[1] = e.gm; out[2] = e.gd; out[3] = e.gp;
    return DCA_OK;
  }
  switch (ae_type) {
    case DCA_AE_ZINB_CONDDISP: e = zmath::zinb_elem<P, true, true>(y, m, sf, d, pi, ridge, lf); break;
    case DCA_AE_ZINB: e = zmath::zinb_elem<P, true, false>(y, m, sf, d, pi, ridge, lf); break;
    case DCA_AE_NB_CONDDISP: e = zmath::zinb_elem<P, false, true>(y, m, sf, d, pi, ridge, lf); break;
    case DCA_AE_NB: e = zmath::zinb_elem<P, false, false>(y, m, sf, d, pi, ridge, lf); break;
    default: set_error("dca_zinb_elem_host: unknown ae_type %d", ae_type); return DCA_ERR_BAD_ARG;
  }
  out[0] = e.loss; out[1] = e.gm; out[2] = e.gd; out[3] = e.gp;
  return DCA_OK;
}
```

### include/dca_b200.h

```cpp
#ifndef DCA_B200_H
#define DCA_B200_H

#include <stddef.h>
#include <stdint.h>

#ifdef __cplusplus
extern "C" {
#endif

#define DCA_B200_VERSION 100
#define DCA_MAX_HIDDEN 8
#define DCA_NAME_LEN 48

typedef enum dca_status {
  DCA_OK = 0,
  DCA_ERR_BAD_ARG = -1,
  DCA_ERR_CUDA = -2,
  DCA_ERR_UNSUPPORTED = -3,
  DCA_ERR_NONFINITE = -4,
  DCA_ERR_NO_DEVICE = -5
} dca_status;

typedef enum dca_ae_type {
  DCA_AE_ZINB_CONDDISP = 0,
  DCA_AE_ZINB = 1,
  DCA_AE_NB_CONDDISP = 2,
  DCA_AE_NB = 3,
  DCA_AE_POISSON = 4,
  DCA_AE_NORMAL = 5,
  DCA_AE_NB_SHARED = 6,
  DCA_AE_ZINB_SHARED = 7,
  DCA_AE_ZINB_ELEMPI = 8,
  DCA_AE_NB_FORK = 9,
  DCA_AE_ZINB_FORK = 10
} dca_ae_type;

typedef enum dca_activation {
  DCA_ACT_RELU = 0,
  DCA_ACT_LINEAR = 1,
  DCA_ACT_ELU = 2,
  DCA_ACT_SELU = 3,
  DCA_ACT_TANH = 4,
  DCA_ACT_SIGMOID = 5,
  DCA_ACT_HARD_SIGMOID = 6,
  DCA_ACT_SOFTPLUS = 7,
  DCA_ACT_SOFTSIGN = 8,
  DCA_ACT_EXPONENTIAL = 9,
  DCA_ACT_LEAKY_RELU = 10,
  DCA_ACT_PRELU = 11
} dca_activation;

typedef enum dca_dtype { DCA_F32 = 0, DCA_BF16 = 1 } dca_dtype;

typedef enum dca_gemm_path {
  DCA_GEMM_AUTO = 0,
  DCA_GEMM_GENERIC = 1,
  DCA_GEMM_TCGEN05 = 2
} dca_gemm_path;

typedef enum dca_region_id {
  DCA_REGION_PARAMS = 0,
  DCA_REGION_GRADS = 1,
  DCA_REGION_RMS = 2,
  DCA_REGION_BN_STATE = 3,
  DCA_REGION_EPOCH_ACC = 4
} dca_region_id;

typedef struct dca_config {
  int32_t struct_bytes;
  int32_t n_in;
  int32_t n_out;
  int32_t n_hidden;
  int32_t hidden[DCA_MAX_HIDDEN];
  int32_t ae_type;
  int32_t batchnorm;
  int32_t max_batch;
  int32_t x_dtype;
  int32_t gemm_path;
  float ridge;
  float l1, l2, l1_enc, l2_enc;
  float bn_momentum, bn_eps;
  float rms_rho, rms_eps;
  int32_t elempi_shared;
  int32_t sync_bn;
  int32_t activation;
  float input_dropout;
  float hidden_dropout[DCA_MAX_HIDDEN];
  uint64_t dropout_seed;
} dca_config;

typedef struct dca_handle dca_handle;

typedef struct dca_tensor_info {
  char name[DCA_NAME_LEN];
  int64_t offset;
  int32_t rows, cols;
} dca_tensor_info;

int dca_version(void);
const char* dca_last_error(void);
void dca_config_default(dca_config* cfg);

int dca_arena_bytes(const dca_config* cfg, size_t* bytes);
int dca_create(const dca_config* cfg, void* arena, size_t arena_bytes, dca_handle** out);
int dca_destroy(dca_handle* h);

int dca_param_count(const dca_handle* h, int64_t* n_params, int32_t* n_tensors);
int dca_param_info(const dca_handle* h, int32_t index, dca_tensor_info* info);
int dca_state_count(const dca_handle* h, int64_t* n_state, int32_t* n_tensors);
int dca_state_info(const dca_handle* h, int32_t index, dca_tensor_info* info);
int dca_region(dca_handle* h, int32_t region_id, void** dev_ptr, int64_t* count);

int dca_init_params(dca_handle* h, uint64_t seed, void* stream);
int dca_params_changed(dca_handle* h, void* stream);

int dca_train_step(dca_handle* h, const void* X, int64_t ldx, const float* Y, int64_t ldy,
                   const float* sf, const int32_t* rows, int32_t batch, void* stream);

int dca_train_step_phase(dca_handle* h, const void* X, int64_t ldx, const float* Y, int64_t ldy,
                         const float* sf, const int32_t* rows, int32_t batch, int32_t phase, void* stream);
int dca_grad_buckets(const dca_handle* h, int64_t* head_bucket_offset);

int dca_comm_unique_id(void* id128);
int dca_comm_init(dca_handle* h, const void* id128, int32_t rank, int32_t world);
int dca_comm_destroy(dca_handle* h);
int dca_allreduce(dca_handle* h, void* stream);
int dca_train_step_dp(dca_handle* h, const void* X, int64_t ldx, const float* Y, int64_t ldy,
                      const float* sf, const int32_t* rows, int32_t batch, void* stream);

typedef enum dca_optimizer {
  DCA_OPT_RMSPROP = 0, DCA_OPT_SGD = 1, DCA_OPT_ADAGRAD = 2, DCA_OPT_ADADELTA = 3, DCA_OPT_ADAM = 4, DCA_OPT_ADAMAX = 5,
  DCA_OPT_NADAM = 6
} dca_optimizer;
int dca_set_optimizer(dca_handle* h, int32_t optimizer, void* stream);
int dca_reset_optimizer(dca_handle* h, void* stream);

int dca_apply_update(dca_handle* h, float lr, float clip, float grad_scale, void* stream);

int dca_eval_step(dca_handle* h, const void* X, int64_t ldx, const float* Y, int64_t ldy,
                  const float* sf, const int32_t* rows, int32_t batch, void* stream);

int dca_predict(dca_handle* h, const void* X, int64_t ldx, const float* sf, const int32_t* rows,
                int32_t batch, float* mean_out, float* disp_out, float* pi_out, int64_t ld_out,
                float* latent_out, void* stream);

int dca_read_loss(dca_handle* h, float* loss_host, int32_t* nonfinite_host, void* stream);
int dca_read_epoch_acc(dca_handle* h, double acc_host[4], int32_t reset, void* stream);

int dca_set_loss_ring(dca_handle* h, float* host_ring, int32_t n_slots);

int dca_train_step_host(dca_handle* h, const void* x_host, const float* y_host,
                        const float* sf_host, int32_t batch, float lr, float clip,
                        float* loss_host, void* stream);

int dca_set_input_transform(dca_handle* h, const float* gene_mean_host, const float* gene_inv_std_host,
                            int32_t use_size_factors, int32_t use_log1p, void* stream);
int dca_stream_begin(dca_handle* h, const uint16_t* counts_host, int64_t ld_counts, const float* sf_host,
                     int64_t n_rows, int32_t batch, void* stream);
int dca_stream_begin_packed(dca_handle* h, const void* packed_host, int32_t bits, int64_t row_bytes,
                            const int64_t* ovf_indptr_host, const void* ovf_entries_host, const float* sf_host,
                            int64_t n_rows, int32_t batch, void* stream);
int dca_stream_begin_sparse(dca_handle* h, const void* bitmap_host, const int64_t* nib_indptr_host, const void* nibbles_host,
                            const int64_t* ovf_indptr_host, const void* ovf_entries_host, const float* sf_host,
                            int64_t n_rows, int32_t batch, void* stream);
int dca_stream_step(dca_handle* h, int64_t batch_index, int64_t next_batch_index , void* stream);
int dca_stream_end(dca_handle* h, void* stream);
int dca_set_input_transform_exact(dca_handle* h, const double* gene_mean_host, const double* gene_std_host, double median,
                                  int32_t flags, void* stream);
int dca_stream_row_totals(dca_handle* h, const double* n_counts_host);
int dca_stream_predict(dca_handle* h, int64_t batch_index, int64_t next_batch_index, float* mean_out, float* disp_out,
                       float* pi_out, int64_t ld_out, float* latent_out, void* stream);
int dca_stream_eval(dca_handle* h, int64_t batch_index, int64_t next_batch_index, void* stream);
int dca_stream_capacity(const dca_handle* h, int64_t* ovf_entries, int64_t* nibble_bytes);
int dca_expand_packed_counts(const void* packed, int32_t bits, const int64_t* ovf_indptr, const void* ovf_entries,
                             const float* sf, int32_t n_rows, int32_t genes, const float* gene_mean,
                             const float* gene_inv_std, int32_t use_size_factors, int32_t use_log1p,
                             float* Y, void* X, int32_t x_dtype, float* sf_out, void* stream);
int dca_expand_sparse_counts(const void* bitmap, const int64_t* nib_indptr, const void* nibbles,
                             int32_t max_row_nibble_bytes, const int64_t* ovf_indptr, const void* ovf_entries,
                             const float* sf, int32_t n_rows, int32_t genes, const float* gene_mean,
                             const float* gene_inv_std, int32_t use_size_factors, int32_t use_log1p,
                             float* Y, void* X, int32_t x_dtype, float* sf_out, void* stream);
int dca_expand_packed_counts_exact(const void* packed, int32_t bits, const int64_t* ovf_indptr, const void* ovf_entries,
                                   const double* n_counts, int32_t n_rows, int32_t genes, double median, int32_t flags,
                                   const double* gene_mean, const double* gene_std, float* Y, void* X, int32_t x_dtype,
                                   float* sf_out, void* stream);
int dca_expand_sparse_counts_exact(const void* bitmap, const int64_t* nib_indptr, const void* nibbles,
                                   int32_t max_row_nibble_bytes, const int64_t* ovf_indptr, const void* ovf_entries,
                                   const double* n_counts, int32_t n_rows, int32_t genes, double median, int32_t flags,
                                   const double* gene_mean, const double* gene_std, float* Y, void* X, int32_t x_dtype,
                                   float* sf_out, void* stream);

typedef struct dca_packed_counts {
  int32_t struct_bytes;
  int32_t bits;
  int64_t n_rows;
  int32_t genes;
  int32_t max_row_nibble_bytes;
  const void* packed;
  const int64_t* ovf_indptr;
  const void* ovf_entries;
  const int64_t* nib_indptr;
  const void* nibbles;
  const double* n_counts;
} dca_packed_counts;

int dca_pack_count_rows(const float* Y, int64_t ldy, int64_t n_rows, int32_t genes, int64_t* stats, int64_t ld_stats,
                        void* stream);
int dca_pack_rows_device(const float* Y, int64_t ldy, int64_t n_rows, int64_t row0, const dca_packed_counts* dst,
                         void* stream);
int dca_expand_rows_exact(const dca_packed_counts* src, const int32_t* rows, int32_t n, double median, int32_t flags,
                          const double* gene_mean, const double* gene_std, float* Y, void* X, int32_t x_dtype,
                          float* sf_out, void* stream);
int dca_packed_train_step(dca_handle* h, const dca_packed_counts* src, const int32_t* rows, int32_t batch, void* stream);
int dca_packed_eval_step(dca_handle* h, const dca_packed_counts* src, const int32_t* rows, int32_t batch, void* stream);
int dca_packed_predict(dca_handle* h, const dca_packed_counts* src, const int32_t* rows, int32_t batch, float* mean_out,
                       float* disp_out, float* pi_out, int64_t ld_out, float* latent_out, void* stream);

int dca_zinb_loss_fwd_bwd(const float* Y, int64_t ldy, const int32_t* rows, const float* sf,
                          const float* m, const float* d, const float* pi, int64_t ld,
                          int32_t batch, int32_t genes, int32_t ae_type, float ridge, float inv_n,
                          void* dzm, void* dzd, void* dzp, int32_t grad_dtype,
                          float* dtheta, double* loss_sum, void* workspace, size_t workspace_bytes,
                          void* stream);
int dca_zinb_loss_workspace_bytes(int32_t batch, int32_t genes, size_t* bytes);
int dca_zinb_loss_fwd(const float* Y, int64_t ldy, const int32_t* rows, const float* sf,
                      const float* m, const float* d, const float* pi, int64_t ld,
                      int32_t batch, int32_t genes, int32_t ae_type, float ridge,
                      double* loss_sum, void* workspace, size_t workspace_bytes, void* stream);

int dca_zinb_elem_host(int32_t ae_type, float y, float m, float sf, float d, float pi, float ridge,
                       float out[4]);

int dca_dropout_mask_host(uint64_t seed, uint64_t step, int32_t layer, int64_t n, float rate, uint8_t* keep);
int dca_activation_host(int32_t act, float x, float alpha, float out[2]);

int dca_dense_heads_fwd(const float* H, int64_t ldh, int32_t batch, int32_t K, int32_t genes,
                        const float* w_mean, const float* b_mean,
                        const float* w_disp, const float* b_disp,
                        const float* w_pi, const float* b_pi,
                        const float* row_scale,
                        float* m_out, float* d_out, float* pi_out, int64_t ld_out, void* stream);

int dca_tc_heads_fwd(const void* Hb, int32_t batch, const void* Wk, const float* bias, int32_t genes,
                     int32_t n_heads, const int32_t kind[3], const float* row_scale,
                     float* out0, float* out1, float* out2, int64_t ld_out, void* stream);

int dca_tc_heads_loss(const void* Hb, int32_t batch, const void* Wk, const float* bias, int32_t genes,
                      const float* Y, int64_t ldy, const int32_t* rows, const float* sf, float ridge, float inv_n,
                      void* dzm, void* dzd, void* dzp, int64_t ldz, double* loss_sum, void* workspace,
                      size_t workspace_bytes, void* stream);

int dca_tc_gene_gemm(int32_t mode, const void* Z0, const void* Z1, const void* Z2, int64_t ldz, int32_t batch,
                     int32_t genes, int32_t n_heads, const void* H, const void* W, float* out_b,
                     float* dW0, float* dW1, float* dW2, int64_t dW_ld, int32_t dW_transposed,
                     float* db0, float* db1, float* db2, void* stream);
int dca_tc_gene_gemm_sms(int32_t mode, const void* Z0, const void* Z1, const void* Z2, int64_t ldz, int32_t batch,
                         int32_t genes, int32_t n_heads, const void* H, const void* W, float* out_b,
                         float* dW0, float* dW1, float* dW2, int64_t dW_ld, int32_t dW_transposed,
                         float* db0, float* db1, float* db2, void* stream, int32_t sm_count);
int dca_tc_gene_gemm_rows(int32_t mode, const void* Z0, const void* Z1, const void* Z2, int64_t ldz, const int32_t* rows,
                          int32_t batch, int32_t genes, int32_t n_heads, const void* H, const void* W, float* out_b,
                          float* dW0, float* dW1, float* dW2, int64_t dW_ld, int32_t dW_transposed,
                          float* db0, float* db1, float* db2, void* stream, int32_t sm_count);

#define DCA_PRE_SIZE_FACTORS 1
#define DCA_PRE_LOG1P 2
#define DCA_PRE_SCALE 4
int dca_preprocess_workspace_bytes(int64_t n_cells, int32_t genes, size_t* bytes);
int dca_counts_csr_to_dense(const int64_t* indptr, const int32_t* indices, const float* data, int64_t n_cells,
                            int32_t genes, float* Y, int64_t ldy, void* stream);
int dca_count_totals(const float* Y, int64_t ldy, int64_t n_cells, int32_t genes, double* cell_totals,
                     double* gene_totals, int64_t* n_bad, void* workspace, size_t workspace_bytes, void* stream);
int dca_gather_counts(const float* Y, int64_t ldy, const int32_t* rows, int64_t n_rows, const int32_t* cols,
                      int32_t n_cols, float* out, int64_t ldo, void* stream);
int dca_log_moments(const float* Y, int64_t ldy, int64_t n_cells, int32_t genes, const double* n_counts, double median,
                    int32_t flags, double* mean, double* std, void* workspace, size_t workspace_bytes, void* stream);
int dca_normalize_write(const float* Y, int64_t ldy, int64_t n_cells, int32_t genes, const double* n_counts,
                        double median, int32_t flags, const double* mean, const double* std, void* X, int32_t x_dtype,
                        int64_t ldx, void* stream);
int dca_stats_workspace_bytes(int64_t n_cells, int32_t genes, int64_t max_chunk_rows, size_t* bytes);
int dca_stats_begin(int64_t n_cells, int32_t genes, void* workspace, size_t workspace_bytes, void* stream);
int dca_count_totals_rows(const float* Y, int64_t ldy, int64_t row0, int64_t n_rows, int64_t n_cells, int32_t genes,
                          double* cell_totals, void* workspace, size_t workspace_bytes, void* stream);
int dca_count_totals_finish(int64_t n_cells, int32_t genes, double* gene_totals, int64_t* n_bad, void* workspace,
                            size_t workspace_bytes, void* stream);
int dca_log_moments_rows(int32_t pass, const float* Y, int64_t ldy, int64_t row0, int64_t n_rows, int64_t n_cells,
                         int32_t genes, const double* n_counts, double median, int32_t flags, const double* mean,
                         void* workspace, size_t workspace_bytes, void* stream);
int dca_log_moments_finish(int32_t pass, int64_t n_cells, int32_t genes, int32_t flags, double* out, void* workspace,
                           size_t workspace_bytes, void* stream);

int dca_tc_probe(const void* A, int32_t a_rows, int32_t a_cols, const void* B, int32_t b_rows, int32_t b_cols,
                 int32_t a_mn_major, int32_t b_mn_major, int32_t M, int32_t N, int32_t K,
                 int32_t a_lbo, int32_t a_sbo, int32_t b_lbo, int32_t b_sbo, float* D, void* stream);

#define DCA_N_PHASES 6
int dca_profile_enable(dca_handle* h, int32_t on);
int dca_profile_read(dca_handle* h, double ms[DCA_N_PHASES], int64_t counts[DCA_N_PHASES], int32_t reset);

int dca_engine_info(const dca_handle* h, int32_t info[8]);

int dca_write_text_matrix(const char* path, const void* matrix, int32_t is_float64, int64_t rows, int64_t cols,
                          int64_t ld, const char* const* row_names, const char* const* col_names,
                          int32_t transpose, int32_t threads);

int dca_read_text_counts(const char* path, int32_t sep, int32_t transpose, int64_t chunk_bytes, int32_t device,
                         void* stream, float* out, int64_t out_elems, int64_t* label_offsets, char* label_bytes,
                         int64_t label_cap, int64_t* info);

int dca_count_escapes(const void* counts, int32_t dtype, int64_t rows, int64_t cols, int64_t ld, int64_t* per_row,
                      int32_t threads);
int dca_pack_counts(const void* counts, int32_t dtype, int64_t rows, int64_t cols, int64_t ld, int32_t bits,
                    void* packed, const int64_t* indptr, void* entries, int32_t threads);

int dca_sparse_counts(const void* counts, int32_t dtype, int64_t rows, int64_t cols, int64_t ld, int64_t* nnz, int64_t* esc,
                      int32_t threads);
int dca_pack_sparse(const void* counts, int32_t dtype, int64_t rows, int64_t cols, int64_t ld, void* bitmap,
                    const int64_t* nib_indptr, void* nibbles, const int64_t* ovf_indptr, void* entries, int32_t threads);

int64_t dca_launch_count(void);
int dca_set_tunable(const char* name, int64_t value);

#ifdef __cplusplus
}
#endif
#endif
```

Measured before the change: 2.662 million.

## Store head gradients dZ in gene-tiled layout and load them via 3D TMA

The fused heads-loss kernel now writes the bf16 dZ gradients in a gene-tile-major layout, with each 128-gene tile stored contiguously over all cells. It zero-fills inactive rows so that padded tiles stay clean. The gene GEMM backward (mode 3) reads that layout through a new 3D tensor map, which turns its TMA loads into contiguous chunks instead of strided rows across the full gene width. The intent is better write coalescing and DRAM/L2 locality between the loss and backward stages. A separate CTA-count override for the loss kernel is exposed but left unused by default.

```diff
diff --git a/dca_b200/_lib.py b/dca_b200/_lib.py
--- a/dca_b200/_lib.py
+++ b/dca_b200/_lib.py
@@ -109,6 +109,8 @@
     "dca_tc_heads_fwd": (C.c_int, [_vp, _i32, _vp, _vp, _i32, _i32, C.POINTER(_i32 * 3), _vp, _vp, _vp, _vp, _i64, _vp]),
     "dca_tc_heads_loss": (C.c_int, [_vp, _i32, _vp, _vp, _i32, _vp, _i64, _vp, _vp, _f, _f, _vp, _vp, _vp, _i64, _vp,
                                     _vp, _sz, _vp]),
+    "dca_tc_heads_loss_ctas": (C.c_int, [_vp, _i32, _vp, _vp, _i32, _vp, _i64, _vp, _vp, _f, _f, _vp, _vp, _vp, _i64, _vp,
+                                         _vp, _sz, _vp, _i32]),
     "dca_tc_gene_gemm": (C.c_int, [_i32, _vp, _vp, _vp, _i64, _i32, _i32, _i32, _vp, _vp, _vp, _vp, _vp, _vp, _i64, _i32,
                                    _vp, _vp, _vp, _vp]),
     "dca_tc_gene_gemm_sms": (C.c_int, [_i32, _vp, _vp, _vp, _i64, _i32, _i32, _i32, _vp, _vp, _vp, _vp, _vp, _vp, _i64,
diff --git a/dca_b200/csrc/dca_internal.cuh b/dca_b200/csrc/dca_internal.cuh
--- a/dca_b200/csrc/dca_internal.cuh
+++ b/dca_b200/csrc/dca_internal.cuh
@@ -116,8 +116,10 @@
                  cudaStream_t s);
 int gene_gemm_tc(int mode, const __nv_bfloat16* const Z[3], int64_t ldz, const int32_t* rows, int B, int G, int n_heads,
                  const __nv_bfloat16* H, const __nv_bfloat16* const W[3], float* out_b, float* const dW[3], int64_t dW_ld,
-                 int dW_transposed, float* const db[3], void* ws, size_t ws_bytes, int sm_count, cudaStream_t s);
+                 int dW_transposed, float* const db[3], void* ws, size_t ws_bytes, int sm_count, cudaStream_t s,
+                 int z_tiled = 0);
 size_t gene_gemm_workspace_bytes(int B);
+inline size_t dz_tiled_elems(int B, int G) { return (size_t)cdiv(G, 128) * 128 * (size_t)B; }
 int flash_zinb_tc(const __nv_bfloat16* H3, int B, int G, const __nv_bfloat16* const W[3], const float* const bias[3],
                   const float* Y, int64_t ldy, const int32_t* rows, const float* sf, float ridge, float inv_n,
                   float* dH3, float* const dW[3], float* const db[3], void* ws, size_t ws_bytes, double* loss_sum,
@@ -151,6 +153,8 @@
   double* loss_sum; void* ws; size_t ws_bytes;
   int counter_ready = 0;
   float* fin_loss_slot = nullptr; double* fin_epoch_acc = nullptr; const double* fin_penalty = nullptr; int fin_batch = 0;
+  int ctas = 0;
+  int dz_tiled = 0;
 };
 int heads_loss_tc(const HeadsLossArgs& a, cudaStream_t s);
 
diff --git a/dca_b200/csrc/dense_tc.cu b/dca_b200/csrc/dense_tc.cu
--- a/dca_b200/csrc/dense_tc.cu
+++ b/dca_b200/csrc/dense_tc.cu
@@ -38,6 +38,24 @@
   if (r != CUDA_SUCCESS) {
     set_error("cuTensorMapEncodeTiled failed (%d): rows=%llu cols=%llu ld=%llu box=%ux%u elem=%d", (int)r,
               (unsigned long long)rows, (unsigned long long)cols, (unsigned long long)ld_elems, box_rows, box_cols, elem_bytes);
+    return DCA_ERR_CUDA;
+  }
+  return DCA_OK;
+}
+
+int make_tensor_map_gene_tiles(CUtensorMap* out, const void* base, uint64_t rows, uint64_t tiles) {
+  EncodeTiledFn fn = encode_fn();
+  if (!fn) { set_error("cuTensorMapEncodeTiled is not available from the driver"); return DCA_ERR_CUDA; }
+  cuuint64_t dims[3] = {128, rows, tiles};
+  cuuint64_t strides[2] = {128 * 2, rows * 128 * 2};
+  cuuint32_t box[3] = {64, 128, 1};
+  cuuint32_t estr[3] = {1, 1, 1};
+  CUresult r = fn(out, CU_TENSOR_MAP_DATA_TYPE_BFLOAT16, 3, const_cast<void*>(base), dims, strides, box, estr,
+                  CU_TENSOR_MAP_INTERLEAVE_NONE, CU_TENSOR_MAP_SWIZZLE_128B, CU_TENSOR_MAP_L2_PROMOTION_L2_256B,
+                  CU_TENSOR_MAP_FLOAT_OOB_FILL_NONE);
+  if (r != CUDA_SUCCESS) {
+    set_error("cuTensorMapEncodeTiled failed (%d): gene tiles, rows=%llu tiles=%llu", (int)r, (unsigned long long)rows,
+              (unsigned long long)tiles);
     return DCA_ERR_CUDA;
   }
   return DCA_OK;
diff --git a/dca_b200/csrc/engine.cu b/dca_b200/csrc/engine.cu
--- a/dca_b200/csrc/engine.cu
+++ b/dca_b200/csrc/engine.cu
@@ -1,3 +1,4 @@
+#include <algorithm>
 #include <cmath>
 #include <cstdarg>
 #include <cstdio>
@@ -183,7 +184,7 @@
   if (tc_heads || tc_enc) { ggws_bytes = tc::gene_gemm_workspace_bytes((int)B); o_ggws = take(ggws_bytes); }
   if (tc_heads) {
     o_h3b = take(2 * B * 64);
-    for (int k = 0; k < n_slots; ++k) o_dzb[k] = take(2 * B * (size_t)G);
+    for (int k = 0; k < n_slots; ++k) o_dzb[k] = take(2 * std::max(B * (size_t)G, tc::dz_tiled_elems((int)B, G)));
   }
   if (tc_enc) {
     o_da1b = take(2 * B * 64);
@@ -481,6 +482,7 @@
     ha.H3 = bf(o_h3b); ha.B = Bn; ha.G = G;
     for (int k = 0; k < 3; ++k) { ha.W[k] = bf(o_pbf) + head_W[slot_head[k]]; ha.bias[k] = pp(head_b[slot_head[k]]); ha.dz[k] = bf(o_dzb[k]); }
     ha.Y = Y; ha.ldy = ldy; ha.rows = rows; ha.sf = sf; ha.ridge = cfg.ridge; ha.inv_n = inv_n; ha.ldz = G;
+    ha.dz_tiled = 1;
     ha.loss_sum = d(o_acc) + 4; ha.ws = base + o_lossws; ha.ws_bytes = loss_ws_bytes;
     ha.counter_ready = 1;
     ha.fin_loss_slot = gp(P); ha.fin_epoch_acc = d(o_acc); ha.fin_penalty = any_pen ? d(o_acc) + 5 : nullptr; ha.fin_batch = Bn;
@@ -520,14 +522,16 @@
       for (int k = 0; k < n_slots; ++k) {
         const __nv_bfloat16* Z1[3] = {Z[k], Z[k], Z[k]}; const __nv_bfloat16* W1[3] = {Wk[k], Wk[k], Wk[k]};
         float* dW1[3] = {dWp[k], dWp[k], dWp[k]}; float* db1[3] = {dbp[k], dbp[k], dbp[k]};
-        DCA_TRY(tc::gene_gemm_tc(3, Z1, G, nullptr, Bn, G, 1, bf(o_h3b), W1, dh, dW1, G, 1, db1, base + o_ggws, ggws_bytes, sm_count, s));
+        DCA_TRY(tc::gene_gemm_tc(3, Z1, G, nullptr, Bn, G, 1, bf(o_h3b), W1, dh, dW1, G, 1, db1, base + o_ggws, ggws_bytes, sm_count, s,
+                                 heads_loss));
         const int h = slot_head[k];
         DCA_CUDA_OK(cudaEventRecord(ev_fork, s));
         DCA_CUDA_OK(cudaStreamWaitEvent(comm_stream, ev_fork, 0));
         DCA_TRY(allreduce_range(head_W[h], head_b[h] + G, comm_stream));
       }
     } else
-    DCA_TRY(tc::gene_gemm_tc(3, Z, G, nullptr, Bn, G, n_slots, bf(o_h3b), Wk, dh, dWp, G, 1, dbp, base + o_ggws, ggws_bytes, sm_count, s));
+    DCA_TRY(tc::gene_gemm_tc(3, Z, G, nullptr, Bn, G, n_slots, bf(o_h3b), Wk, dh, dWp, G, 1, dbp, base + o_ggws, ggws_bytes, sm_count, s,
+                             heads_loss));
   } else
   for (int k = 0; k < 3; ++k) {
     if (head_W[k] < 0 || !dz[k]) continue;
diff --git a/dca_b200/csrc/gene_gemm_tc.cu b/dca_b200/csrc/gene_gemm_tc.cu
--- a/dca_b200/csrc/gene_gemm_tc.cu
+++ b/dca_b200/csrc/gene_gemm_tc.cu
@@ -33,6 +33,7 @@
   float* db[3];
   float* part; int64_t part_stride;
   const int32_t* rows; const __nv_bfloat16* zsrc; int64_t ldz;
+  int z_tiled;
 };
 
 __device__ __forceinline__ void cp_async_16(uint32_t smem_dst, const void* src, uint32_t src_bytes) {
@@ -101,7 +102,10 @@
       const int cb = cb0 + t / ng, gb = gb0 + t % ng;
       uint8_t* dst = s_st + st * kStage;
       mbar_expect_tx(&full[st], gather ? kStage - kZBytes : kStage);
-      if (!gather) {
+      if (p.z_tiled) {
+        tma_load_3d(dst, mz, 0, cb * 128, gb, &full[st]);
+        tma_load_3d(dst + kZBytes / 2, mz, 64, cb * 128, gb, &full[st]);
+      } else if (!gather) {
         tma_load_2d(dst, mz, gb * 128, cb * 128, &full[st]);
         tma_load_2d(dst + kZBytes / 2, mz, gb * 128 + 64, cb * 128, &full[st]);
       }
@@ -272,15 +276,21 @@
 
 int gene_gemm_tc(int mode, const __nv_bfloat16* const Z[3], int64_t ldz, const int32_t* rows, int B, int G, int n_heads,
                  const __nv_bfloat16* H, const __nv_bfloat16* const W[3], float* out_b, float* const dW[3], int64_t dW_ld,
-                 int dW_transposed, float* const db[3], void* ws, size_t ws_bytes, int sm_count, cudaStream_t s) {
+                 int dW_transposed, float* const db[3], void* ws, size_t ws_bytes, int sm_count, cudaStream_t s,
+                 int z_tiled) {
   using namespace gg;
+  if (z_tiled && (mode != 3 || rows)) { set_error("gene_gemm_tc: gene-tiled Z is for mode 3 on a contiguous batch"); return DCA_ERR_BAD_ARG; }
   if (ldz % 8 != 0) { set_error("gene_gemm_tc: ldz must be a multiple of 8 (16-byte TMA stride)"); return DCA_ERR_BAD_ARG; }
   if (mode < 1 || mode > 3) { set_error("gene_gemm_tc: bad mode %d", mode); return DCA_ERR_BAD_ARG; }
   if (rows && (mode == 3 || n_heads != 1)) { set_error("gene_gemm_tc: row indices are for modes 1 and 2 (one Z)"); return DCA_ERR_BAD_ARG; }
   const bool do_a = mode & 2, do_b = mode & 1;
   if (do_b && (!ws || ws_bytes < gene_gemm_workspace_bytes(B))) { set_error("gene_gemm_tc: workspace too small"); return DCA_ERR_BAD_ARG; }
   CUtensorMap mz[3], mh, mw[3], mdw[3];
-  for (int i = 0; i < 3; ++i) DCA_TRY(make_tensor_map_2d(&mz[i], Z[i < n_heads ? i : 0], 2, 1, (uint64_t)B, (uint64_t)G, (uint64_t)ldz, 128, 64, 1));
+  for (int i = 0; i < 3; ++i) {
+    const __nv_bfloat16* z = Z[i < n_heads ? i : 0];
+    if (z_tiled) DCA_TRY(make_tensor_map_gene_tiles(&mz[i], z, (uint64_t)B, (uint64_t)cdiv(G, 128)));
+    else DCA_TRY(make_tensor_map_2d(&mz[i], z, 2, 1, (uint64_t)B, (uint64_t)G, (uint64_t)ldz, 128, 64, 1));
+  }
   mh = mz[0];
   for (int i = 0; i < 3; ++i) mw[i] = mdw[i] = mz[0];
   if (do_a) {
@@ -306,7 +316,7 @@
   base.n_cb = cdiv(B, 128); base.n_gb = cdiv(G, 128);
   for (int i = 0; i < 3; ++i) base.db[i] = db ? db[i] : nullptr;
   base.part = reinterpret_cast<float*>(ws); base.part_stride = (int64_t)base.n_cb * 128 * 64;
-  base.rows = rows; base.zsrc = Z[0]; base.ldz = ldz;
+  base.rows = rows; base.zsrc = Z[0]; base.ldz = ldz; base.z_tiled = z_tiled;
 
 #define DCA_GG_LAUNCH(P, A, Bb, Cc, WKk, MG)                                                                           \
   do {                                                                                                                 \
diff --git a/dca_b200/csrc/tc_common.cuh b/dca_b200/csrc/tc_common.cuh
--- a/dca_b200/csrc/tc_common.cuh
+++ b/dca_b200/csrc/tc_common.cuh
@@ -66,6 +66,13 @@
   asm volatile(
       "cp.async.bulk.tensor.2d.shared::cluster.global.mbarrier::complete_tx::bytes [%0], [%1, {%2, %3}], [%4];"
       ::"r"(smem_u32(smem_dst)), "l"(reinterpret_cast<uint64_t>(m)), "r"(c0), "r"(c1), "r"(smem_u32(bar)) : "memory");
+}
+__device__ __forceinline__ void tma_load_3d(void* smem_dst, const CUtensorMap* m, int32_t c0, int32_t c1, int32_t c2,
+                                            uint64_t* bar) {
+  asm volatile(
+      "cp.async.bulk.tensor.3d.shared::cluster.global.mbarrier::complete_tx::bytes [%0], [%1, {%2, %3, %4}], [%5];"
+      ::"r"(smem_u32(smem_dst)), "l"(reinterpret_cast<uint64_t>(m)), "r"(c0), "r"(c1), "r"(c2), "r"(smem_u32(bar))
+      : "memory");
 }
 __device__ __forceinline__ void tma_reduce_add_2d(const CUtensorMap* m, int32_t c0, int32_t c1, const void* smem_src) {
   asm volatile("cp.reduce.async.bulk.tensor.2d.global.shared::cta.add.tile.bulk_group [%0, {%1, %2}], [%3];"
@@ -143,6 +150,7 @@
 
 int make_tensor_map_2d(CUtensorMap* out, const void* base, int elem_bytes, int is_bf16, uint64_t rows, uint64_t cols,
                        uint64_t ld_elems, uint32_t box_rows, uint32_t box_cols, int swizzle);
+int make_tensor_map_gene_tiles(CUtensorMap* out, const void* base, uint64_t rows, uint64_t tiles);
 
 }
 }
diff --git a/dca_b200/csrc/zinb_loss.cu b/dca_b200/csrc/zinb_loss.cu
--- a/dca_b200/csrc/zinb_loss.cu
+++ b/dca_b200/csrc/zinb_loss.cu
@@ -790,6 +790,7 @@
   int B, G, nblk, units;
   float ridge, inv_n;
   __nv_bfloat16* dz[3]; int64_t ldz;
+  int dz_tiled;
   double* loss_partial; const float* lf;
 };
 
@@ -922,10 +923,13 @@
           const RowGrads g = zinb_row_ring<true>(vy, vm, vd, vp, row_sf, active, p.ridge, p.inv_n, q, lf, lsum_lg, lsum_nb,
                                                  lsum_r, tacc, [] {});
           if (active) {
-            const int64_t off = (int64_t)r * p.ldz + gcol0;
+            const int64_t off = p.dz_tiled ? ((int64_t)t * p.B + r) * 128 + col : (int64_t)r * p.ldz + gcol0;
             st4(p.dz[0] + off, g.gmA.x, g.gmA.y, g.gmB.x, g.gmB.y);
             st4(p.dz[1] + off, g.gdA.x, g.gdA.y, g.gdB.x, g.gdB.y);
             st4(p.dz[2] + off, g.gpA.x, g.gpA.y, g.gpB.x, g.gpB.y);
+          } else if (p.dz_tiled) {
+            const int64_t off = ((int64_t)t * p.B + r) * 128 + 4 * lane;
+            for (int h = 0; h < 3; ++h) st4(p.dz[h] + off, 0.f, 0.f, 0.f, 0.f);
           }
         }
       }
@@ -1102,7 +1106,7 @@
   using namespace hl;
   const int B = a.B, G = a.G;
   auto al = [](const void* q, uintptr_t n) { return (reinterpret_cast<uintptr_t>(q) & (n - 1)) == 0; };
-  if (B <= 0 || G <= 0 || G % 8 != 0 || a.ldy % 4 != 0 || !al(a.Y, 16) || a.ldz % 4 != 0 || a.ldz < G ||
+  if (B <= 0 || G <= 0 || G % 8 != 0 || a.ldy % 4 != 0 || !al(a.Y, 16) || (!a.dz_tiled && (a.ldz % 4 != 0 || a.ldz < G)) ||
       !al(a.dz[0], 8) || !al(a.dz[1], 8) || !al(a.dz[2], 8)) {
     set_error("heads_loss_tc: need G %% 8 == 0, a 16-byte aligned Y with ldy %% 4 == 0 and 8-byte aligned dZ with ldz %% 4 == 0 (>= G)");
     return DCA_ERR_BAD_ARG;
@@ -1115,7 +1119,7 @@
   for (int i = 0; i < 3; ++i) DCA_TRY(tc::make_tensor_map_2d(&mw[i], a.W[i], 2, 1, 64, (uint64_t)G, (uint64_t)G, 64, 64, 1));
   Params p;
   for (int i = 0; i < 3; ++i) { p.bias[i] = a.bias[i]; p.dz[i] = a.dz[i]; }
-  p.Y = a.Y; p.ldy = a.ldy; p.rows = a.rows; p.sf = a.sf; p.B = B; p.G = G; p.ldz = a.ldz;
+  p.Y = a.Y; p.ldy = a.ldy; p.rows = a.rows; p.sf = a.sf; p.B = B; p.G = G; p.ldz = a.ldz; p.dz_tiled = a.dz_tiled;
   p.nblk = cdiv(B, 64);
   const long long units = (long long)cdiv(G, 128) * p.nblk;
   if (units > INT_MAX) { set_error("heads_loss_tc: %lld (gene tile, cell block) units, over 2^31 - 1", units); return DCA_ERR_BAD_ARG; }
@@ -1127,7 +1131,8 @@
   if (!a.counter_ready) DCA_CUDA_OK(cudaMemsetAsync(fa.counter, 0, sizeof(unsigned), s));
   static bool attr = false;
   if (!attr) { DCA_CUDA_OK(cudaFuncSetAttribute(heads_loss_kernel, cudaFuncAttributeMaxDynamicSharedMemorySize, (int)kSmemBytes)); attr = true; }
-  const int grid = (int)std::min<long long>(p.units, sm_count_cached());
+  const int ctas = a.ctas > 0 ? std::min(a.ctas, sm_count_cached()) : sm_count_cached();
+  const int grid = (int)std::min<long long>(p.units, ctas);
   heads_loss_kernel<<<grid, kCtaThreads, kSmemBytes, s>>>(mh, mw[0], mw[1], mw[2], p, fa);
   DCA_LAUNCH_CHECK();
   return DCA_OK;
@@ -1172,7 +1177,15 @@
                                  const float* Y, int64_t ldy, const int32_t* rows, const float* sf, float ridge, float inv_n,
                                  void* dzm, void* dzd, void* dzp, int64_t ldz, double* loss_sum, void* workspace,
                                  size_t workspace_bytes, void* stream) {
-  if (!Hb || !Wk || !bias || !Y || !dzm || !dzd || !dzp || !loss_sum || batch <= 0 || genes <= 0) {
+  return dca_tc_heads_loss_ctas(Hb, batch, Wk, bias, genes, Y, ldy, rows, sf, ridge, inv_n, dzm, dzd, dzp, ldz, loss_sum,
+                                workspace, workspace_bytes, stream, 0);
+}
+
+extern "C" int dca_tc_heads_loss_ctas(const void* Hb, int32_t batch, const void* Wk, const float* bias, int32_t genes,
+                                      const float* Y, int64_t ldy, const int32_t* rows, const float* sf, float ridge,
+                                      float inv_n, void* dzm, void* dzd, void* dzp, int64_t ldz, double* loss_sum,
+                                      void* workspace, size_t workspace_bytes, void* stream, int32_t ctas) {
+  if (!Hb || !Wk || !bias || !Y || !dzm || !dzd || !dzp || !loss_sum || batch <= 0 || genes <= 0 || ctas < 0) {
     set_error("dca_tc_heads_loss: bad argument"); return DCA_ERR_BAD_ARG;
   }
   HeadsLossArgs a{};
@@ -1180,7 +1193,7 @@
   for (int i = 0; i < 3; ++i) { a.W[i] = (const __nv_bfloat16*)Wk + (size_t)i * 64 * genes; a.bias[i] = bias + (size_t)i * genes; }
   a.Y = Y; a.ldy = ldy; a.rows = rows; a.sf = sf; a.ridge = ridge; a.inv_n = inv_n;
   a.dz[0] = (__nv_bfloat16*)dzm; a.dz[1] = (__nv_bfloat16*)dzd; a.dz[2] = (__nv_bfloat16*)dzp; a.ldz = ldz;
-  a.loss_sum = loss_sum; a.ws = workspace; a.ws_bytes = workspace_bytes;
+  a.loss_sum = loss_sum; a.ws = workspace; a.ws_bytes = workspace_bytes; a.ctas = ctas;
   return heads_loss_tc(a, (cudaStream_t)stream);
 }
 
diff --git a/include/dca_b200.h b/include/dca_b200.h
--- a/include/dca_b200.h
+++ b/include/dca_b200.h
@@ -250,6 +250,10 @@
                       const float* Y, int64_t ldy, const int32_t* rows, const float* sf, float ridge, float inv_n,
                       void* dzm, void* dzd, void* dzp, int64_t ldz, double* loss_sum, void* workspace,
                       size_t workspace_bytes, void* stream);
+int dca_tc_heads_loss_ctas(const void* Hb, int32_t batch, const void* Wk, const float* bias, int32_t genes,
+                           const float* Y, int64_t ldy, const int32_t* rows, const float* sf, float ridge, float inv_n,
+                           void* dzm, void* dzd, void* dzp, int64_t ldz, double* loss_sum, void* workspace,
+                           size_t workspace_bytes, void* stream, int32_t ctas);
 
 int dca_tc_gene_gemm(int32_t mode, const void* Z0, const void* Z1, const void* Z2, int64_t ldz, int32_t batch,
                      int32_t genes, int32_t n_heads, const void* H, const void* W, float* out_b,
```

New measurement: 2.706 million (median of 6 runs). 1.6% higher.
